# nv-tlabs/ASE

Measured on AMD Instinct MI355X. Metric: ASE PPO-update samples/sec (4096 envs x horizon 32), higher is better.
Workload: dtype f16; 1 GPU; BASELINE configs[1]: ASE agent, 4096 envs x horizon 32, obs 253 / act 31 / amp obs 1400 / latent 64, [1024,1024,512] MLPs + disc + shared-trunk encoder, minibatch 16384 (amp 4096) x 6 mini-epochs = 48 optimisation steps per update; random-init weights; precision_choice=auto without an oracle leg: the first candidate, replay=program, parallelism=single GPU

## Files before the change

ase_amd/backend.py:

```python
import ctypes as C

import torch

from . import lib as L


_HOSTFN = C.CFUNCTYPE(None, C.c_void_p)


def _ptr(t):
    return None if t is None else C.c_void_p(t.data_ptr())


def _ld(t):
    return 0 if t is None else int(t.stride(0))


def _code(dtype):
    if dtype == torch.bfloat16:
        return L.BF16
    if dtype == torch.float32:
        return L.F32
    if dtype == torch.float16:
        return L.F16
    raise L.AseHipError(f"unsupported storage dtype {dtype}")


class HipBackend:
    name = "hip"
    nt_fused_epilogue = True

    def __init__(self, device=None, x3=False):
        self.x3 = x3 if x3 == 'f16' else bool(x3)
        self._recording, self._host_keep, self._host_error = None, {}, None
        self.tn_workspace = True
        if not torch.cuda.is_available():
            raise L.AseHipError("HipBackend needs a ROCm GPU (torch.cuda.is_available() is False); "
                                "the update path has no CPU fallback")
        self.device = torch.device(device if device is not None else f"cuda:{torch.cuda.current_device()}")
        self.lib = L.get()
        self._head_scratch = torch.zeros(L.PPO_SCRATCH, dtype=torch.float64, device=self.device)
        self._head_scratch_ls = None

    def _stream(self):
        return C.c_void_p(torch.cuda.current_stream(self.device).cuda_stream)

    def zero_(self, t):
        assert t.is_contiguous()
        L.check(self.lib.ase_hip_memset(_ptr(t), 0, t.numel() * t.element_size(), self._stream()), "memset")

    def copy_(self, dst, src):
        assert dst.is_contiguous() and src.is_contiguous() and dst.dtype == src.dtype and dst.numel() == src.numel()
        L.check(self.lib.ase_hip_memcpy(_ptr(dst), _ptr(src), dst.numel() * dst.element_size(), self._stream()), "memcpy")

    def mark(self):
        ev = C.c_int(0)
        L.check(self.lib.ase_hip_mark(self._stream(), C.byref(ev)), "mark")
        return ev.value

    def wait(self, ev):
        L.check(self.lib.ase_hip_wait(self._stream(), int(ev)), "wait")

    def prog_create(self):
        p = C.c_void_p()
        L.check(self.lib.ase_hip_prog_create(C.byref(p)), "prog_create")
        return p

    def prog_begin(self, prog):
        L.check(self.lib.ase_hip_prog_begin(prog), "prog_begin")
        self._recording = prog.value
        self._host_keep.setdefault(prog.value, [])

    def prog_end(self, prog):
        self._recording = None
        L.check(self.lib.ase_hip_prog_end(prog), "prog_end")

    def host_call(self, fn):
        if self._recording is None:
            fn()
            return

        def trampoline(_arg, fn=fn):
            try:
                fn()
            except BaseException as e:
                self._host_error = e
        cb = _HOSTFN(trampoline)
        self._host_keep[self._recording].append(cb)
        L.check(self.lib.ase_hip_prog_host(C.cast(cb, C.c_void_p), None), "prog_host")

    def prog_launch(self, prog):
        L.check(self.lib.ase_hip_prog_launch(prog), "prog_launch")
        if self._host_error is not None:
            e, self._host_error = self._host_error, None
            raise e

    def prog_size(self, prog):
        return self.lib.ase_hip_prog_size(prog)

    def prog_destroy(self, prog):
        self.lib.ase_hip_prog_destroy(prog)
        self._host_keep.pop(prog.value, None)

    def _gemm_code(self, dtype, exps=None):
        c = _code(dtype)
        if self.x3 and c == L.F32:
            if self.x3 == 'f16' and exps is not None:
                return L.F32H3 | (int(exps[0]) << 8) | (int(exps[1]) << 16)
            return L.F32X3
        return c

    def gemm_nt(self, A, B, Cm, M, N, K, bias=None, aux=None, aux_mode=L.AUX_NONE, colsum=None, colsum_n=0,
                act=L.ACT_NONE, alpha=1.0, aux_split=0, aux_delta=0, mask_out=None, x3_exps=None, alpha_dev=None,
                seed=None, twin=None, sq=None, store=True):
        dt = self._gemm_code(A.dtype, x3_exps)
        assert B.dtype == A.dtype
        if aux_mode == L.AUX_RELU_BITS:
            assert aux.dtype == torch.int32
        else:
            assert aux is None or aux.dtype == A.dtype
        assert mask_out is None or mask_out.dtype == (A.dtype if act >= L.ACT_SILU else torch.int32)
        if seed is not None or twin is not None or sq is not None:
            assert (dt & 0xFF) == L.F32H3, "seed / twin / sq belong to the half-split f32 launches (x3 = 'f16', x3_exps)"
            assert Cm.dtype == torch.float32 and (store or twin is not None)
            sw, ss = seed if seed is not None else (None, 0.0)
            acc, slot, sscale, dyn = sq if sq is not None else (None, 0, 0.0, None)
            assert acc is None or acc.dtype == torch.float64
            L.check(self.lib.ase_hip_gemm_nt_ex(_ptr(A), _ld(A), _ptr(B), _ld(B), _ptr(Cm) if store else None, _ld(Cm), _ptr(bias), _ptr(aux),
                                                _ld(aux), int(aux_split), int(aux_delta), _ptr(colsum), int(colsum_n),
                                                _ptr(mask_out), _ld(mask_out), M, N, K, act, aux_mode, 0,
                                                float(alpha), _ptr(alpha_dev), dt,
                                                _ptr(sw), 0 if sw is None else sw.numel(), float(ss),
                                                _ptr(twin), _ld(twin), 0 if twin is None else _code(twin.dtype),
                                                None if acc is None else C.c_void_p(acc.data_ptr() + 8 * int(slot)), float(sscale),
                                                _ptr(dyn), self._stream()), "gemm_nt_ex")
            return
        out_f32 = int(Cm.dtype == torch.float32 and A.dtype != torch.float32)
        L.check(self.lib.ase_hip_gemm_nt(_ptr(A), _ld(A), _ptr(B), _ld(B), _ptr(Cm), _ld(Cm), _ptr(bias), _ptr(aux),
                                         _ld(aux), int(aux_split), int(aux_delta), _ptr(colsum), int(colsum_n),
                                         _ptr(mask_out), _ld(mask_out), M, N, K, act, aux_mode, out_f32,
                                         float(alpha), _ptr(alpha_dev), dt, self._stream()), "gemm_nt")

    def gemm_tn(self, A, B, G, M, N, K, n_real, k_real, split_src, split_dst, alpha=1.0, gbias=None, bias_rows=0, alpha_dev=None):
        L.check(self.lib.ase_hip_gemm_tn(_ptr(A), _ld(A), _ptr(B), _ld(B), _ptr(G), _ptr(gbias), int(bias_rows), M, N, K,
                                         n_real, k_real,
                                         split_src, split_dst, float(alpha), _ptr(alpha_dev), self._gemm_code(A.dtype), self._stream()),
                "gemm_tn")

    def grouped_tn_ok(self, dtype, M, n_real, K, bias_rows):
        return dtype in (torch.bfloat16, torch.float16) and M % 64 == 0 and bias_rows % 64 == 0

    def make_tn_plan(self, problems, target_wg=0, alpha_dev=None):
        import struct
        n = len(problems)
        tab = (C.c_int64 * (16 * n))()
        for i, (A, B, G, gb, br, M, N, K, nr, kr, ss, sd, alpha) in enumerate(problems):
            assert A.dtype in (torch.bfloat16, torch.float16) and B.dtype == A.dtype and G.dtype == torch.float32
            row = [A.data_ptr(), _ld(A), B.data_ptr(), _ld(B), G.data_ptr(), 0 if gb is None else gb.data_ptr(), int(br),
                   M, N, K, nr, kr, ss, sd, struct.unpack('<i', struct.pack('<f', float(alpha)))[0], 0]
            for j, v in enumerate(row):
                tab[16 * i + j] = int(v)
        max_work = 8192
        work = (C.c_int32 * (4 * max_work))()
        red = (C.c_int32 * (4 * max_work))()
        n_work, n_red = C.c_int(0), C.c_int(0)
        L.check(self.lib.ase_hip_gemm_tn_grouped_plan(tab, n, int(target_wg), work, max_work, C.byref(n_work), red, max_work,
                                                      C.byref(n_red)), "gemm_tn_grouped_plan")
        nw, nr = n_work.value, n_red.value
        dev_tab = torch.tensor(list(tab), dtype=torch.int64, device=self.device)
        dev_work = torch.tensor(list(work[:4 * nw]), dtype=torch.int32, device=self.device)
        dev_red = torch.tensor(list(red[:4 * nr]), dtype=torch.int32, device=self.device)
        ws = torch.empty(nw * L.TN_SLAB, dtype=torch.float32, device=self.device) if self.tn_workspace else None
        return {'problems': dev_tab, 'work': dev_work, 'n_work': nw, 'red': dev_red, 'n_red': nr, 'ws': ws, 'keep': problems,
                'dtype': _code(problems[0][0].dtype), 'alpha_dev': alpha_dev}

    def gemm_tn_grouped(self, plan):
        L.check(self.lib.ase_hip_gemm_tn_grouped(_ptr(plan['problems']), _ptr(plan['work']), plan['n_work'], _ptr(plan['red']),
                                                 plan['n_red'], _ptr(plan['ws']), _ptr(plan.get('alpha_dev')), plan['dtype'],
                                                 self._stream()),
                "gemm_tn_grouped")

    def refresh_shadow(self, W, Ws, Wts, split_src, split_dst, x3_exp=None):
        n, k = W.shape
        ref = Ws if Ws is not None else Wts
        code = _code(ref.dtype)
        if x3_exp is not None:
            assert ref.dtype == torch.float32
            code = L.F32H3 | (int(x3_exp) << 16)
        L.check(self.lib.ase_hip_refresh_shadow(_ptr(W), n, k, _ptr(Ws), _ld(Ws), _ptr(Wts), _ld(Wts), split_src,
                                                split_dst, code, self._stream()), "refresh_shadow")

    def refresh_shadow_multi(self, desc, items, dtype):
        L.check(self.lib.ase_hip_refresh_shadow_multi(_ptr(desc), desc.shape[0], _code(dtype), self._stream()),
                "refresh_shadow_multi")

    def apply_multi(self, desc, items, dtype, opt_state, acc):
        L.check(self.lib.ase_hip_apply_multi(_ptr(desc), desc.shape[0], _ptr(opt_state), _ptr(acc), _code(dtype),
                                             self._stream()), "apply_multi")

    def apply_multi_split(self, desc, items, dtype, opt_state, acc, desc2, items2):
        assert desc2.shape == (desc.shape[0], 8) and desc2.is_contiguous()
        L.check(self.lib.ase_hip_apply_multi_v2(_ptr(desc), desc.shape[0], _ptr(desc2), _ptr(opt_state), _ptr(acc), _code(dtype),
                                                self._stream()), "apply_multi_v2")

    def gather_multi(self, desc, items, idx, remap, M):
        L.check(self.lib.ase_hip_gather_multi(_ptr(desc), desc.shape[0], _ptr(idx), remap[0], remap[1], M,
                                              self._stream()), "gather_multi")

    def build_amp_obs(self, root_pos, root_rot, root_vel, root_ang_vel, dof_pos, dof_vel, key_body_pos, dof_offsets,
                      local_root_obs, root_height_obs, hist, shift=True):
        n, S, F = hist.shape
        offs = (C.c_int32 * len(dof_offsets))(*[int(x) for x in dof_offsets])
        for t in (root_pos, root_rot, root_vel, root_ang_vel, dof_pos, dof_vel, key_body_pos, hist):
            assert t.dtype == torch.float32 and t.is_contiguous()
        L.check(self.lib.ase_hip_build_amp_obs(_ptr(root_pos), _ptr(root_rot), _ptr(root_vel), _ptr(root_ang_vel), _ptr(dof_pos),
                                               _ptr(dof_vel), _ptr(key_body_pos), n, dof_pos.shape[1], key_body_pos.shape[1], offs,
                                               len(dof_offsets) - 1, int(local_root_obs), int(root_height_obs), _ptr(hist), S,
                                               int(shift), self._stream()), "build_amp_obs")

    def motion_state(self, clips, motion_ids, times):
# ... 541 lines not shown
        L.check(self.lib.ase_hip_rms_moments(_ptr(src), _ld(src), D, _ptr(idx), remap[0], remap[1], M, _ptr(state),
                                             _ptr(sums), self._stream()), "rms_moments")

    @staticmethod
    def _stream_arrays(streams):
        n = len(streams)
        srcs = (C.c_void_p * n)(*[s[0].data_ptr() for s in streams])
        lds = (C.c_int64 * n)(*[int(s[0].stride(0)) for s in streams])
        idxs = (C.c_void_p * n)(*[None if s[1] is None else s[1].data_ptr() for s in streams])
        rh = (C.c_int * n)(*[int(s[2][0]) for s in streams])
        rn = (C.c_int * n)(*[int(s[2][1]) for s in streams])
        return n, srcs, lds, idxs, rh, rn

    def rms_moments_multi(self, streams, D, M, state, sums_list):
        n, srcs, lds, idxs, rh, rn = self._stream_arrays(streams)
        sums = (C.c_void_p * n)(*[t.data_ptr() for t in sums_list])
        L.check(self.lib.ase_hip_rms_moments_multi(srcs, lds, idxs, rh, rn, sums, n, D, M, _ptr(state), self._stream()),
                "rms_moments_multi")

    def rms_normalize_multi(self, streams, D, M, means, stds, outs):
        n, srcs, lds, idxs, rh, rn = self._stream_arrays(streams)
        mp = (C.c_void_p * n)(*[t.data_ptr() for t in means])
        sp = (C.c_void_p * n)(*[t.data_ptr() for t in stds])
        op = (C.c_void_p * n)(*[t.data_ptr() for t in outs])
        lo = (C.c_int64 * n)(*[int(t.stride(0)) for t in outs])
        L.check(self.lib.ase_hip_rms_normalize_multi(srcs, lds, idxs, rh, rn, mp, sp, op, lo, n, D, M, _code(outs[0].dtype),
                                                     self._stream()), "rms_normalize_multi")

    def rms_normalize_multi_twin(self, streams, D, M, means, stds, outs, outs32):
        n, srcs, lds, idxs, rh, rn = self._stream_arrays(streams)
        mp = (C.c_void_p * n)(*[t.data_ptr() for t in means])
        sp = (C.c_void_p * n)(*[t.data_ptr() for t in stds])
        op = (C.c_void_p * n)(*[t.data_ptr() for t in outs])
        lo = (C.c_int64 * n)(*[int(t.stride(0)) for t in outs])
        assert all(t is None or t.dtype == torch.float32 for t in outs32)
        op32 = (C.c_void_p * n)(*[None if t is None else t.data_ptr() for t in outs32])
        lo32 = (C.c_int64 * n)(*[0 if t is None else int(t.stride(0)) for t in outs32])
        L.check(self.lib.ase_hip_rms_normalize_multi_v2(srcs, lds, idxs, rh, rn, mp, sp, op, lo, op32, lo32, n, D, M,
                                                        _code(outs[0].dtype), self._stream()), "rms_normalize_multi_v2")

    def rms_finalize(self, state, D, sums, count, n_streams, mean_out, std_out):
        counts = (C.c_int32 * max(n_streams, 1))(*([int(count)] * max(n_streams, 1)))
        L.check(self.lib.ase_hip_rms_finalize(_ptr(state), D, _ptr(sums), counts, n_streams, _ptr(mean_out),
                                              _ptr(std_out), self._stream()), "rms_finalize")

    def rms_normalize(self, src, D, idx, remap, M, mean, std, outs):
        outs = list(outs) + [None] * (3 - len(outs))
        dt = _code(outs[0].dtype)
        L.check(self.lib.ase_hip_rms_normalize(_ptr(src), _ld(src), D, _ptr(idx), remap[0], remap[1], M, _ptr(mean),
                                               _ptr(std), _ptr(outs[0]), _ld(outs[0]), _ptr(outs[1]), _ld(outs[1]),
                                               _ptr(outs[2]), _ld(outs[2]), dt, self._stream()), "rms_normalize")

    def rms_unnormalize(self, state, x, y):
        L.check(self.lib.ase_hip_rms_unnormalize(_ptr(state), _ptr(x), _ptr(y), x.numel(), self._stream()),
                "rms_unnormalize")

    def gather_rows(self, src, D, idx, remap, M, dst):
        L.check(self.lib.ase_hip_gather_rows(_ptr(src), _ld(src), D, _ptr(idx), remap[0], remap[1], M, _ptr(dst),
                                             _ld(dst), _code(dst.dtype), self._stream()), "gather_rows")

    def reduce_sum(self, x, n, square, acc, slot):
        L.check(self.lib.ase_hip_reduce_sum(_ptr(x), n, int(square), _ptr(acc), slot, self._stream()), "reduce_sum")

    def ppo_head(self, mu, value, mb, new_z, logstd, d_mu, d_value, db_mu, db_value, acc, M, m_global, act_dim,
                 z_dim, masked, div_on, mu_tanh, clip_value, e_clip, critic_coef, bounds_coef, div_coef, div_tar,
                 mu_out=None, grad_scale=1.0, dyn=None, ls_mode=L.LS_FROZEN, d_logstd=None, db_logstd=None, entropy_coef=0.0):
        scratch = self._head_scratch if ls_mode == L.LS_FROZEN else self.reserve_learned_logstd()
        L.check(self.lib.ase_hip_ppo_head(
            _ptr(mu), _ld(mu), _ptr(value), _ld(value), _ptr(mb['actions']), _ptr(mb['mu']), _ptr(mb['sigma']),
            _ptr(mb['old_logp_actions']), _ptr(mb['advantages']), _ptr(mb.get('old_values')), _ptr(mb['returns']),
            _ptr(mb.get('rand_action_mask')), _ptr(mb.get('ase_latents')), _ptr(new_z), _ptr(logstd),
            _ptr(d_mu), _ld(d_mu), _ptr(d_value), _ld(d_value), _ptr(db_mu), _ptr(db_value), _ptr(mu_out), _ptr(acc),
            _ptr(scratch),
            M, m_global, act_dim, z_dim, int(masked), int(div_on), int(mu_tanh), int(clip_value),
            float(e_clip), float(critic_coef), float(bounds_coef), float(div_coef), float(div_tar), float(grad_scale),
            _ptr(dyn), int(ls_mode), _ld(logstd) if ls_mode == L.LS_ROWS else 0, _ptr(d_logstd), _ld(d_logstd),
            _ptr(db_logstd), float(entropy_coef), _code(d_mu.dtype), self._stream()), "ppo_head")

    def reserve_learned_logstd(self):
        if self._head_scratch_ls is None:
            self._head_scratch_ls = torch.zeros(L.PPO_SCRATCH_LS, dtype=torch.float64, device=self.device)
        return self._head_scratch_ls

    def disc_head(self, logit, d_logit, db_logit, acc, amb, amb_global, disc_coef, grad_scale=1.0, dyn=None):
        L.check(self.lib.ase_hip_disc_head(_ptr(logit), _ld(logit), _ptr(d_logit), _ld(d_logit), _ptr(db_logit),
                                           _ptr(acc), amb, amb_global, float(disc_coef), float(grad_scale), _ptr(dyn),
                                           _code(d_logit.dtype), self._stream()), "disc_head")

    def enc_head(self, e, z, d_e, db_enc, enc_out, acc, amb, amb_global, z_dim, enc_coef, grad_scale=1.0, dyn=None):
        L.check(self.lib.ase_hip_enc_head(_ptr(e), _ld(e), _ptr(z), _ld(z), _ptr(d_e), _ld(d_e), _ptr(db_enc),
                                          _ptr(enc_out), _ptr(acc), amb, amb_global, z_dim, float(enc_coef), float(grad_scale),
                                          _ptr(dyn), _code(d_e.dtype), self._stream()), "enc_head")

    def enc_gp_seed(self, e, z, u, rows, z_dim, scale=1.0):
        assert e.dtype == torch.float32 and z.dtype == torch.float32
        L.check(self.lib.ase_hip_enc_gp_seed(_ptr(e), _ld(e), _ptr(z), _ld(z), _ptr(u), _ld(u), rows, z_dim, float(scale),
                                             _code(u.dtype), self._stream()), "enc_gp_seed")

    def enc_gp_back(self, e, z, du, d_e, db_enc, rows, z_dim, grad_scale=1.0, dyn=None):
        assert e.dtype == torch.float32 and z.dtype == torch.float32 and du.dtype == torch.float32
        L.check(self.lib.ase_hip_enc_gp_back(_ptr(e), _ld(e), _ptr(z), _ld(z), _ptr(du), _ld(du), _ptr(d_e), _ld(d_e),
                                             _ptr(db_enc), rows, z_dim, float(grad_scale), _ptr(dyn), _code(d_e.dtype),
                                             self._stream()), "enc_gp_back")

    def gp_seed(self, h, w, g, rows, width, scale=1.0, act=L.ACT_RELU):
        L.check(self.lib.ase_hip_gp_seed(_ptr(h), _ld(h), _ptr(w), _ptr(g), _ld(g), rows, width, float(scale), int(act),
                                         _code(h.dtype), self._stream()), "gp_seed")

    def gp_second(self, twin, g, dg, dz, rows, width, act):
        L.check(self.lib.ase_hip_gp_second(_ptr(twin), _ld(twin), _ptr(g), _ld(g), _ptr(dg), _ld(dg), _ptr(dz), _ld(dz), rows,
                                           width, int(act), _code(dz.dtype), self._stream()), "gp_second")

    def colsum(self, x, rows, cols, out, scale=1.0):
        assert x.dtype == torch.float32 and out.dtype == torch.float32
        L.check(self.lib.ase_hip_colsum(_ptr(x), _ld(x), rows, cols, float(scale), _ptr(out), self._stream()), "colsum")

    def sqnorm(self, x, rows, cols, acc, slot, scale=1.0, dyn=None):
        L.check(self.lib.ase_hip_sqnorm(_ptr(x), _ld(x), rows, cols, _ptr(acc), slot, float(scale), _ptr(dyn), _code(x.dtype),
                                        self._stream()),
                "sqnorm")

    def finalize_scalars(self, acc, out, m_global, amb_global, masked, has_disc, has_enc, has_div, c, opt_state=None, kl_threshold=0.0):
        L.check(self.lib.ase_hip_finalize_scalars(
            _ptr(acc), _ptr(out), m_global, amb_global, int(masked), int(has_disc), int(has_enc), int(has_div),
            float(c['critic_coef']), float(c['entropy_coef']), float(c.get('bounds_loss_coef') or 0.0), float(c.get('disc_coef', 0)),
            float(c.get('disc_logit_reg', 0)), float(c.get('disc_grad_penalty', 0)), float(c.get('disc_weight_decay', 0)),
            float(c.get('enc_coef', 0)), float(c.get('enc_weight_decay', 0)), float(c.get('amp_diversity_bonus', 0)),
            float(c.get('enc_grad_penalty', 0)), _ptr(opt_state), float(kl_threshold), self._stream()), "finalize_scalars")

    def begin_step(self, opt_state, acc, zero2=None, rng_bump=None):
        L.check(self.lib.ase_hip_begin_step(_ptr(opt_state), _ptr(acc), 0 if acc is None else acc.numel(), _ptr(zero2),
                                            0 if zero2 is None else zero2.numel(), _ptr(rng_bump), self._stream()),
                "begin_step")

    def adam(self, w, g, m, v, opt_state):
        L.check(self.lib.ase_hip_adam(_ptr(w), _ptr(g), _ptr(m), _ptr(v), w.numel(), _ptr(opt_state), self._stream()),
                "adam")

    def clip_scale(self, g, acc, slot, max_norm):
        L.check(self.lib.ase_hip_clip_scale(_ptr(g), g.numel(), _ptr(acc[slot:]), float(max_norm), self._stream()), "clip_scale")

    def axpy(self, g, w, c):
        L.check(self.lib.ase_hip_axpy(_ptr(g), _ptr(w), g.numel(), float(c), self._stream()), "axpy")

    def scaler_check(self, buf, scaler):
        assert buf.is_contiguous()
        L.check(self.lib.ase_hip_scaler_check(_ptr(buf), buf.numel(), _code(buf.dtype), _ptr(scaler), self._stream()),
                "scaler_check")

    def scaler_check_multi(self, bufs, scaler, table=None):
        if table is None:
            table = self.make_check_table(bufs)
        L.check(self.lib.ase_hip_scaler_check_multi(_ptr(table['rows']), table['n'], table['wg'], _ptr(scaler), self._stream()),
                "scaler_check_multi")

    def make_check_table(self, bufs):
        rows = []
        for t in bufs:
            assert t.is_contiguous() and t.numel() > 0
            rows.append([t.data_ptr(), t.numel(), _code(t.dtype)])
        big = max(t.numel() * t.element_size() for t in bufs)
        wg = max(1, min(1024, (big + 16383) // 16384))
        return {'rows': torch.tensor(rows, dtype=torch.int64, device=self.device), 'n': len(rows), 'wg': int(wg), 'keep': list(bufs)}

    def scaler_fold(self, scaler, scale_tab):
        L.check(self.lib.ase_hip_scaler_fold(_ptr(scaler), _ptr(scale_tab), self._stream()), "scaler_fold")

    def scaler_step(self, scaler, opt_state, opt_eff, grads, scale_tab=None):
        L.check(self.lib.ase_hip_scaler_step(_ptr(scaler), _ptr(opt_state), _ptr(opt_eff), _ptr(grads), grads.numel(),
                                             _ptr(scale_tab), self._stream()), "scaler_step")
# ... 38 lines not shown
```

ase_amd/csrc/gemm.hip:

```cpp
#include "gemm_nt.h"
#include <math.h>

namespace ase_nt {

unsigned long long* g_nt_prof = nullptr;
int g_nt_prof_clk = 0;

int nt_choice(int M, int N, int K, int es, bool b16) {
    if (N <= 64) return 0;
    const int t256 = ((M + 255) / 256) * ((N + 255) / 256);
    const bool big = N % 256 == 0 && t256 >= 192 && (t256 <= 256 || t256 % 256 == 0 || t256 >= 1024);
    if (big) {
        if (!(b16 && (K * es) % 128 == 0)) return 3;
        const int t192 = ((M + 191) / 192) * (N / 256);
        return (t256 < 256 && t192 <= 256 && t192 > t256) ? 6 : 2;
    }
    if ((K * es) % 128 != 0) return 1;
    const int t128 = ((M + 127) / 128) * ((N + 127) / 128), t64x128 = ((M + 63) / 64) * ((N + 127) / 128);
    if (t128 >= 512) return 1;
    if (t64x128 >= 512) return 4;
    return 5;
}

}

using namespace ase_nt;

extern "C" int ase_hip_debug_nt_profile(void* buf) {
    g_nt_prof = reinterpret_cast<unsigned long long*>(buf);
    return ASE_OK;
}

extern "C" int ase_hip_debug_nt_profile_clock(int shader_clock) {
    g_nt_prof_clk = shader_clock ? 1 : 0;
    return ASE_OK;
}

extern "C" int ase_hip_gemm_nt_kernel_id(int M, int N, int K, int dtype) {
    dtype &= 0xFF;
    return nt_choice(M, N, K, ase_elem_size(dtype), ase_elem_size(dtype) == 2);
}

namespace {

struct NTFused {
    const float* seed_w = nullptr; int seed_n = 0; float seed_scale = 0.f;
    void* twin = nullptr; int64_t ldtwin = 0; int twin_dtype = 0;
    double* sq_acc = nullptr; double sq_scale = 0.0; const float* sq_dyn = nullptr;
    bool any() const { return seed_w || twin || sq_acc; }
};

int gemm_nt_impl(const void* A, int64_t lda, const void* B, int64_t ldb, void* C, int64_t ldc,
                 const float* bias, const void* aux, int64_t ldaux, int aux_split, int aux_delta,
                 float* colsum, int colsum_n, void* mask_out, int64_t ldmask, int M, int N, int K, int act,
                 int aux_mode, int out_f32, float alpha, float* alpha_dev, int dtype_word, const NTFused& fu, void* stream) {
    const int dtype = dtype_word & 0xFF, ea = (dtype_word >> 8) & 0xFF, eb = (dtype_word >> 16) & 0xFF;
    const int es = ase_elem_size(dtype);
    ASE_CHECK_ARG(dtype == ASE_F32 || dtype == ASE_BF16 || dtype == ASE_F32X3 || dtype == ASE_F16 || dtype == ASE_F32H3,
                  "gemm_nt: bad dtype %d", dtype);
    ASE_CHECK_ARG(ea >= 0 && ea <= 24 && eb >= 0 && eb <= 24 && (dtype == ASE_F32H3 || (ea | eb) == 0),
                  "gemm_nt: operand scale exponents (bits 8-15 / 16-23 of dtype) are 0..24 and belong to ASE_F32H3 only");
    ASE_CHECK_ARG(A && B && (C || fu.twin) && M > 0 && N > 0 && K > 0, "gemm_nt: null/empty operand (M=%d N=%d K=%d)", M, N, K);
    if (fu.any()) {
        ASE_CHECK_ARG(dtype == ASE_F32H3 && colsum == nullptr && act <= ASE_ACT_RELU &&
                          (aux_mode == ASE_AUX_NONE || aux_mode == ASE_AUX_RELU_BITS),
                      "gemm_nt_ex: seed / twin / sum of squares belong to ASE_F32H3 launches without column sums, with no activation or "
                      "ReLU and no mask operand or a bit matrix");
        ASE_CHECK_ARG(fu.seed_w == nullptr || (fu.seed_n >= 0 && fu.seed_n <= N), "gemm_nt_ex: seed_n=%d outside [0, N]", fu.seed_n);
        ASE_CHECK_ARG(fu.twin == nullptr || ((fu.twin_dtype == ASE_F16 || fu.twin_dtype == ASE_BF16) && fu.ldtwin >= N &&
                                             ((uintptr_t)fu.twin % 8) == 0 && (fu.ldtwin * 2) % 8 == 0),
                      "gemm_nt_ex: the twin is f16 / bf16, 8-byte aligned, ldtwin >= N in whole 8-byte steps");
        ASE_CHECK_ARG(fu.sq_acc == nullptr || ((uintptr_t)fu.sq_acc % 8) == 0, "gemm_nt_ex: misaligned sq_acc");
    }
    ASE_CHECK_ARG((K * es) % 64 == 0, "gemm_nt: K=%d is not a multiple of %d elements", K, 64 / es);
    ASE_CHECK_ARG(lda >= K && ldb >= K && (ldc >= N || C == nullptr), "gemm_nt: leading dimension too small");
    ASE_CHECK_ARG(((uintptr_t)A % 16) == 0 && ((uintptr_t)B % 16) == 0 && (lda * es) % 16 == 0 && (ldb * es) % 16 == 0,
                  "gemm_nt: A/B must be 16-byte aligned with 16-byte row pitch");
    ASE_CHECK_ARG(aux_mode == ASE_AUX_NONE || aux != nullptr, "gemm_nt: aux_mode %d without aux", aux_mode);
    const bool bits = aux_mode == ASE_AUX_RELU_BITS;
    ASE_CHECK_ARG(N % 4 == 0 && ((uintptr_t)C % 16) == 0 && (ldc * (out_f32 ? 4 : es)) % 8 == 0 &&
                      (aux == nullptr || bits || (((uintptr_t)aux % 8) == 0 && (ldaux * es) % 8 == 0)),
                  "gemm_nt: C / aux must allow 8/16-byte row-vector access (N %% 4 == 0, aligned pitches)");
    ASE_CHECK_ARG(!bits || (((uintptr_t)aux % 4) == 0 && ldaux * 32 >= N), "gemm_nt: bit mask needs ldaux >= N / 32 words");
    const bool smooth = act >= ASE_ACT_SILU;
    ASE_CHECK_ARG(act >= ASE_ACT_NONE && act <= ASE_ACT_SOFTPLUS, "gemm_nt: unknown activation %d", act);
    ASE_CHECK_ARG((aux_mode & 0xFF) <= ASE_AUX_PREACT && ((aux_mode & 0xFF) == ASE_AUX_PREACT || (aux_mode >> 8) == 0) &&
                      (aux_mode >> 8) <= ASE_ACT_SOFTPLUS, "gemm_nt: bad aux_mode 0x%x", aux_mode);
    ASE_CHECK_ARG(mask_out == nullptr || smooth || (N % 32 == 0 && ((uintptr_t)mask_out % 4) == 0 && ldmask * 32 >= N),
                  "gemm_nt: mask_out needs N %% 32 == 0 and ldmask >= N / 32 words");
    ASE_CHECK_ARG(mask_out == nullptr || !smooth || (ldmask >= N && ((uintptr_t)mask_out % 16) == 0 && (ldmask * es) % 8 == 0),
                  "gemm_nt: the pre-activation twin needs ldmask >= N elements, 16-byte alignment");
    NTParams p;
    p.A = (const char*)A; p.lda = lda * es;
    p.B = (const char*)B; p.ldb = ldb * es;
    p.C = (char*)C; p.ldc = ldc * (out_f32 ? 4 : es);
    p.mask_out = smooth ? nullptr : (uint32_t*)mask_out; p.ldmask = ldmask;
    p.pre_out = smooth ? (char*)mask_out : nullptr; p.ldpre = ldmask * es;
    p.bias = bias; p.aux = (const char*)aux; p.ldaux = bits ? ldaux * 4 : ldaux * es; p.aux_split = aux_split > 0 ? aux_split : M; p.aux_delta = aux_delta; p.colsum = colsum; p.colsum_n = colsum ? colsum_n : 0;
    p.M = M; p.N = N; p.K = K; p.act = act; p.aux_mode = aux_mode; p.out_f32 = out_f32; p.alpha = alpha; p.alpha_dev = alpha_dev;
    p.tiles_m = p.tiles_n = 0;
    p.prof = nullptr;
    p.prof_clk = 0;
    p.sa = 1.f;
    p.seed_w = fu.seed_w; p.seed_n = fu.seed_n; p.seed_scale = fu.seed_scale;
    p.twin = (char*)fu.twin; p.ldtwin = fu.ldtwin * 2; p.twin_dtype = fu.twin_dtype;
    p.sq_acc = fu.sq_acc; p.sq_scale = fu.sq_scale; p.sq_dyn = fu.sq_dyn;
    if (dtype == ASE_BF16) return dispatch_nt_bf16(p, (hipStream_t)stream);
    if (dtype == ASE_F16) return dispatch_nt_f16(p, (hipStream_t)stream);
    if (dtype == ASE_F32X3) return dispatch_nt_x3(p, (hipStream_t)stream);
    if (dtype == ASE_F32H3) {
        p.sa = ldexpf(1.f, ea);
        p.alpha = ldexpf(alpha, -(ea + eb));
        return dispatch_nt_h3(p, (hipStream_t)stream);
    }
    return dispatch_nt_f32(p, (hipStream_t)stream);
}

}

extern "C" int ase_hip_gemm_nt(const void* A, int64_t lda, const void* B, int64_t ldb, void* C, int64_t ldc,
                               const float* bias, const void* aux, int64_t ldaux, int aux_split, int aux_delta,
                               float* colsum, int colsum_n, void* mask_out, int64_t ldmask, int M, int N, int K, int act,
                               int aux_mode, int out_f32, float alpha, float* alpha_dev, int dtype_word, void* stream) {
    return gemm_nt_impl(A, lda, B, ldb, C, ldc, bias, aux, ldaux, aux_split, aux_delta, colsum, colsum_n, mask_out, ldmask, M, N, K,
                        act, aux_mode, out_f32, alpha, alpha_dev, dtype_word, NTFused{}, stream);
}

extern "C" int ase_hip_gemm_nt_ex(const void* A, int64_t lda, const void* B, int64_t ldb, void* C, int64_t ldc,
                                  const float* bias, const void* aux, int64_t ldaux, int aux_split, int aux_delta,
                                  float* colsum, int colsum_n, void* mask_out, int64_t ldmask, int M, int N, int K, int act,
                                  int aux_mode, int out_f32, float alpha, float* alpha_dev, int dtype_word,
                                  const float* seed_w, int seed_n, float seed_scale, void* twin, int64_t ldtwin, int twin_dtype,
                                  double* sq_acc, double sq_scale, const float* sq_dyn, void* stream) {
    NTFused fu;
    fu.seed_w = seed_w; fu.seed_n = seed_n; fu.seed_scale = seed_scale;
    fu.twin = twin; fu.ldtwin = ldtwin; fu.twin_dtype = twin_dtype;
    fu.sq_acc = sq_acc; fu.sq_scale = sq_scale; fu.sq_dyn = sq_dyn;
    return gemm_nt_impl(A, lda, B, ldb, C, ldc, bias, aux, ldaux, aux_split, aux_delta, colsum, colsum_n, mask_out, ldmask, M, N, K,
                        act, aux_mode, out_f32, alpha, alpha_dev, dtype_word, fu, stream);
}
```

ase_amd/csrc/gemm_nt.h:

```cpp
#pragma once
#include "common.h"
#include "act.h"
#include <type_traits>

namespace ase_nt {


__device__ __forceinline__ int xcd_remap(int bid, int nwg) {
    const int q = nwg >> 3, r = nwg & 7, xcd = bid & 7, loc = bid >> 3;
    const int base = (xcd < r) ? xcd * (q + 1) : r * (q + 1) + (xcd - r) * q;
    return base + loc;
}


template <int RB> __device__ __forceinline__ int lds_swz(int r) { return RB == 128 ? ((r >> 1) & 7) : ((r >> 2) & 3); }

typedef __attribute__((address_space(1))) const void gptr_t;
typedef __attribute__((address_space(3))) void lptr_t;

template <int N> __device__ __forceinline__ void wait_vmcnt() { asm volatile("s_waitcnt vmcnt(%0)" ::"n"(N) : "memory"); }

struct NTParams {
    const char* A; int64_t lda;
    const char* B; int64_t ldb;
    char* C; int64_t ldc;
    const float* bias;
    const char* aux; int64_t ldaux;
    int aux_split, aux_delta;
    float* colsum; int colsum_n;
    uint32_t* mask_out; int64_t ldmask;
    char* pre_out; int64_t ldpre;
    int M, N, K;
    int act, aux_mode, out_f32;
    float alpha;
    float* alpha_dev;
    float sa;
    int tiles_m, tiles_n;
    unsigned long long* prof;
    int prof_clk;
    const float* seed_w; int seed_n; float seed_scale;
    char* twin; int64_t ldtwin; int twin_dtype;
    double* sq_acc; double sq_scale; const float* sq_dyn;
};


typedef __attribute__((ext_vector_type(4))) int i32x4;

__device__ __forceinline__ i32x4 raw_buffer(const void* base) {
    const uint64_t a = (uint64_t)(uintptr_t)base;
    return i32x4{(int)(uint32_t)a, (int)(uint32_t)(a >> 32), (int)0x7FFFFFFF, 0x00020000};
}
#pragma clang diagnostic push
#pragma clang diagnostic ignored "-Winline-asm"
#define LDS_DMA16_ASM(SET_M0, ...)                                            \
    asm volatile(SET_M0 "\n\tbuffer_load_dwordx4 %1, %2, %3 offen lds"          \
                 :                                                              \
                 : "s"(lds_s), "v"(voff), "s"(rs), "s"(soff), "n"(IMM)          \
                 : "memory", "m0", ##__VA_ARGS__)
template <int IMM = 0, bool ADD = (IMM != 0)>
__device__ __forceinline__ void lds_dma16(uint32_t lds_s, uint32_t voff, i32x4 rs, uint32_t soff) {
    if constexpr (ADD) LDS_DMA16_ASM("s_add_u32 m0, %0, %4", "scc");
    else LDS_DMA16_ASM("s_mov_b32 m0, %0");
}
#undef LDS_DMA16_ASM
template <int IMM>
__device__ __forceinline__ void lds_dma16_global(uint32_t lds_s, const char* src) {
    asm volatile("s_add_u32 m0, %0, %2\n\ts_nop 0\n\tglobal_load_lds_dwordx4 %1, off" : : "s"(lds_s), "v"(src), "n"(IMM) : "memory", "m0", "scc");
}
#pragma clang diagnostic pop

template <typename T, bool SW>
__device__ __forceinline__ f32x16 nt8_mfma(const i32x4& a, const i32x4& b, const f32x16& c) {
    typedef typename V16<T>::x8 x8;
    if constexpr (SW) return mfma16<T>(__builtin_bit_cast(x8, b), __builtin_bit_cast(x8, a), c);
    else return mfma16<T>(__builtin_bit_cast(x8, a), __builtin_bit_cast(x8, b), c);
}


#define NT8_BARRIER()                        \
    do {                                     \
        __builtin_amdgcn_sched_barrier(0);   \
        __builtin_amdgcn_s_barrier();        \
        __builtin_amdgcn_sched_barrier(0);   \
    } while (0)


typedef float f32x2 __attribute__((ext_vector_type(2)));
typedef short i16x2 __attribute__((ext_vector_type(2)));
typedef int i32x2 __attribute__((ext_vector_type(2)));
typedef unsigned short u16x2 __attribute__((ext_vector_type(2)));
typedef __bf16 bf16x2 __attribute__((ext_vector_type(2)));
typedef _Float16 f16x2 __attribute__((ext_vector_type(2)));

template <typename T> __device__ __forceinline__ uint32_t cvt_relu_pk16(f32x2 v, float lo);
template <> __device__ __forceinline__ uint32_t cvt_relu_pk16<bf16_t>(f32x2 v, float lo) {
    const f32x2 l = {lo, lo};
    return __builtin_bit_cast(uint32_t, __builtin_convertvector(__builtin_elementwise_maximum(v, l), bf16x2));
}
template <> __device__ __forceinline__ uint32_t cvt_relu_pk16<f16_t>(f32x2 v, float lo) {
    const f16_t l16 = (f16_t)__builtin_amdgcn_fmed3f(lo, -65504.f, 65504.f);
    const f16x2 hi = {(f16_t)65504.f, (f16_t)65504.f}, l = {l16, l16};
    const f16x2 c = __builtin_elementwise_maximum(__builtin_elementwise_minimum(__builtin_convertvector(v, f16x2), hi), l);
    return __builtin_bit_cast(uint32_t, c);
}

__device__ __forceinline__ uint32_t ovf_fold(uint32_t run, uint32_t packed) {
    const uint32_t mag = packed & 0x7FFF7FFFu;
    asm("v_pk_max_u16 %0, %0, %1" : "+v"(run) : "v"(mag));
    return run;
}
template <typename T> __device__ __forceinline__ bool ovf_hit(uint32_t run) {
    return (run & 0xFFFFu) >= ovf_threshold<T>() || (run >> 16) >= ovf_threshold<T>();
}

template <typename T, int AUXK, bool MASK>
__device__ __forceinline__ uint32_t rows_frag(const f32x16& c, const f32x4 (&bias)[4], uint32_t w, f32x2 al, float relu_lo, int h,
                                              uint32_t (&pk)[4][2]) {
    uint32_t mlo = 0, mhi = 0;
#pragma unroll
    for (int g = 0; g < 4; ++g)
#pragma unroll
        for (int pr = 0; pr < 2; ++pr) {
            f32x2 v = {c[g * 4 + 2 * pr], c[g * 4 + 2 * pr + 1]};
            const f32x2 b = {bias[g][2 * pr], bias[g][2 * pr + 1]};
            v = v * al + b;
// ... 42 lines not shown
        uint32_t mword[NJ];
        uint4 out[NJ][2];
#pragma unroll
        for (int j = 0; j < NJ; ++j) {
            uint32_t pk[4][2];
            mword[j] = rows_frag<T, AUXK, MASK>(acc[i][j], bias[j], AUXK == 2 ? bits[i][j] >> (4 * h) : 0u, al, relu_lo, h, pk);
#pragma unroll
            for (int g = 0; g < 4; g += 2) {
                const auto s0 = __builtin_amdgcn_permlane32_swap(pk[g][0], pk[g + 1][0], false, false);
                const auto s1 = __builtin_amdgcn_permlane32_swap(pk[g][1], pk[g + 1][1], false, false);
                out[j][g >> 1] = make_uint4(s0[0], s1[0], s0[1], s1[1]);
                ovf = ovf_fold(ovf_fold(ovf_fold(ovf_fold(ovf, s0[0]), s1[0]), s0[1]), s1[1]);
            }
        }
        if (row_ok) {
#pragma unroll
            for (int j = 0; j < NJ; ++j)
#pragma unroll
                for (int g = 0; g < 4; g += 2) *reinterpret_cast<uint4*>(crow + (j * 32 + 8 * g) * 2) = out[j][g >> 1];
        }
        if constexpr (MASK) {
#pragma unroll
            for (int jp = 0; jp < NJ; jp += 2) {
                const auto w = __builtin_amdgcn_permlane32_swap(mword[jp], mword[jp + 1], false, false);
                const uint32_t full = w[0] | w[1];
                if (row_ok) p.mask_out[(int64_t)m * p.ldmask + (ncol0 >> 5) + jp + h] = full;
            }
        }
    }
    ovf_report(p.alpha_dev, ovf_hit<T>(ovf));
}

template <typename T, int AUXK, int NJ = 2, int NI = 4>
__device__ __forceinline__ void nt8_epilogue_rows(const NTParams& p, f32x16 (&acc)[NI][NJ], int lane, int mrow0, int ncol0,
                                                  const uint32_t (&bits)[NI][NJ]) {
    if (ncol0 >= p.N) return;
    if (p.mask_out) nt8_epilogue_rows_impl<T, AUXK, true, NJ, NI>(p, acc, lane, mrow0, ncol0, bits);
    else nt8_epilogue_rows_impl<T, AUXK, false, NJ, NI>(p, acc, lane, mrow0, ncol0, bits);
}


template <int UNITS> __device__ __forceinline__ void wait_dma_units() { wait_vmcnt<2 * UNITS>(); }
__device__ __forceinline__ void wait_dma_units_rt(int units) {
    if (units >= 4) wait_vmcnt<8>();
    else if (units == 3) wait_vmcnt<6>();
    else if (units == 2) wait_vmcnt<4>();
    else if (units == 1) wait_vmcnt<2>();
    else wait_vmcnt<0>();
}
__device__ __forceinline__ void nt8_sync_in() {
    NT8_BARRIER();
    asm volatile("s_waitcnt lgkmcnt(0)" ::: "memory");
    __builtin_amdgcn_sched_barrier(0);
    __builtin_amdgcn_s_setprio(1);
}
__device__ __forceinline__ void nt8_sync_out() {
    __builtin_amdgcn_s_setprio(0);
    NT8_BARRIER();
}

#define NT_PROF_STAMP(prof, tid, slot, shader_clk)                                                              \
    do {                                                                                                        \
        if ((prof) && (tid) == 0) (prof)[slot] = (shader_clk) ? (unsigned long long)clock64() : wall_clock64(); \
    } while (0)
#define NT_PROF_CLOSE(prof, tid, slot)                         \
    do {                                                       \
        if (prof) {                                            \
            asm volatile("s_waitcnt vmcnt(0)" ::: "memory");   \
            __syncthreads();                                   \
            if ((tid) == 0) (prof)[slot] = wall_clock64();     \
        }                                                      \
    } while (0)

extern unsigned long long* g_nt_prof;
extern int g_nt_prof_clk;

int nt_choice(int M, int N, int K, int es, bool b16);

int dispatch_nt_bf16(const NTParams& p, hipStream_t s);
int dispatch_nt_f16(const NTParams& p, hipStream_t s);
int dispatch_nt_f32(const NTParams& p, hipStream_t s);
int dispatch_nt_x3(const NTParams& p, hipStream_t s);
int dispatch_nt_h3(const NTParams& p, hipStream_t s);

}
```

ase_amd/csrc/gemm_nt_bf16.hip:

```cpp
#include "gemm_nt_kernels.h"

int ase_nt::dispatch_nt_bf16(const NTParams& p, hipStream_t s) { return dispatch_nt<bf16_t>(p, s); }
```

ase_amd/csrc/gemm_nt_f16.hip:

```cpp
#include "gemm_nt_kernels.h"

int ase_nt::dispatch_nt_f16(const NTParams& p, hipStream_t s) { return dispatch_nt<f16_t>(p, s); }
```

ase_amd/csrc/gemm_nt_kernels.h:

```cpp
#pragma once
#include "gemm_nt.h"
#include <stdlib.h>
#include <utility>

namespace {

using namespace ase_nt;

typedef uint32_t u32x4 __attribute__((ext_vector_type(4)));
template <int N, typename F, int... I> __device__ __forceinline__ void static_for_impl(F&& f, std::integer_sequence<int, I...>) {
    (f(std::integral_constant<int, I>{}), ...);
}
template <int N, typename F> __device__ __forceinline__ void static_for(F&& f) { static_for_impl<N>(f, std::make_integer_sequence<int, N>{}); }

template <typename T> struct Mma;

template <typename T> struct Mma16 {
    typedef typename V16<T>::x8 x8;
    template <int FM, int FN, int RB, bool SW = false>
    static __device__ __forceinline__ void tile(const char* sA, const char* sB, int lane, f32x16 (&acc)[FM][FN]) {
        const int r = lane & 31, h = lane >> 5, sw = lds_swz<RB>(r);
#pragma unroll
        for (int ks = 0; ks < RB / 32; ++ks) {
            x8 a[FM], b[FN];
// ... 620 lines not shown
    NTParams p = p0;
    p.tiles_m = (p.M + BM - 1) / BM;
    p.tiles_n = (p.N + BN - 1) / BN;
    ASE_LAUNCH(kern, dim3(p.tiles_m * p.tiles_n), dim3(WGM * WGN * 64), lds, stream, p);
    ASE_CHECK_LAUNCH("gemm_nt");
    return ASE_OK;
}


struct NT8Lane {
    uint32_t voff[4][2];
    uint32_t dst[4][2];
    int roff[4];
    i32x4 rsA, rsB;
};

template <int KIND>
__device__ __forceinline__ void nt8_piece(const NT8Lane& L, int g, int tile) {
    constexpr bool isB = (KIND == 1 || KIND == 2);
    lds_dma16(__builtin_amdgcn_readfirstlane(L.dst[KIND][g] + (uint32_t)(tile & 1) * 65536u), L.voff[KIND][g], isB ? L.rsB : L.rsA,
              (uint32_t)tile * 128u);
}

template <int KIND>
__device__ __forceinline__ void nt8_issue(const NT8Lane& L, int tile) {
#pragma unroll
    for (int g = 0; g < 2; ++g) nt8_piece<KIND>(L, g, tile);
}

__device__ __forceinline__ void nt8_read(i32x4 (&f)[4], const char* base, const NT8Lane& L) {
#pragma unroll
    for (int ks = 0; ks < 4; ++ks) f[ks] = *reinterpret_cast<const i32x4*>(base + L.roff[ks]);
}

template <typename T, int KIND, bool SW, int NA = 2>
__device__ __forceinline__ void nt8_mma_issue(f32x16& c0, f32x16& c1, const i32x4 (&a0)[4], const i32x4 (&a1)[4],
                                              const i32x4 (&b)[4], const NT8Lane& L, int tile, bool live) {
#pragma unroll
    for (int ks = 0; ks < 4; ++ks) {
        if (ks == 3) NT8_BARRIER();
        c0 = nt8_mfma<T, SW>(a0[ks], b[ks], c0);
        if constexpr (NA == 2) c1 = nt8_mfma<T, SW>(a1[ks], b[ks], c1);
        if (ks == 0 || ks == 2) {
            __builtin_amdgcn_sched_barrier(0);
            if (live) nt8_piece<KIND>(L, ks >> 1, tile);
            __builtin_amdgcn_sched_barrier(0);
        }
    }
    __builtin_amdgcn_sched_barrier(0);
    __builtin_amdgcn_s_setprio(0);
    __builtin_amdgcn_sched_barrier(0);
}

template <typename T, bool TAIL, bool SW, int NI = 4>
__device__ __forceinline__ void nt8_ktile(int t, int nk, const NT8Lane& L, const char* aP, const char* bP,
                                          f32x16 (&acc)[NI][2], i32x4 (&a0)[4], i32x4 (&a1)[4], i32x4 (&b0)[4],
                                          i32x4 (&b1)[4]) {
    constexpr int RB = 128;
    const int U = 4 * nk;
    const bool l1 = !TAIL || t + 1 < nk, l2 = !TAIL || t + 2 < nk;
    nt8_read(b0, bP, L);
    nt8_read(a0, aP, L);
    nt8_read(a1, aP + 32 * RB, L);
    if (!TAIL) wait_dma_units<3>();
    else wait_dma_units_rt(min(U, 4 * t + 6) - (4 * t + 3));
    nt8_sync_in();
    nt8_mma_issue<T, 2, SW>(acc[0][0], acc[1][0], a0, a1, b0, L, t + 1, l1);
    nt8_read(b1, bP + 32 * RB, L);
    if (!TAIL) wait_dma_units<3>();
    else wait_dma_units_rt(min(U, 4 * t + 7) - (4 * t + 4));
    nt8_sync_in();
    nt8_mma_issue<T, 3, SW>(acc[0][1], acc[1][1], a0, a1, b1, L, t + 1, l1);
    nt8_read(a0, aP + 64 * RB, L);
    if constexpr (NI == 4) nt8_read(a1, aP + 96 * RB, L);
    nt8_sync_in();
    nt8_mma_issue<T, 0, SW, NI - 2>(acc[2][1], acc[NI - 1][1], a0, a1, b1, L, t + 2, l2);
    if (!TAIL) wait_dma_units<3>();
    else if (t + 1 < nk) wait_dma_units_rt(min(U, 4 * t + 9) - (4 * t + 6));
    nt8_sync_in();
    nt8_mma_issue<T, 1, SW, NI - 2>(acc[2][0], acc[NI - 1][0], a0, a1, b0, L, t + 2, l2);
}


template <typename T, bool SW, int BM = 256>
__global__ __launch_bounds__(512) void gemm_nt8_kernel(NTParams p) {
    static_assert(sizeof(T) == 2, "the phased kernel takes the 16-bit storage types");
    static_assert(BM == 256 || (BM == 192 && SW), "192-row tiles come with the row-per-lane epilogue");
    constexpr int RB = 128, BN = 256, BK = 64, WM = BM / 2, NI = WM / 32;
    constexpr int kBuf = 512 * RB;
    extern __shared__ __attribute__((aligned(16))) char smem[];
    if (p.alpha_dev) p.alpha *= *p.alpha_dev;

    const int tid = threadIdx.x, lane = tid & 63;
    const int wid = __builtin_amdgcn_readfirstlane(tid >> 6);
    const int wr = wid >> 2, wc = wid & 3;
    const int nwg = p.tiles_m * p.tiles_n;
    const int tile = xcd_remap(blockIdx.x, nwg);
    const int bm0 = (tile / p.tiles_n) * BM, bn0 = (tile % p.tiles_n) * BN;

    NT_PROF_STAMP(p.prof, tid, blockIdx.x * 4 + 0, false);
    NT8Lane L;
    {
        const int lr = lane >> 3, slot = lane & 7;
#pragma unroll
        for (int g = 0; g < 2; ++g) {
            const int ra = g * WM + wid * 8;
            const int rb = (g * 2 + (wid >> 2)) * 64 + (wid & 3) * 8;
            const int ra1 = BM == 256 ? ra + 64 : (wid >> 2) * WM + 64 + (wid & 3) * 8;
            const int rows[4] = {ra, rb, rb + 32, ra1};
#pragma unroll
            for (int kind = 0; kind < 4; ++kind) {
                const int r = rows[kind] + lr;
                const bool isB = (kind == 1 || kind == 2);
                const int64_t grow = isB ? min(bn0 + r, p.N - 1) : min(bm0 + r, p.M - 1);
                L.voff[kind][g] = (uint32_t)(grow * (isB ? p.ldb : p.lda)) + (uint32_t)((slot ^ lds_swz<RB>(r)) << 4);
                L.dst[kind][g] = (uint32_t)(uintptr_t)smem + (isB ? BM * RB : 0) + rows[kind] * RB;
            }
        }
        const int r = lane & 31, h = lane >> 5, sw = lds_swz<RB>(r);
#pragma unroll
        for (int ks = 0; ks < 4; ++ks) L.roff[ks] = r * RB + (((ks * 2 + h) ^ sw) << 4);
        L.rsA = raw_buffer(p.A);
        L.rsB = raw_buffer(p.B);
    }

    f32x16 acc[NI][2];
#pragma unroll
    for (int i = 0; i < NI; ++i)
#pragma unroll
        for (int j = 0; j < 2; ++j)
#pragma unroll
            for (int e = 0; e < 16; ++e) acc[i][j][e] = 0.f;

    AuxReg<T, 2> pre_bits[16];
    uint32_t row_bits[NI][2];
    if constexpr (!SW) {
        if (p.aux_mode == ASE_AUX_RELU_BITS) nt_aux_load<T, 4, 2, 2, 2, 2>(p, 0, lane, bm0 + wr * WM, bn0 + wc * 64, pre_bits);
    }

    const int nk = p.K / BK;
    nt8_issue<0>(L, 0);
    nt8_issue<1>(L, 0);
    nt8_issue<2>(L, 0);
    nt8_issue<3>(L, 0);
    if (nk > 1) {
        nt8_issue<0>(L, 1);
        nt8_issue<1>(L, 1);
    }
    bool mask_dma = false;
    if constexpr (SW) {
        mask_dma = p.aux_mode == ASE_AUX_RELU_BITS && bn0 + wc * 64 < p.N;
        if (mask_dma) {
            char* mlds = smem + 2 * kBuf + wid * 1024;
#pragma unroll
            for (int i = 0; i < NI; ++i) {
                const int m = bm0 + wr * WM + i * 32 + (lane & 31);
                const int ma = (m >= p.aux_split) ? m - p.aux_delta : m;
                const uint32_t* w = reinterpret_cast<const uint32_t*>(p.aux + (int64_t)min(ma, p.M - 1) * p.ldaux) +
                                    ((bn0 + wc * 64) >> 5) + (lane >> 5);
                __builtin_amdgcn_global_load_lds((gptr_t*)w, (lptr_t*)(mlds + i * 256), 4, 0, 0);
            }
        }
    }
    if (nk > 1) {
        if (mask_dma) wait_vmcnt<8 + NI>(); else wait_dma_units<4>();
    } else {
        if (mask_dma) wait_vmcnt<4 + NI>(); else wait_dma_units<2>();
    }
    NT8_BARRIER();
    NT_PROF_STAMP(p.prof, tid, blockIdx.x * 4 + 1, p.prof_clk);
    if (wr == 1) NT8_BARRIER();

    i32x4 a0[4], a1[4], b0[4], b1[4];
    const int aoff = wr * WM * RB, boff = BM * RB + wc * 64 * RB;
    int t = 0;
    for (; t + 2 < nk; ++t) {
        const char* buf = smem + (t & 1) * kBuf;
        nt8_ktile<T, false, SW, NI>(t, nk, L, buf + aoff, buf + boff, acc, a0, a1, b0, b1);
    }
    for (; t < nk; ++t) {
        const char* buf = smem + (t & 1) * kBuf;
        nt8_ktile<T, true, SW, NI>(t, nk, L, buf + aoff, buf + boff, acc, a0, a1, b0, b1);
    }
    if (wr == 0) NT8_BARRIER();
    __syncthreads();
    NT_PROF_STAMP(p.prof, tid, blockIdx.x * 4 + 2, p.prof_clk);

    float* slab = reinterpret_cast<float*>(smem) + wid * (64 * 64);
    if constexpr (SW) {
        if (p.aux_mode == ASE_AUX_RELU_BITS) {
            const uint32_t* mw = reinterpret_cast<const uint32_t*>(smem + 2 * kBuf + wid * 1024);
#pragma unroll
            for (int i = 0; i < NI; ++i) {
                row_bits[i][0] = mw[i * 64 + (lane & 31)];
                row_bits[i][1] = mw[i * 64 + 32 + (lane & 31)];
            }
            nt8_epilogue_rows<T, 2, 2, NI>(p, acc, lane, bm0 + wr * WM, bn0 + wc * 64, row_bits);
        } else nt8_epilogue_rows<T, 0, 2, NI>(p, acc, lane, bm0 + wr * WM, bn0 + wc * 64, row_bits);
    } else if constexpr (BM == 256) {
        if (p.aux_mode == ASE_AUX_RELU_BITS)
            nt_epilogue_impl<T, 4, 2, 2, 2, 2, true>(p, acc, slab, lane, bm0 + wr * 128, bn0 + wc * 64, &pre_bits);
        else
            nt_epilogue<T, 4, 2, 2, 2>(p, acc, slab, lane, bm0 + wr * 128, bn0 + wc * 64);
    }
    NT_PROF_CLOSE(p.prof, tid, blockIdx.x * 4 + 3);
}

template <typename T, bool SW = false, int BM = 256> int launch_nt8(const NTParams& p0, hipStream_t stream) {
    constexpr int lds = 2 * 512 * 128 + (SW ? 8 * 1024 : 0);
    constexpr auto kern = gemm_nt8_kernel<T, SW, BM>;
    if (const int rc = ase_dynamic_lds<kern>("gemm_nt8", lds)) return rc;
    NTParams p = p0;
    p.prof = g_nt_prof;
    p.prof_clk = g_nt_prof_clk;
    p.tiles_m = (p.M + BM - 1) / BM;
    p.tiles_n = (p.N + 255) / 256;
    ASE_LAUNCH(kern, dim3(p.tiles_m * p.tiles_n), dim3(512), lds, stream, p);
    ASE_CHECK_LAUNCH("gemm_nt8");
    return ASE_OK;
}

}
#include "gemm_nt4.h"
namespace {

inline bool rows_epi(const NTParams& p, int wave_cols) {
    return !p.out_f32 && p.N % wave_cols == 0 && p.colsum == nullptr && p.act <= ASE_ACT_RELU &&
           (p.mask_out == nullptr || p.act == ASE_ACT_RELU) &&
           (p.aux_mode == ASE_AUX_NONE || p.aux_mode == ASE_AUX_RELU_BITS);
}

template <typename T> int dispatch_nt(const NTParams& p, hipStream_t s) {
    const bool k128 = (p.K * (int)sizeof(T)) % 128 == 0;
    const bool fits32 = (int64_t)p.M * p.lda < (int64_t)0x7FFFFFFF && (int64_t)p.N * p.ldb < (int64_t)0x7FFFFFFF;
    int choice = nt_choice(p.M, p.N, p.K, (int)sizeof(T), sizeof(T) == 2);
    if ((choice == 2 || choice == 6) && !fits32) choice = 3;
    if constexpr (std::is_same<T, f32h_t>::value) {
        if (p.seed_w || p.twin || p.sq_acc) {
            switch (choice) {
                case 0: return launch_nt<T, 2, 2, 1, 1, 64, 4, 1, false, true>(p, s);
                case 2: case 3: case 6:
                    if (k128) return launch_nt<T, 4, 2, 2, 4, 128, 2, 1, false, true>(p, s);
                    return launch_nt<T, 4, 2, 2, 4, 64, 4, 1, false, true>(p, s);
                case 4: return launch_nt<T, 2, 2, 1, 2, 128, 2, 2, false, true>(p, s);
                case 5: return launch_nt<T, 2, 2, 1, 1, 128, 4, 2, false, true>(p, s);
                default:
                    if (k128) return launch_nt<T, 2, 2, 2, 2, 128, 2, 2, false, true>(p, s);
                    return launch_nt<T, 2, 2, 2, 2, 64, 4, 2, false, true>(p, s);
            }
        }
    }
    switch (choice) {
        case 0: return launch_nt<T, 2, 2, 1, 1, 64, 4>(p, s);
        case 6:
            if constexpr (sizeof(T) == 2) if (rows_epi(p, 64)) return launch_nt8<T, true, 192>(p, s);
            [[fallthrough]];
        case 2:
            if constexpr (sizeof(T) == 2) {
                if (p.M >= 65536 && rows_epi(p, 128)) return launch_nt4<T>(p, s);
                if (rows_epi(p, 64)) return launch_nt8<T, true>(p, s);
                return launch_nt8<T, false>(p, s);
            }
            [[fallthrough]];
        case 3:
            if (k128) return launch_nt<T, 4, 2, 2, 4, 128, 2>(p, s);
            return launch_nt<T, 4, 2, 2, 4, 64, 4>(p, s);
        case 4:
            if constexpr (sizeof(T) == 2) if (rows_epi(p, 64)) return launch_nt<T, 2, 2, 1, 2, 128, 2, 2, true>(p, s);
            return launch_nt<T, 2, 2, 1, 2, 128, 2, 2>(p, s);
        case 5:
            if constexpr (sizeof(T) == 2) if (rows_epi(p, 32)) return launch_nt<T, 2, 2, 1, 1, 128, 4, 2, true>(p, s);
            return launch_nt<T, 2, 2, 1, 1, 128, 4, 2>(p, s);
        default:
            if constexpr (sizeof(T) == 2) if (k128 && rows_epi(p, 64)) return launch_nt<T, 2, 2, 2, 2, 128, 2, 1, true>(p, s);
            if (k128) return launch_nt<T, 2, 2, 2, 2, 128, 2>(p, s);
            return launch_nt<T, 2, 2, 2, 2, 64, 4>(p, s);
    }
}

}
```

ase_amd/csrc/heads.hip:

```cpp
#include "common.h"
#include "act.h"

namespace {

constexpr float kHalfLog2Pi = 0.91893853320467274178f;

__global__ __launch_bounds__(256) void reduce_sum_kernel(const float* __restrict__ x, int64_t n, int square,
                                                         double* __restrict__ acc) {
    __shared__ double sm[16];
    double v[1] = {0.0};
    for (int64_t i = blockIdx.x * (int64_t)blockDim.x + threadIdx.x; i < n; i += (int64_t)gridDim.x * blockDim.x) {
        const double t = (double)x[i];
        v[0] += square ? t * t : t;
    }
    block_sum<1>(v, sm);
    if (threadIdx.x == 0) atomic_add_f64(acc, v[0]);
}

struct PpoArgs {
    const float* mu; int64_t ld_mu;
    const float* value; int64_t ld_v;
    const float *actions, *old_mu, *old_sigma, *old_logp, *adv, *old_value, *ret, *mask, *z, *new_z, *logstd;
    void* d_mu; int64_t ld_dmu;
    void* d_value; int64_t ld_dv;
// ... 141 lines not shown
            } else {
                c = (R - v) * (R - v);
                dv = 2.f * (v - R);
            }
            const T ov = from_f32<T>(p.gs * (p.critic_coef * dv / (float)p.m_global));
            reinterpret_cast<T*>(p.d_value)[(int64_t)i * p.ld_dv] = ov;
            bad |= ovf_hit1(ov);
            dv_out += p.inv_gs * to_f32(ov);
            part[0] += (double)(mk * a_loss);
            part[1] += (double)(mk * b_row);
            part[2] += (double)(mk * ent_row);
            part[3] += (double)(mk * ((fabsf(ratio - 1.f) > p.e_clip) ? 1.f : 0.f));
            part[4] += (double)c;
            part[5] += (double)kl_row;
            part[6] += (double)(mk * div_row);
        }
    }
    ovf_report(p.gs_dev, bad);
    double* const slabs = p.scratch + 8;
    double* mine = slabs + (int64_t)blockIdx.x * NSLOT;
    sdb[rib][lane] = gm_out + gm2_out;
    if (lane == 0) sdb[rib][LPR] = dv_out;
    if constexpr (LS != LS_FROZEN) sdl[rib][lane] = gl_out;
    __syncthreads();
    if (threadIdx.x < LPR + 1) {
        float t = 0.f;
#pragma unroll
        for (int q = 0; q < ROWS; ++q) t += sdb[q][threadIdx.x];
        mine[7 + (threadIdx.x < LPR ? threadIdx.x : 64)] = (double)t;
    }
    if constexpr (LS != LS_FROZEN) {
        if (threadIdx.x >= 128 && threadIdx.x < 128 + LPR) {
            const int c = threadIdx.x - 128;
            float t = 0.f;
#pragma unroll
            for (int q = 0; q < ROWS; ++q) t += sdl[q][c];
            mine[kPpoSlots + c] = (double)t;
        }
    }
    block_sum<7>(part, sm);
    if (threadIdx.x == 0) {
#pragma unroll
        for (int k = 0; k < 7; ++k) mine[k] = part[k];
    }
}

template <int NS>
__global__ __launch_bounds__(256) void ppo_head_fold_kernel(const double* __restrict__ slabs, int nblocks, double* __restrict__ acc,
                                                            float* __restrict__ db_mu, float* __restrict__ db_value, int act_dim,
                                                            int div_on, float* __restrict__ db_ls) {
    __shared__ double fold[4][NS];
    const int c = threadIdx.x & 63, g4 = threadIdx.x >> 6;
    const int per = (nblocks + gridDim.x - 1) / gridDim.x, lo = blockIdx.x * per, hi = min(nblocks, lo + per);
    for (int cc = c; cc < NS; cc += 64) {
        double t[8] = {0, 0, 0, 0, 0, 0, 0, 0};
        int b = lo + g4;
        for (; b + 28 < hi; b += 32) {
#pragma unroll
            for (int u = 0; u < 8; ++u) t[u] += slabs[(int64_t)(b + 4 * u) * NS + cc];
        }
        for (; b < hi; b += 4) t[0] += slabs[(int64_t)b * NS + cc];
        fold[g4][cc] = ((t[0] + t[1]) + (t[2] + t[3])) + ((t[4] + t[5]) + (t[6] + t[7]));
    }
    __syncthreads();
    if (threadIdx.x < NS) {
        const int cc = threadIdx.x;
        const double t = fold[0][cc] + fold[1][cc] + fold[2][cc] + fold[3][cc];
        if (cc < 7) {
            const int slot[7] = {ASE_ACC_A_LOSS, ASE_ACC_B_LOSS, ASE_ACC_ENTROPY, ASE_ACC_CLIPPED, ASE_ACC_C_LOSS, ASE_ACC_KL, ASE_ACC_DIV};
            if (cc < 6 || div_on) atomic_add_f64(acc + slot[cc], t);
        } else if (db_mu) {
            const int j = cc - 7;
            if (j < act_dim) atomic_add_f32(db_mu + j, (float)t);
            else if (j == 64 && db_value) atomic_add_f32(db_value, (float)t);
        }
        if (NS > 72 && cc >= 72 && cc - 72 < act_dim && db_ls) atomic_add_f32(db_ls + (cc - 72), (float)t);
    }
}

template <typename T>
__global__ __launch_bounds__(256) void disc_head_kernel(const float* __restrict__ logit, int64_t ld_l, T* __restrict__ d_logit,
                                                        int64_t ld_d, float* __restrict__ db_logit, double* __restrict__ acc,
                                                        int amb, int amb_global, float disc_coef, float gs,
                                                        float* __restrict__ gs_dev) {
    __shared__ double sm[5 * 16];
    if (gs_dev) gs *= *gs_dev;
    const int r = blockIdx.x * blockDim.x + threadIdx.x;
    double part[5] = {0, 0, 0, 0, 0};
    bool bad = false;
    if (r < 3 * amb) {
        const float l = logit[(int64_t)r * ld_l];
        const float sp_abs = log1pf(expf(-fabsf(l)));
        float g;
        if (r < 2 * amb) {
            part[0] = (double)(fmaxf(l, 0.f) + sp_abs);
            part[2] = (l < 0.f) ? 1.0 : 0.0;
            const float sig = 1.f / (1.f + expf(-l));
            g = disc_coef * 0.5f * sig / (2.f * (float)amb_global);
        } else {
            part[1] = (double)(fmaxf(-l, 0.f) + sp_abs);
            part[3] = (l > 0.f) ? 1.0 : 0.0;
            const float sig_neg = 1.f / (1.f + expf(l));
            g = -disc_coef * 0.5f * sig_neg / (float)amb_global;
        }
        const T o = from_f32<T>(gs * g);
        d_logit[(int64_t)r * ld_d] = o;
        bad = ovf_hit1(o);
        part[4] = (double)(to_f32(o) / gs);
    }
    ovf_report(gs_dev, bad);
    block_sum<5>(part, sm);
    if (threadIdx.x == 0) {
        if (db_logit) atomic_add_f32(db_logit, (float)part[4]);
        atomic_add_f64(acc + ASE_ACC_BCE_AGENT, part[0]);
        atomic_add_f64(acc + ASE_ACC_BCE_DEMO, part[1]);
        atomic_add_f64(acc + ASE_ACC_AGENT_ACC, part[2]);
        atomic_add_f64(acc + ASE_ACC_DEMO_ACC, part[3]);
    }
}

template <typename T>
__global__ __launch_bounds__(256) void enc_head_kernel(const float* __restrict__ e, int64_t ld_e, const float* __restrict__ z,
                                                       int64_t ld_z, T* __restrict__ d_e, int64_t ld_de,
                                                       float* __restrict__ db_enc, float* __restrict__ enc_out,
                                                       double* __restrict__ acc, int amb, int amb_global, int z_dim,
                                                       float enc_coef, float gs, float* __restrict__ gs_dev) {
    __shared__ double sm[16];
    if (gs_dev) gs *= *gs_dev;
    __shared__ float sdb[4][128];
    float dbv[2] = {0.f, 0.f};
    const int lane = threadIdx.x & 63;
    double part[1] = {0.0};
    bool bad = false;
    for (int r = blockIdx.x * 4 + (threadIdx.x >> 6); r < amb; r += gridDim.x * 4) {
        float ev[2] = {0.f, 0.f}, zv[2] = {0.f, 0.f};
#pragma unroll
        for (int q = 0; q < 2; ++q) {
            const int j = lane + 64 * q;
            if (j < z_dim) {
                ev[q] = e[(int64_t)r * ld_e + j];
                zv[q] = z[(int64_t)r * ld_z + j];
            }
        }
        const float ss = wave_sum(ev[0] * ev[0] + ev[1] * ev[1]);
        const float nrm = floor_nan(sqrtf(ss), 1e-12f);
        const float h0 = ev[0] / nrm, h1 = ev[1] / nrm;
        const float dot = wave_sum(h0 * zv[0] + h1 * zv[1]);
        const float sc = enc_coef / (float)amb_global;
#pragma unroll
        for (int q = 0; q < 2; ++q) {
            const int j = lane + 64 * q;
            if (j < z_dim) {
                const float h = q ? h1 : h0;
                const T o = from_f32<T>(gs * (-sc * (zv[q] - h * dot) / nrm));
                d_e[(int64_t)r * ld_de + j] = o;
                bad |= ovf_hit1(o);
                dbv[q] += to_f32(o) / gs;
                if (enc_out) enc_out[(int64_t)r * z_dim + j] = h;
            }
        }
        if (lane == 0) part[0] += (double)(-dot);
    }
    ovf_report(gs_dev, bad);
    if (db_enc) {
        sdb[threadIdx.x >> 6][lane] = dbv[0];
        sdb[threadIdx.x >> 6][lane + 64] = dbv[1];
        __syncthreads();
        if (threadIdx.x < z_dim) {
            const float t = sdb[0][threadIdx.x] + sdb[1][threadIdx.x] + sdb[2][threadIdx.x] + sdb[3][threadIdx.x];
            atomic_add_f32(db_enc + threadIdx.x, t);
        }
    }
    block_sum<1>(part, sm);
    if (threadIdx.x == 0) atomic_add_f64(acc + ASE_ACC_ENC, part[0]);
}

template <typename T, int MODE>
__global__ __launch_bounds__(256) void enc_gp_kernel(const float* __restrict__ e, int64_t ld_e, const float* __restrict__ z,
                                                     int64_t ld_z, const float* __restrict__ du, int64_t ld_du,
                                                     T* __restrict__ out, int64_t ld_out, float* __restrict__ db_enc,
                                                     int rows, int z_dim, float scale, float* __restrict__ scale_dev) {
    __shared__ float sdb[4][128];
    if (scale_dev) scale *= *scale_dev;
    float dbv[2] = {0.f, 0.f};
    bool bad = false;
    const int lane = threadIdx.x & 63;
    for (int r = blockIdx.x * 4 + (threadIdx.x >> 6); r < rows; r += gridDim.x * 4) {
        float ev[2] = {0.f, 0.f}, zv[2] = {0.f, 0.f}, dv[2] = {0.f, 0.f};
#pragma unroll
        for (int q = 0; q < 2; ++q) {
            const int j = lane + 64 * q;
            if (j < z_dim) {
                ev[q] = e[(int64_t)r * ld_e + j];
                zv[q] = z[(int64_t)r * ld_z + j];
                if (MODE == 1) dv[q] = du[(int64_t)r * ld_du + j];
            }
        }
        const float len = sqrtf(wave_sum(ev[0] * ev[0] + ev[1] * ev[1]));
        const float nrm = floor_nan(len, 1e-12f);
        const bool flat = len < 1e-12f;
// ... 180 lines not shown
    out[ASE_RES_LOSS] = (float)loss;
    if (a.opt_state) {
        double lr = a.opt_state[1];
        const double cur = lr;
        out[ASE_RES_LR] = (float)cur;
        if (kl > 2.0 * (double)a.kl_threshold) lr = fmax(cur / 1.5, 1e-6);
        if (kl < 0.5 * (double)a.kl_threshold) lr = fmin(cur * 1.5, 1e-2);
        a.opt_state[1] = lr;
    }
}

inline int grid_for(int64_t n, int block = 256, int cap = 2048) {
    int64_t g = (n + block - 1) / block;
    return (int)(g < 1 ? 1 : (g > cap ? cap : g));
}

}

extern "C" int ase_hip_reduce_sum(const float* x, int64_t n, int square, double* acc, int slot, void* stream) {
    ASE_CHECK_ARG(x && acc && n > 0 && slot >= 0, "reduce_sum: null/empty operand");
    ASE_LAUNCH(reduce_sum_kernel, dim3(grid_for(n, 1024, 128)), dim3(256), 0, (hipStream_t)stream, x, n, square,
                       acc + slot);
    ASE_CHECK_LAUNCH("reduce_sum");
    return ASE_OK;
}

extern "C" int ase_hip_ppo_head(const float* mu, int64_t ld_mu, const float* value, int64_t ld_v,
                                const float* mb_actions, const float* mb_old_mu, const float* mb_old_sigma,
                                const float* mb_old_logp, const float* mb_adv, const float* mb_old_value,
                                const float* mb_return, const float* mb_mask, const float* mb_z, const float* new_z,
                                const float* logstd, void* d_mu, int64_t ld_dmu, void* d_value, int64_t ld_dv,
                                float* db_mu, float* db_value, float* mu_out, double* acc, double* scratch, int M, int m_global, int act_dim, int z_dim, int masked,
                                int div_on, int mu_tanh, int clip_value, float e_clip, float critic_coef,
                                float bounds_coef, float div_coef, float div_tar, float grad_scale, float* grad_scale_dev,
                                int ls_mode, int64_t ld_ls, void* d_ls, int64_t ld_dls, float* db_ls, float entropy_coef, int dtype,
                                void* stream) {
    ASE_CHECK_ARG(mu && value && mb_actions && mb_old_mu && mb_old_sigma && mb_old_logp && mb_adv && mb_return &&
                      logstd && d_mu && d_value && acc && scratch && M > 0 && m_global >= M,
                  "ppo_head: null/empty operand");
    ASE_CHECK_ARG(act_dim >= 1 && act_dim <= 64, "ppo_head: act_dim %d not in [1,64]", act_dim);
    ASE_CHECK_ARG(!masked || mb_mask, "ppo_head: masked reduction without a mask");
    ASE_CHECK_ARG(!div_on || (mb_z && new_z && z_dim > 0), "ppo_head: diversity loss without latents");
    ASE_CHECK_ARG(!clip_value || mb_old_value, "ppo_head: clip_value without old values");
    ASE_CHECK_ARG(grad_scale > 0.f, "ppo_head: grad_scale must be positive");
    ASE_CHECK_ARG(ls_mode >= LS_FROZEN && ls_mode <= LS_ROWS, "ppo_head: log-std mode %d", ls_mode);
    ASE_CHECK_ARG(ls_mode != LS_ROWS || ld_ls >= act_dim, "ppo_head: per-row log-std stride %lld < act_dim", (long long)ld_ls);
    ASE_CHECK_ARG(!d_ls || (ls_mode != LS_FROZEN && ld_dls >= act_dim), "ppo_head: bad d logstd operand");
    PpoArgs p;
    p.mu = mu; p.ld_mu = ld_mu; p.value = value; p.ld_v = ld_v;
    p.actions = mb_actions; p.old_mu = mb_old_mu; p.old_sigma = mb_old_sigma; p.old_logp = mb_old_logp;
    p.adv = mb_adv; p.old_value = mb_old_value; p.ret = mb_return; p.mask = mb_mask; p.z = mb_z; p.new_z = new_z;
    p.logstd = logstd; p.d_mu = d_mu; p.ld_dmu = ld_dmu; p.d_value = d_value; p.ld_dv = ld_dv; p.db_mu = db_mu; p.db_value = db_value; p.mu_out = mu_out;
    p.acc = acc; p.scratch = scratch; p.M = M; p.m_global = m_global; p.act_dim = act_dim; p.z_dim = z_dim; p.masked = masked;
    p.div_on = div_on; p.mu_tanh = mu_tanh; p.clip_value = clip_value; p.e_clip = e_clip; p.critic_coef = critic_coef;
    p.bounds_coef = bounds_coef; p.div_coef = div_coef; p.div_tar = div_tar; p.gs = grad_scale; p.inv_gs = 1.f / grad_scale; p.gs_dev = grad_scale_dev;
    p.ld_ls = ld_ls; p.d_ls = d_ls; p.ld_dls = ld_dls; p.db_ls = db_ls; p.entropy_coef = entropy_coef;
    const int rows = act_dim <= 32 ? 8 : 4;
    const dim3 grid(min((M + rows - 1) / rows, 1024));
    const int rc = ase_dispatch_storage(dtype, [&](auto tag) {
        typedef typename decltype(tag)::type T;
        if (ls_mode == LS_FROZEN) {
            if (act_dim <= 32) ASE_LAUNCH((ppo_head_kernel<T, 32, LS_FROZEN>), grid, dim3(256), 0, (hipStream_t)stream, p);
            else ASE_LAUNCH((ppo_head_kernel<T, 64, LS_FROZEN>), grid, dim3(256), 0, (hipStream_t)stream, p);
        } else if (ls_mode == LS_VECTOR) {
            if (act_dim <= 32) ASE_LAUNCH((ppo_head_kernel<T, 32, LS_VECTOR>), grid, dim3(256), 0, (hipStream_t)stream, p);
            else ASE_LAUNCH((ppo_head_kernel<T, 64, LS_VECTOR>), grid, dim3(256), 0, (hipStream_t)stream, p);
        } else {
            if (act_dim <= 32) ASE_LAUNCH((ppo_head_kernel<T, 32, LS_ROWS>), grid, dim3(256), 0, (hipStream_t)stream, p);
            else ASE_LAUNCH((ppo_head_kernel<T, 64, LS_ROWS>), grid, dim3(256), 0, (hipStream_t)stream, p);
        }
        return ASE_OK;
    });
    ASE_CHECK_ARG(rc == ASE_OK, "ppo_head: bad dtype %d", dtype);
    if (ls_mode == LS_FROZEN)
        ASE_LAUNCH(ppo_head_fold_kernel<kPpoSlots>, dim3(grid.x >= 64 ? 8 : 1), dim3(256), 0, (hipStream_t)stream, (const double*)(scratch + 8),
                   (int)grid.x, acc, db_mu, db_value, act_dim, div_on, (float*)nullptr);
    else
        ASE_LAUNCH(ppo_head_fold_kernel<kPpoSlotsLs>, dim3(grid.x >= 64 ? 8 : 1), dim3(256), 0, (hipStream_t)stream, (const double*)(scratch + 8),
                   (int)grid.x, acc, db_mu, db_value, act_dim, div_on, db_ls);
    ASE_CHECK_LAUNCH("ppo_head");
    return ASE_OK;
}

extern "C" int ase_hip_disc_head(const float* logit, int64_t ld_l, void* d_logit, int64_t ld_d, float* db_logit,
                                 double* acc, int amb, int amb_global, float disc_coef, float grad_scale,
                                 float* grad_scale_dev, int dtype, void* stream) {
    ASE_CHECK_ARG(logit && d_logit && acc && amb > 0 && amb_global >= amb && grad_scale > 0.f, "disc_head: null/empty operand");
    const dim3 grid((3 * amb + 255) / 256);
    const int rc = ase_dispatch_storage(dtype, [&](auto tag) {
        typedef typename decltype(tag)::type T;
        ASE_LAUNCH(disc_head_kernel<T>, grid, dim3(256), 0, (hipStream_t)stream, logit, ld_l, (T*)d_logit, ld_d, db_logit, acc, amb,
                   amb_global, disc_coef, grad_scale, grad_scale_dev);
        return ASE_OK;
    });
    ASE_CHECK_ARG(rc == ASE_OK, "disc_head: bad dtype %d", dtype);
    ASE_CHECK_LAUNCH("disc_head");
    return ASE_OK;
}

extern "C" int ase_hip_enc_head(const float* e, int64_t ld_e, const float* z, int64_t ld_z, void* d_e, int64_t ld_de,
                                float* db_enc, float* enc_out, double* acc, int amb, int amb_global, int z_dim, float enc_coef,
                                float grad_scale, float* grad_scale_dev, int dtype, void* stream) {
    ASE_CHECK_ARG(e && z && d_e && acc && amb > 0 && amb_global >= amb && grad_scale > 0.f, "enc_head: null/empty operand");
    ASE_CHECK_ARG(z_dim >= 1 && z_dim <= 128, "enc_head: z_dim %d not in [1,128]", z_dim);
    const dim3 grid(min((amb + 3) / 4, 128));
    const int rc = ase_dispatch_storage(dtype, [&](auto tag) {
        typedef typename decltype(tag)::type T;
        ASE_LAUNCH(enc_head_kernel<T>, grid, dim3(256), 0, (hipStream_t)stream, e, ld_e, z, ld_z, (T*)d_e, ld_de, db_enc, enc_out, acc,
                   amb, amb_global, z_dim, enc_coef, grad_scale, grad_scale_dev);
        return ASE_OK;
    });
    ASE_CHECK_ARG(rc == ASE_OK, "enc_head: bad dtype %d", dtype);
    ASE_CHECK_LAUNCH("enc_head");
    return ASE_OK;
}

extern "C" int ase_hip_enc_gp_seed(const float* e, int64_t ld_e, const float* z, int64_t ld_z, void* u, int64_t ld_u, int rows,
                                   int z_dim, float scale, int dtype, void* stream) {
    ASE_CHECK_ARG(e && z && u && rows > 0, "enc_gp_seed: null/empty operand");
    ASE_CHECK_ARG(z_dim >= 1 && z_dim <= 128, "enc_gp_seed: z_dim %d not in [1,128]", z_dim);
    const dim3 grid(min((rows + 3) / 4, 1024));
    const int rc = ase_dispatch_storage(dtype, [&](auto tag) {
        typedef typename decltype(tag)::type T;
        ASE_LAUNCH((enc_gp_kernel<T, 0>), grid, dim3(256), 0, (hipStream_t)stream, e, ld_e, z, ld_z, (const float*)nullptr,
                   (int64_t)0, (T*)u, ld_u, (float*)nullptr, rows, z_dim, scale, (float*)nullptr);
        return ASE_OK;
    });
    ASE_CHECK_ARG(rc == ASE_OK, "enc_gp_seed: bad dtype %d", dtype);
    ASE_CHECK_LAUNCH("enc_gp_seed");
    return ASE_OK;
}

extern "C" int ase_hip_enc_gp_back(const float* e, int64_t ld_e, const float* z, int64_t ld_z, const float* du, int64_t ld_du,
                                   void* d_e, int64_t ld_de, float* db_enc, int rows, int z_dim, float grad_scale,
                                   float* grad_scale_dev, int dtype, void* stream) {
    ASE_CHECK_ARG(e && z && du && d_e && rows > 0 && grad_scale > 0.f, "enc_gp_back: null/empty operand");
    ASE_CHECK_ARG(z_dim >= 1 && z_dim <= 128, "enc_gp_back: z_dim %d not in [1,128]", z_dim);
    const dim3 grid(min((rows + 3) / 4, 128));
    const int rc = ase_dispatch_storage(dtype, [&](auto tag) {
        typedef typename decltype(tag)::type T;
        ASE_LAUNCH((enc_gp_kernel<T, 1>), grid, dim3(256), 0, (hipStream_t)stream, e, ld_e, z, ld_z, du, ld_du, (T*)d_e, ld_de,
                   db_enc, rows, z_dim, grad_scale, grad_scale_dev);
        return ASE_OK;
    });
    ASE_CHECK_ARG(rc == ASE_OK, "enc_gp_back: bad dtype %d", dtype);
    ASE_CHECK_LAUNCH("enc_gp_back");
    return ASE_OK;
}

extern "C" int ase_hip_gp_seed(const void* h, int64_t ld_h, const float* w, void* g, int64_t ld_g, int rows, int width,
                               float scale, int act, int dtype, void* stream) {
    ASE_CHECK_ARG(h && w && g && rows > 0 && width > 0, "gp_seed: null/empty operand");
    ASE_CHECK_ARG(act >= ASE_ACT_RELU && act <= ASE_ACT_SOFTPLUS, "gp_seed: activation %d", act);
    const dim3 grid(grid_for((int64_t)rows * width));
    const int rc = ase_dispatch_storage(dtype, [&](auto tag) {
        typedef typename decltype(tag)::type T;
        ASE_LAUNCH(gp_seed_kernel<T>, grid, dim3(256), 0, (hipStream_t)stream, (const T*)h, ld_h, w, (T*)g, ld_g, rows, width, scale,
                   act);
        return ASE_OK;
    });
    ASE_CHECK_ARG(rc == ASE_OK, "gp_seed: bad dtype %d", dtype);
    ASE_CHECK_LAUNCH("gp_seed");
    return ASE_OK;
}

extern "C" int ase_hip_gp_second(const void* twin, int64_t ld_t, const void* g, int64_t ld_g, const void* dg, int64_t ld_dg,
                                 void* dz, int64_t ld_dz, int rows, int width, int act, int dtype, void* stream) {
    ASE_CHECK_ARG(twin && g && dg && dz && rows > 0 && width > 0, "gp_second: null/empty operand");
    ASE_CHECK_ARG(act >= ASE_ACT_RELU && act <= ASE_ACT_SOFTPLUS, "gp_second: activation %d", act);
    const dim3 grid(grid_for((int64_t)rows * width));
    const int rc = ase_dispatch_storage(dtype, [&](auto tag) {
        typedef typename decltype(tag)::type T;
        ASE_LAUNCH(gp_second_kernel<T>, grid, dim3(256), 0, (hipStream_t)stream, (const T*)twin, ld_t, (const T*)g, ld_g, (const T*)dg,
                   ld_dg, (T*)dz, ld_dz, rows, width, act);
        return ASE_OK;
    });
    ASE_CHECK_ARG(rc == ASE_OK, "gp_second: bad dtype %d", dtype);
    ASE_CHECK_LAUNCH("gp_second");
    return ASE_OK;
}
// ... 47 lines not shown
```

ase_amd/engine.py:

```python
import contextlib
import math

import torch

from . import lib as L
from .forward import _ACT, _AUX, Dense, ForwardEngine, P


class _StepState:
    __slots__ = ('disc_fwd_out', 'merged_stats', 'stats_mark_a', 'stats_mark_b', 'stats_exchanged', 'pre_done', 'prep',
                 'lat_ready', 'fill_done', 'early_fork', 'enc_z_ready', 'gp_x_done', 'gp_value_done', 'disc_acc_mark',
                 'acc_in_bucket', 'lr_live')

    def __init__(self):
        self.disc_fwd_out = self.stats_mark_a = self.stats_mark_b = self.pre_done = self.prep = self.lat_ready = None
        self.fill_done = self.early_fork = self.gp_value_done = self.disc_acc_mark = None
        self.merged_stats = self.stats_exchanged = self.enc_z_ready = self.gp_x_done = self.acc_in_bucket = self.lr_live = False


class UpdateEngine(ForwardEngine):

    def __init__(self, kind, net, cfg, backend, *, minibatch, amp_minibatch=0, dtype=torch.bfloat16,
                 world_size=1, rank=0, dp_mode='shard', grad_scale=None):
        self.R, self.rank = world_size, rank
        assert dp_mode in ('shard', 'horovod')
        self.shard = dp_mode == 'shard'
        div = world_size if self.shard else 1
        assert minibatch % div == 0 and amp_minibatch % div == 0
        self.Mg, self.AMBg = minibatch, amp_minibatch
        self.M, self.AMB = minibatch // div, amp_minibatch // div
        scale_given = grad_scale is not None
        if grad_scale is None:
            grad_scale = 2.0 ** max(0, round(math.log2(max(minibatch, 4) / 4.0))) if dtype == torch.float16 else 1.0
        ls = cfg.get('loss_scale', None)
        if ls is None:
            ls = 'dynamic' if (cfg.get('mixed_precision', False) and dtype == torch.float16 and not scale_given) else 'static'
        assert ls in ('static', 'dynamic'), ls
        self.dyn_scale = ls == 'dynamic'
        if self.dyn_scale:
            assert dtype == torch.float16, "loss_scale: dynamic belongs to half storage (precision f16 / f16gp32 / f16gpx3)"
            assert not (cfg.get('graph_capture') == 'hipgraph' and (world_size > 1 or cfg.get('force_dist', False))), \
                "loss_scale: dynamic exchanges its overflow flag inside the optimizer phase: not capturable as a hipGraph"
            sc = dict(init_scale=65536.0, growth_factor=2.0, backoff_factor=0.5, growth_interval=2000)
            unknown = set(cfg.get('loss_scaler', {}) or {}) - set(sc)
            assert not unknown, f"unknown loss_scaler keys {sorted(unknown)}"
            sc.update(cfg.get('loss_scaler', {}) or {})
            for k in ('init_scale', 'growth_factor', 'backoff_factor'):
                assert sc[k] > 0 and math.log2(sc[k]) == round(math.log2(sc[k])), f"loss_scaler.{k} must be a power of two"
            assert sc['growth_factor'] >= 1.0 and sc['backoff_factor'] <= 1.0 and int(sc['growth_interval']) >= 1
            self.loss_scaler = sc
            if not scale_given:
                grad_scale = float(sc['init_scale'])
        self._gs_init = float(grad_scale)
        self.gs = 1.0 if self.dyn_scale else float(grad_scale)
        self.truncate = bool(cfg.get('truncate_grads', False))
        self.grad_norm = float(cfg.get('grad_norm', 1.0))
        self.bounds_coef = float(cfg.get('bounds_loss_coef') or 0.0)
        self.adaptive_lr = cfg.get('lr_schedule', 'constant') == 'adaptive'
        self.kl_threshold = float(cfg.get('kl_threshold', 0.008))
        self.masked = kind in ('amp', 'ase')
        self.div_on = kind == 'ase' and cfg.get('amp_diversity_bonus', 0) != 0
        self.enc_gp = kind == 'ase' and cfg.get('enc_grad_penalty', 0) != 0 and cfg.get('enc_coef', 0) != 0
        self.ls_mode = {'frozen': L.LS_FROZEN, 'vector': L.LS_VECTOR, 'head': L.LS_ROWS}[getattr(net, 'sigma_mode', 'frozen')]
        self.gp32 = bool(cfg.get('gp_f32', False)) and kind in ('amp', 'ase') and dtype in (torch.float16, torch.bfloat16) and \
            cfg.get('disc_coef', 0) * cfg.get('disc_grad_penalty', 0) != 0
        self.multi_stream = bool(cfg.get('multi_stream', True)) and getattr(backend, 'name', '') == 'hip'
        self._side_streams = None
        o = dict(tn_grouped=True, tn_wg_side=64, disc_early=True, short_prologue=True, relu_bits=True, fused_apply=True,
                 apply_wide=True, xstep=True, gp_stream='auto', side_priority=None, prefetch=True, gp_fuse='auto')
        unknown = set(cfg.get('engine_opts', {}) or {}) - set(o)
        assert not unknown, f"unknown engine_opts {sorted(unknown)}"
        o.update(cfg.get('engine_opts', {}) or {})
        self.engine_opts = o
        self._tn_defer = bool(getattr(backend, 'grouped_tn_ok', None)) and bool(o['tn_grouped'])
        self._tn_queue, self._tn_plans = [], {}
        self._tn_wg_side = int(o['tn_wg_side'])
        self._disc_early = bool(o['disc_early'])
        self._short_prologue = bool(o['short_prologue']) and cfg.get('graph_capture') != 'hipgraph'
        self._apply_groups = None
        self._use_bits = bool(o['relu_bits'])
        self._fused_apply = hasattr(backend, 'apply_multi') and bool(o['fused_apply'])
        self._xstep = bool(o['xstep']) and cfg.get('graph_capture') != 'hipgraph'
        gp_side = (self.dyn_scale or self.M < 8192) if o['gp_stream'] == 'auto' else bool(o['gp_stream'])
        self._gp_side = gp_side and cfg.get('graph_capture') != 'hipgraph'
        self._gp_fuse = bool(self.gp32 and getattr(backend, 'nt_fused_epilogue', False) and cfg.get('gp_f32') == 'x3'
                             and getattr(backend, 'x3', None) is not None and (o['gp_fuse'] == 'auto' or bool(o['gp_fuse'])))
        self._gp_split = self._gp_fuse and hasattr(backend, 'apply_multi_split') and self._fused_apply and dtype == torch.float16
        self._prefetch = bool(o['prefetch'])
        self._par, self._par_set, self._last_par, self._fenced = 0, False, None, False
        sp = o['side_priority']
        if sp is None:
            sp = [0, -1, 0] if (self.gp32 or self.dyn_scale) else [-1, 0, 0]
        self._side_prio = [int(x) for x in sp] if isinstance(sp, (list, tuple)) else [int(sp)] * 3
        self._gp_stream_obj = None
        self._xs = False
        self._st = _StepState()
        self._apply_wide = bool(o['apply_wide'])
        self._apply_desc = self._apply_items = None
        self.force_dist = bool(cfg.get('force_dist', False))
        self.dp_grad_dtype = cfg.get('dp_grad_dtype', 'f32')
        assert self.dp_grad_dtype in ('f32', 'bf16'), self.dp_grad_dtype
        self._xbuf = {}
        self._mb_desc = None
        self._mb_desc_key = None
        super().__init__(kind, net, cfg, backend, dtype=dtype)

    def _bind_params(self):
        super()._bind_params()
        net, dev = self.net, self.dev
        n = self.params.numel()
        self.grads = torch.zeros(n, dtype=torch.float32, device=dev)
        self.adam_m = torch.zeros(n, dtype=torch.float32, device=dev)
        self.adam_v = torch.zeros(n, dtype=torch.float32, device=dev)
        self.n_train = net.trainable_numel
        lr = float(self.cfg['learning_rate'])
        self.opt_state = torch.tensor([0.0, lr, 0.9, 0.999, 1e-8, 1.0, 1.0, 0.0], dtype=torch.float64, device=dev)
        self.scaler = torch.zeros(8, dtype=torch.float64, device=dev)
        self.scale_tab = torch.tensor([1.0, 0.0, 1.0, 0.0, 1.0, 0.0, 1.0, 0.0], dtype=torch.float32, device=dev)
        if self.dyn_scale:
            sc = self.loss_scaler
            self.scaler[4:8] = torch.tensor([self._gs_init, sc['growth_factor'], sc['backoff_factor'], float(int(sc['growth_interval']))],
                                            dtype=torch.float64)
            self.set_grad_scale(self._gs_init)
        self.opt_eff = self.opt_state.clone()
        self._scaler_list = None
        self._check_tabs = {}
        for d in self.layers:
            d.gW, d.gb = [], []
            for name, nr, off in d.parts:
                o, _ = net.param_slices[name + '.weight']
                d.gW.append(self.grads[o:o + nr * d.K].view(nr, d.K))
                ob, _ = net.param_slices[name + '.bias']
                d.gb.append(self.grads[ob:ob + nr])
        self.glogstd = None
        if self.ls_mode != L.LS_FROZEN and hasattr(self.be, 'reserve_learned_logstd'):
            self.be.reserve_learned_logstd()
        if self.sigma_mode == 'vector':
            o, shp = net.param_slices['sigma']
            assert o + shp[0] <= self.n_train, "the learned log-std vector must be trainable"
            self.glogstd = self.grads[o:o + shp[0]]
        self.l2_terms = []
        c = self.cfg
        if self.has_disc:
            dc, wd, lr_ = c['disc_coef'], c['disc_weight_decay'], c['disc_logit_reg']
            for d in self.disc:
                self.l2_terms.append((d.W[0], d.gW[0], dc * 2.0 * wd, L.ACC_DISC_W2 if wd != 0 else None))
            self.l2_terms.append((self.disc_head.W[0], self.disc_head.gW[0], dc * 2.0 * (wd + lr_), None))
        if self.has_enc and c.get('enc_weight_decay', 0) != 0:
            ew = c['enc_coef'] * 2.0 * c['enc_weight_decay']
            chain = self.enc_chain if self.enc_sep else self.disc
            for d in chain:
                self.l2_terms.append((d.W[0], d.gW[0], ew, L.ACC_ENC_W2))
            eh = self.enc_head if self.enc_sep else self.disc_head
            ei = 0 if self.enc_sep else 1
            self.l2_terms.append((eh.W[ei], eh.gW[ei], ew, L.ACC_ENC_W2))

    def _latent_seed(self):
        return super()._latent_seed() + (0 if self.shard else 7919 * self.rank)

    def _alloc(self):
        super()._alloc()
        dev, T = self.dev, self.dtype
        M, AMB = self.M, self.AMB
        Ra = 2 * M if self.div_on else M
        self.Ra = Ra

        def zt(r, c, dt=T):
            return torch.zeros(r, c, dtype=dt, device=dev)

        def with_bits(h, d):
            if d.act == L.ACT_RELU and self._use_bits:
                self._bits[h.untyped_storage().data_ptr()] = (h, torch.zeros(h.shape[0], h.shape[1] // 32, dtype=torch.int32,
                                                                                device=dev))
            elif d.act >= L.ACT_SILU:
                self._bits[h.untyped_storage().data_ptr()] = (h, torch.zeros_like(h))
            return h

        def chain_bufs(chain, rows):
            return [with_bits(zt(rows, d.n_pad), d) for d in chain], [zt(rows, d.n_pad) for d in chain]

        f32 = torch.float32
        nset = 2 if (self._prefetch and self._xstep and self.multi_stream) else 1
        self._Xa2 = [zt(Ra, self.actor[0].k_pad) for _ in range(nset)]
        self._Xc2 = [zt(M, self.critic[0].k_pad) for _ in range(nset)]
        self.Xa, self.Xc = self._Xa2[0], self._Xc2[0]
        self.Ha, self.dZa = chain_bufs(self.actor, Ra)
        self.Hc, self.dZc = chain_bufs(self.critic, M)
        self.MU = zt(Ra, self.mu_head.n_pad, f32)
        self.dMU = zt(Ra, self.mu_head.n_pad)
        self.V = zt(M, self.value_head.n_pad, f32)
        self.dV = zt(M, self.value_head.n_pad)
        if self.style:
            self._Zs2 = [zt(Ra, P(self.z)) for _ in range(nset)]
            self.Zs = self._Zs2[0]
            self.Hs, self.dZs = chain_bufs(self.style[:-1], Ra)
            self.dStyle = zt(Ra, P(self.z))
            self.new_z = zt(M, self.z, f32)
            self.div_rng = torch.tensor([self._latent_seed() ^ 0xD1755EED, 0], dtype=torch.int64, device=dev)
        if self.has_disc:
            Rd = 3 * AMB
            self.Xd4 = zt(4 * AMB, self.disc[0].k_pad)
            self.Xd = self.Xd4[:Rd]
            self.G0 = self.Xd4[Rd:]
            self.Hd4 = [with_bits(zt(4 * AMB, d.n_pad), d) for d in self.disc]
            self.dZd4 = [zt(4 * AMB, d.n_pad) for d in self.disc]
            self.Hd = [h[:Rd] for h in self.Hd4]
            self.dGp = [h[Rd:] for h in self.Hd4]
            self.dZd = [z[:Rd] for z in self.dZd4]
            self.Gp = [z[Rd:] for z in self.dZd4]
            self.HD = zt(Rd, self.disc_head.n_pad, f32)
            self.dHD = zt(Rd, self.disc_head.n_pad)
            self.GpTop = zt(AMB, self.disc[-1].n_pad, f32)
            if self.gp32:
                assert all(d.act == L.ACT_RELU for d in self.disc), "gp_f32 is built for ReLU discriminators"
                import types
                g = self._gp32 = types.SimpleNamespace()
                g.X = zt(AMB, self.disc[0].k_pad, f32)
                g.Ws = [zt(d.n_pad, d.k_pad, f32) for d in self.disc]
                g.Wts = [zt(d.k_pad, d.n_pad, f32) for d in self.disc]
                g.H = [None if (self._gp_fuse and d is self.disc[-1]) else zt(AMB, d.n_pad, f32) for d in self.disc]
                g.bits = [torch.zeros(AMB, d.n_pad // 32, dtype=torch.int32, device=dev) for d in self.disc]
                g.Gp = [zt(AMB, d.n_pad, f32) for d in self.disc]
                g.G0 = (torch.empty(AMB, self.disc[0].k_pad, dtype=f32, device='meta') if self._gp_fuse
                        else zt(AMB, self.disc[0].k_pad, f32))
                g.cast = None
            if self.enc_chain:
                self.He, self.dZe = chain_bufs(self.enc_chain, AMB)
                self.E = zt(AMB, self.enc_head.n_pad, f32)
                self.dE = zt(AMB, self.enc_head.n_pad)
            if self.has_enc:
                self.enc_z = zt(AMB, self.z, f32)
            if self.enc_gp:
                ech = self.enc_chain if self.enc_chain else self.disc
                ehead = self.enc_head if self.enc_chain else self.disc_head
                self.Ue = zt(AMB, ehead.n_pad)
                self.Re = [zt(AMB, d.n_pad) for d in ech]
                self.Ge = zt(AMB, ech[0].k_pad)
                self.Qe = [zt(AMB, d.n_pad) for d in ech]
                self.DUe = zt(AMB, ehead.n_pad, f32)
            self.amp_mean = zt(3, self.amp, f32)
            self.amp_std = zt(3, self.amp, f32)
        n_amp = 3 * 2 * self.amp if self.has_disc else 0
        self.stats_flat = torch.zeros(n_amp + 2 * self.obs + 1, dtype=torch.float64, device=dev)
        self.obs_sums = self.stats_flat[n_amp:n_amp + 2 * self.obs]
        if self.has_disc:
            self.amp_sums_flat = self.stats_flat[:n_amp]
            self.amp_sums = self.amp_sums_flat.view(3, 2 * self.amp)
        self.obs_mean = zt(1, self.obs, f32)
        self.obs_std = zt(1, self.obs, f32)
        self.acc = torch.zeros(L.ACC_COUNT, dtype=torch.float64, device=dev)
        self.set_result_slots(1)
        self.mb = {'actions': zt(M, self.act, f32), 'mu': zt(M, self.act, f32), 'sigma': zt(M, self.act, f32),
                   'old_logp_actions': zt(M, 1, f32), 'advantages': zt(M, 1, f32), 'old_values': zt(M, 1, f32),
                   'returns': zt(M, 1, f32)}
        if self.masked:
            self.mb['rand_action_mask'] = zt(M, 1, f32)
        if self.z:
            self.mb['ase_latents'] = zt(M, self.z, f32)

    def set_result_slots(self, n):
        dev = self.dev
        self.res_ring = torch.zeros(n, L.RES_COUNT, dtype=torch.float32, device=dev)
        self.logit_ring = torch.zeros(n, 3 * self.AMB, dtype=torch.float32, device=dev) if self.has_disc else None
        self.use_slot(0)

    def use_slot(self, i):
        self.slot = i
        self.use_parity(i)
        self.res = self.res_ring[i]
        self.logit_slot = self.logit_ring[i].view(-1, 1) if self.logit_ring is not None else None

    def use_parity(self, p):
        self._par = p = p % len(self._Xa2)
        self._par_set = True
        self.Xa, self.Xc = self._Xa2[p], self._Xc2[p]
        if self.style:
            self.Zs = self._Zs2[p]

    def refresh_shadows(self):
        super().refresh_shadows()
        if self._gp_split:
            self._gp_refresh()

    def _gp_refresh(self):
        g = self._gp32
        half = self.cfg.get('gp_f32') == 'x3' and getattr(self.be, 'x3', None) is not None
        for l, d in enumerate(self.disc):
            self.be.refresh_shadow(d.W[0], g.Ws[l], g.Wts[l], d.split_src, d.split_dst, **({'x3_exp': 11} if half else {}))

    def _apply(self, opt_state, a=None, b=None):
        desc, items = self._apply_desc[a:b], self._apply_items[a:b]
        if self._gp_split:
            self.be.apply_multi_split(desc, items, self.dtype, opt_state, self.acc, self._apply_desc2[a:b], self._apply_items2[a:b])
        else:
            self.be.apply_multi(desc, items, self.dtype, opt_state, self.acc)

    def _build_apply_desc(self):
        if self._apply_desc is not None:
            return
        import struct
        c = self.cfg
        terms = {}
        for W, gW, coef, slot in self.l2_terms:
            t = terms.setdefault(W.data_ptr(), [0.0, []])
            t[0] += coef
            if slot is not None and slot not in t[1]:
                t[1].append(slot)
        if self.has_disc:
            t = terms.setdefault(self.disc_head.W[0].data_ptr(), [0.0, []])
            t[1].insert(0, L.ACC_LOGIT_W2)
            if c['disc_weight_decay'] != 0 and L.ACC_DISC_W2 not in t[1]:
                t[1].append(L.ACC_DISC_W2)
        base = self.params.data_ptr()
        rows, items = [], []
        for d, j, row, item in self._shadow_rows():
            W, ws, wts, _, _, b, bs = item
            gW, gb, nr = d.gW[j], d.gb[j], b.numel()
            ow, ob = (W.data_ptr() - base) // 4, (b.data_ptr() - base) // 4
            mW, vW = self.adam_m[ow:ow + W.numel()], self.adam_v[ow:ow + W.numel()]
            mb, vb = self.adam_m[ob:ob + nr], self.adam_v[ob:ob + nr]
            coef, slots = terms.get(W.data_ptr(), [0.0, []])
            assert len(slots) <= 2, slots
            sa = slots[0] if len(slots) > 0 else -1
            sb = slots[1] if len(slots) > 1 else -1
            gap = d.split_dst - d.split_src
            wide = int(self._apply_wide and d.K % 4 == 0 and ws.stride(0) % 4 == 0 and wts.stride(0) % 4 == 0
                       and (d.split_src >= d.K or (d.split_src % 4 == 0 and gap % 4 == 0))
                       and ws.data_ptr() % 16 == 0 and wts.data_ptr() % 16 == 0)
            rows.append(row + [gW.data_ptr(), mW.data_ptr(), vW.data_ptr(), gb.data_ptr(), mb.data_ptr(), vb.data_ptr(),
                               struct.unpack('<i', struct.pack('<f', float(coef)))[0], sa, sb, wide, 0, 0])
# ... 110 lines not shown
                    src = ds[k].view(ds[k].shape[0], -1)
                    rows.append([src.data_ptr(), src.stride(0), src.shape[1], dst.data_ptr(), dst.stride(0), L.F32])
                    items.append((src, src.shape[1], dst))
            if self.z and part_in != 1:
                src = ds['ase_latents'].view(ds['ase_latents'].shape[0], -1)
                code = {torch.bfloat16: L.BF16, torch.float16: L.F16}.get(self.dtype, L.F32)
                for dst in (self.Zs[:self.M], self.Xc[:, self.actor[0].split_dst:]):
                    rows.append([src.data_ptr(), src.stride(0), self.z, dst.data_ptr(), dst.stride(0), code])
                    items.append((src, self.z, dst))
            self._mb_desc[part] = torch.tensor(rows, dtype=torch.int64, device=self.dev) if rows else None
            self._mb_items[part] = items
        if self._mb_desc[part] is not None:
            self.be.gather_multi(self._mb_desc[part], self._mb_items[part], idx, remap, self.M)

    def sync_from_rank0(self):
        if self.R <= 1 and not self.force_dist:
            return
        import torch.distributed as dist
        bufs = [self.params, self.adam_m, self.adam_v, self.opt_state, self.obs_state, self.val_state]
        if self.has_disc:
            bufs.append(self.amp_state)
        if self.style and self.shard:
            bufs += [self.rng_state, self.div_rng]
        for t in bufs:
            self._staged(lambda x: dist.broadcast(x, 0), t)
        self.refresh_shadows()

    def step(self, ds, idx, remap, amp_streams=None, new_z=None, apply=True, fence=True):
        inline = apply and self._fused_apply and not self.truncate
        self._xs = bool(self._xstep and inline and self.has_disc and self._short_prologue and self._disc_early
                        and self._amp_stats_in_branch())
        if self._xs and (fence or new_z is not None):
            self.fence_side_streams()
        if len(self._Xa2) == 2:
            rec = getattr(self.be, '_recording', None) is not None
            if not rec:
                if not self._par_set:
                    self.use_parity(self._par ^ 1 if self._last_par is not None else self._par)
                if self._xs and self._par == self._last_par and not self._fenced:
                    self.fence_side_streams()
                self._last_par = self._par
            self._par_set, self._fenced = False, False
        self.phase_stats(ds, idx, remap, amp_streams, advance=apply, new_z=new_z)
        self._allreduce_stats()
        self._st.lr_live = apply
        self.phase_main(ds, idx, remap, amp_streams, new_z, inline_apply=inline)
        if inline:
            self.phase_finish()
        else:
            self._allreduce_grads()
            self.phase_apply(apply)
        return self.res

    def _draw_new_latents(self, new_z):
        be, M = self.be, self.M
        if new_z is not None:
            be.copy_(self.new_z, new_z.contiguous())
            be.gather_rows(self.new_z, self.z, None, (0, 0), M, self.Zs[M:])
        else:
            be.sample_latents(self.new_z, M, self.z, self.div_rng,
                              row_offset=self.rank * M if (self.shard and self.R > 1) else 0, advance=False,
                              z2=self.Zs[M:])

    def phase_stats(self, ds, idx, remap, amp_streams=None, advance=True, new_z=None):
        st = self._st = _StepState()
        be, c, M = self.be, self.cfg, self.M
        pf = self._xs and self._prefetch and len(self._Xa2) == 2
        merged = st.merged_stats = bool(pf and self._dist_shard() and self.has_disc and self.masked)
        if merged:
            self._build_apply_desc()
            with self._Branch(self, self._side(0), nowait=True):
                be.begin_step(None, None, zero2=self.stats_flat, rng_bump=self.div_rng if self.div_on else None)
                self.gather_minibatch(ds, idx, remap, part=1)
                be.reduce_sum(self.mb['rand_action_mask'], M, False, self.stats_flat, self.stats_flat.numel() - 1)
                if c.get('normalize_input', True):
                    be.rms_moments(ds['obs'], self.obs, idx, remap, M, self.obs_state, self.obs_sums)
                st.stats_mark_a = self._mark()
        if self._xs:
            self._build_apply_desc()
            lo, hi = self._apply_groups['disc'][2:]
            with self._Branch(self, self._side(1), nowait=True):
                be.zero_(self.grads[lo:hi])
                if not merged:
                    be.zero_(self.amp_sums)
                st.disc_fwd_out = self._disc_forward(amp_streams, ds)
        if pf:
            with self._Branch(self, self._side(0), nowait=True) as st.pre_done:
                if merged:
                    be.wait(st.stats_mark_b)
                else:
                    be.begin_step(None, None, zero2=self.obs_sums, rng_bump=self.div_rng if self.div_on else None)
                if c.get('normalize_input', True) and not merged:
                    be.rms_moments(ds['obs'], self.obs, idx, remap, M, self.obs_state, self.obs_sums)
                    if self._dist_shard():
                        self._ar(self.obs_sums)
                self._obs_inputs(ds, idx, remap)
                self.gather_minibatch(ds, idx, remap, part=2)
                if self.div_on:
                    self._draw_new_latents(new_z)
                st.lat_ready = self._mark()
                if not merged:
                    self.gather_minibatch(ds, idx, remap, part=1)
            tail = self._mark()
            plo, phi = self._apply_groups['policy'][2:]
            with self._Branch(self, self._side(0), tail) as st.prep:
                be.begin_step(self.opt_state if advance else None, self.acc, zero2=None, rng_bump=None)
                st.early_fork = self._mark()
                be.zero_(self.grads[plo:phi])
                if merged:
                    be.copy_(self.acc[L.ACC_MASK_SUM:L.ACC_MASK_SUM + 1], self.stats_flat[-1:])
                elif self.masked:
                    be.reduce_sum(self.mb['rand_action_mask'], M, False, self.acc, L.ACC_MASK_SUM)
                    if self._dist_shard():
                        self._ar(self.acc[L.ACC_MASK_SUM:L.ACC_MASK_SUM + 1])
            st.stats_exchanged = True
            return
        be.begin_step(self.opt_state if advance else None, self.acc,
                      zero2=self.obs_sums if self._xs else self.stats_flat, rng_bump=self.div_rng if self.div_on else None)
        if self._short_prologue and self._amp_stats_in_branch():
            m0 = self._mark()
            with self._Branch(self, self._side(1), m0):
                be.zero_(self.grads[:self.n_train])
                st.fill_done = self._mark()
            st.early_fork = st.fill_done if self.has_disc else None
            with self._Branch(self, self._side(0), m0) as st.prep:
                self.gather_minibatch(ds, idx, remap, part=2)
                if self.div_on:
                    self._draw_new_latents(new_z)
                st.lat_ready = self._mark()
                self.gather_minibatch(ds, idx, remap, part=1)
                if self.masked:
                    be.reduce_sum(self.mb['rand_action_mask'], M, False, self.acc, L.ACC_MASK_SUM)
            if c.get('normalize_input', True):
                be.rms_moments(ds['obs'], self.obs, idx, remap, M, self.obs_state, self.obs_sums)
            return
        be.zero_(self.grads[:self.n_train])
        st.early_fork = self._mark() if (self.has_disc and self._amp_stats_in_branch() and self._disc_early) else None
        self.gather_minibatch(ds, idx, remap)
        if self.masked:
            be.reduce_sum(self.mb['rand_action_mask'], M, False, self.acc, L.ACC_MASK_SUM)
        if c.get('normalize_input', True):
            be.rms_moments(ds['obs'], self.obs, idx, remap, M, self.obs_state, self.obs_sums)
        if self.has_disc and not self._amp_stats_in_branch():
            self._amp_moments(amp_streams)

    def _amp_stats_in_branch(self):
        return self.multi_stream and not (self._dist_shard() and self.cfg.get('graph_capture') == 'hipgraph')

    def _dist_shard(self):
        return self._dist_on() and self.shard

    @property
    def _m_den(self):
        return self.Mg if self.shard else self.M

    @property
    def _amb_den(self):
        return self.AMBg if self.shard else self.AMB

    def _obs_inputs(self, ds, idx, remap):
        be, M = self.be, self.M
        if self.cfg.get('normalize_input', True):
            be.rms_finalize(self.obs_state, self.obs, self.obs_sums, self._m_den, 1, self.obs_mean, self.obs_std)
        else:
            self._identity_stats(self.obs_mean, self.obs_std)
        outs = [self.Xa[:M], self.Xc]
        if self.div_on:
# ... 49 lines not shown
            self.eng, self.stream, self.after, self.nowait = eng, stream, after, nowait

        def __enter__(self):
            if self.stream is not None:
                after = None if self.nowait else (self.after if self.after is not None else self.eng.be.mark())
                self.ctx = torch.cuda.stream(self.stream)
                self.ctx.__enter__()
                if after is not None:
                    self.eng.be.wait(after)
            return self

        def __exit__(self, *a):
            if self.stream is not None:
                self.done = self.eng.be.mark()
                self.ctx.__exit__(*a)

    def _join_branch(self, br):
        if br.stream is not None:
            self.be.wait(br.done)

    def _mark(self):
        return self.be.mark() if self.multi_stream else None

    def _finish_branch(self, group, inline_apply, last=False):
        self._flush_tn(0 if last else self._tn_wg_side)
        if inline_apply:
            a, b, lo, hi = self._apply_groups[group]
            if self._dist_on():
                with_acc = bool(last and self.shard and self.dp_grad_dtype == 'f32')
                if with_acc and self._st.disc_acc_mark is not None:
                    self.be.wait(self._st.disc_acc_mark)
                self._exchange_bucket(group, lo, hi, with_acc)
                self._st.acc_in_bucket = with_acc
                if not self.shard:
                    self._host(lambda: self.grads[lo:hi].mul_(1.0 / self.R))
            if self.dyn_scale:
                self._dyn_check(group, lo, hi)
                if last:
                    self._dyn_apply()
            else:
                self._apply(self.opt_state, a, b)

    def _disc_forward(self, amp_streams, ds=None):
        self._disc_inputs(amp_streams, ds)
        return self._disc_matrices()

    def _disc_inputs(self, amp_streams, ds=None):
        be, c, AMB, st = self.be, self.cfg, self.AMB, self._st
        if self._amp_stats_in_branch():
            self._amp_moments(amp_streams)
            self._exchange_amp_sums()
        if self.has_disc and c.get('normalize_amp_input', True):
            be.rms_finalize(self.amp_state, self.amp, self.amp_sums, self._amb_den, 3, self.amp_mean, self.amp_std)
        else:
            self._identity_stats(self.amp_mean, self.amp_std)
        x_twin = self._gp_fuse and hasattr(be, 'rms_normalize_multi_twin') and self.amp % 4 == 0 and \
            all(src.stride(0) % 4 == 0 for src, _, _ in amp_streams)
        gp_fork = self._mark() if (self.gp32 and self._gp_side and not x_twin) else None
        if self.has_enc and ds is not None:
            self._gather_enc_z(ds, amp_streams)
        xd = [self.Xd[s * AMB:(s + 1) * AMB] for s in range(3)]
        st.gp_x_done = x_twin
        if x_twin:
            be.rms_normalize_multi_twin(amp_streams, self.amp, AMB, [self.amp_mean[s] for s in range(3)],
                                        [self.amp_std[s] for s in range(3)], xd, [None, None, self._gp32.X])
            gp_fork = self._mark() if self._gp_side else None
        elif self.amp % 4 == 0 and all(src.stride(0) % 4 == 0 for src, _, _ in amp_streams):
            be.rms_normalize_multi(amp_streams, self.amp, AMB, [self.amp_mean[s] for s in range(3)],
                                   [self.amp_std[s] for s in range(3)], xd)
        else:
            for s, (src, sidx, srm) in enumerate(amp_streams):
                be.rms_normalize(src, self.amp, sidx, srm, AMB, self.amp_mean[s], self.amp_std[s], [xd[s]])
        if self.gp32:
            gp_coef = c['disc_coef'] * c['disc_grad_penalty']
            if gp_fork is not None:
                with self._Branch(self, self._gp_stream(), gp_fork) as st.gp_value_done:
                    self._gp_value(amp_streams, gp_coef)
            else:
                self._gp_value(amp_streams, gp_coef)

    def _disc_matrices(self):
        be, AMB = self.be, self.AMB
        Rd = 3 * AMB
        hd = self._fwd_chain(self.disc, self.Xd, self.Hd, Rd)
        self._fwd(self.disc_head, hd, self.HD, Rd)
        if self.logit_slot is not None:
            be.gather_rows(self.HD, 1, None, (0, 0), Rd, self.logit_slot)
        he = None
        if self.enc_chain:
            he = self._fwd_chain(self.enc_chain, self.Xd[:AMB], self.He, AMB)
            self._fwd(self.enc_head, he, self.E, AMB)
        return hd, he

    def _gp_stream(self):
        if not self.multi_stream:
            return None
        if self._gp_stream_obj is None:
            self._gp_stream_obj = torch.cuda.Stream(device=self.dev, priority=self._side_prio[2])
        return self._gp_stream_obj

    def phase_main(self, ds, idx, remap, amp_streams=None, new_z=None, inline_apply=False):
        be, c, M, AMB, st = self.be, self.cfg, self.M, self.AMB, self._st
        Ra, Rd = self.Ra, 3 * AMB
        if inline_apply:
            self._build_apply_desc()
        fork0 = st.early_fork if st.early_fork is not None else self._mark()
        disc_early = self.has_disc and st.early_fork is not None and self._disc_early

        if st.disc_fwd_out is not None:
            hd, he = st.disc_fwd_out
        elif disc_early:
            with self._Branch(self, self._side(1), fork0):
                hd, he = self._disc_forward(amp_streams)
        if st.pre_done is None:
            self._obs_inputs(ds, idx, remap)
        fork1 = self._mark()
        if st.prep is not None:
            be.wait(st.lat_ready)
        elif self.div_on:
            self._draw_new_latents(new_z)

        if self.style:
            sd = self.actor[0].split_dst
            h = self._fwd_chain(self.style[:-1], self.Zs, self.Hs, Ra)
            self._fwd(self.style[-1], h, self.Xa[:, sd:], Ra)
        ha = self._fwd_chain(self.actor, self.Xa, self.Ha, Ra)
        self._fwd(self.mu_head, ha, self.MU, Ra)

        with self._Branch(self, self._side(0), fork1) as br_critic:
            hc = self._fwd_chain(self.critic, self.Xc, self.Hc, M)
            self._fwd(self.value_head, hc, self.V, M)

        br_disc = None
        if self.has_disc:
            tnq, self._tn_queue = self._tn_queue, []
            with self._Branch(self, self._side(1), fork0) as br_disc:
                if not disc_early:
                    hd, he = self._disc_forward(amp_streams)
                be.disc_head(self.HD, self.dHD, self.disc_head.gb[0], self.acc, AMB, self._amb_den, c['disc_coef'],
                             grad_scale=self.gs, dyn=self._dS)
                if self.has_enc:
                    self._gather_enc_z(ds, amp_streams)
                    if self.enc_sep:
                        be.enc_head(self.E, self.enc_z, self.dE, self.enc_head.gb[0], None, self.acc, AMB, self._amb_den,
                                    self.z, c['enc_coef'], grad_scale=self.gs, dyn=self._dS)
                    else:
                        off = self.disc_head.parts[1][2]
                        be.enc_head(self.HD[:AMB, off:], self.enc_z, self.dHD[:AMB, off:], self.disc_head.gb[1], None,
                                    self.acc, AMB, self._amb_den, self.z, c['enc_coef'], grad_scale=self.gs, dyn=self._dS)
                if self.enc_gp:
                    self._enc_grad_penalty(he if self.enc_chain else hd[:AMB])
                self._wgrad(self.disc_head, self.dHD, hd, Rd)
                last = self.disc[-1]
                self._dgrad(self.disc_head, self.dHD, self.dZd[-1], Rd, self.Hd[-1], last.act)
                self._disc_backward()
                if self.enc_chain:
                    self._head_backward(self.enc_head, self.dE, he, self.enc_chain, self.Xd[:AMB], self.He, self.dZe, AMB)
                st.disc_acc_mark = self._mark()
                self._finish_branch('disc', inline_apply)
            self._tn_queue = tnq
        self._join_branch(br_critic)
        if st.prep is not None:
            self._join_branch(st.prep)
            if st.fill_done is not None:
                be.wait(st.fill_done)

        ls_kw = {}
        if self.sigma_mode == 'head':
            off = self.mu_head.parts[1][2]
            ls_kw = dict(ls_mode=L.LS_ROWS, d_logstd=self.dMU[:, off:], db_logstd=self.mu_head.gb[1],
                         entropy_coef=c.get('entropy_coef', 0.0))
        elif self.sigma_mode == 'vector':
            ls_kw = dict(ls_mode=L.LS_VECTOR, db_logstd=self.glogstd, entropy_coef=c.get('entropy_coef', 0.0))
        be.ppo_head(self.MU, self.V, self.mb, self.new_z if self.div_on else None, self._logstd_of(self.MU), self.dMU, self.dV,
                    self.mu_head.gb[0], self.value_head.gb[0], self.acc, M, self._m_den, self.act, self.z,
                    self.masked, self.div_on, self.mu_tanh, c['clip_value'], c['e_clip'], c['critic_coef'],
                    self.bounds_coef, c.get('amp_diversity_bonus', 0.0), c.get('amp_diversity_tar', 0.0), grad_scale=self.gs, dyn=self._dS,
                    **ls_kw)
        fork2 = self._mark()

        self._head_backward(self.mu_head, self.dMU, ha, self.actor, self.Xa, self.Ha, self.dZa, Ra)
        tn_actor, self._tn_queue = self._tn_queue, []
        with self._Branch(self, self._side(0), fork2) as br_cb:
            self._head_backward(self.value_head, self.dV, hc, self.critic, self.Xc, self.Hc, self.dZc, M)
            tn_actor = tn_actor + self._tn_queue
            self._tn_queue = []
        if self.style:
            a0, sdn = self.actor[0], self.style[-1]
            sd = a0.split_dst
            self._dgrad(a0, self.dZa[0], self.dStyle, Ra, self.Xa[:, sd:], sdn.act, wts=a0.Wts[sd:], n_out=P(self.z))
            hs_last = self.Hs[-1] if self.Hs else self.Zs
            self._wgrad(sdn, self.dStyle, hs_last, Ra)
            if self.Hs:
                p = self.style[-2]
                self._dgrad(sdn, self.dStyle, self.dZs[-1], Ra, self.Hs[-1], p.act)
                self._bwd_chain(self.style[:-1], self.Zs, self.Hs, self.dZs, Ra)
        self._join_branch(br_cb)
        self._tn_queue = tn_actor + self._tn_queue
        self._finish_branch('policy', inline_apply, last=True)
        if br_disc is not None:
            self._join_branch(br_disc)

    def phase_finish(self):
        if self._dist_shard() and not self._st.acc_in_bucket:
            self._ar(self.acc[1:L.ACC_LOGIT_W2])
        self._finalize(self._st.lr_live)

    def _finalize(self, apply):
        self._average_kl()
        self.be.finalize_scalars(self.acc, self.res, self._m_den, self._amb_den, self.masked, self.has_disc, self.has_enc,
                                 self.div_on, self.cfg, opt_state=self.opt_state if (self.adaptive_lr and apply) else None,
                                 kl_threshold=self.kl_threshold)

    def phase_apply(self, apply=True):
        be, c = self.be, self.cfg
        if apply and self._fused_apply and not self.truncate and not self.dyn_scale:
            self._build_apply_desc()
            self._apply(self.opt_state)
        else:
            if self.has_disc:
                for W, gW, coef, slot in self.l2_terms:
                    if coef != 0:
                        be.axpy(gW.view(-1), W.view(-1), coef)
# ... 113 lines not shown
        assert self.dyn_scale
        return False

    def _enc_grad_penalty(self, h_top):
        be, c, AMB = self.be, self.cfg, self.AMB
        sep = bool(self.enc_chain)
        chain = self.enc_chain if sep else self.disc
        head = self.enc_head if sep else self.disc_head
        H = self.He if sep else [h[:AMB] for h in self.Hd]
        for d in chain:
            assert d.act == L.ACT_RELU, "analytic gradient penalty needs ReLU encoder layers"
        if sep:
            e, d_e, db, off = self.E, self.dE, self.enc_head.gb[0], 0
        else:
            off = self.disc_head.parts[1][2]
            e, d_e, db = self.HD[:AMB, off:], self.dHD[:AMB, off:], self.disc_head.gb[1]
        cg = c['enc_coef'] * c['enc_grad_penalty'] * 2.0 / self._amb_den
        s = math.sqrt(cg)
        nl = len(chain)
        be.enc_gp_seed(e, self.enc_z, self.Ue[:, off:], AMB, self.z, scale=s)
        self._dgrad(head, self.Ue, self.Re[-1], AMB, H[-1], chain[-1].act)
        for l in range(nl - 1, 0, -1):
            self._dgrad(chain[l], self.Re[l], self.Re[l - 1], AMB, H[l - 1], chain[l - 1].act)
        d0 = chain[0]
        S = self.gs
        self._nt(self.Re[0], d0.Wts, self.Ge, AMB, d0.k_pad, d0.n_pad, alpha=S, alpha_dev=self._dS)
        be.sqnorm(self.Ge, AMB, d0.k_pad, self.acc, L.ACC_ENC_GP, scale=1.0 / (cg * S * S), dyn=self._dI2)
        x = self.Ge
        for l in range(nl):
            d = chain[l]
            aux, mode = self._aux(H[l], L.AUX_RELU_MASK)
            self._nt(x, d.Ws, self.Qe[l], AMB, d.n_pad, d.k_pad, aux=aux, aux_mode=mode)
            x = self.Qe[l]
        self._nt(x, head.Ws, self.DUe, AMB, head.n_pad, head.k_pad, alpha=s / S, alpha_dev=self._dI)
        for l in range(nl):
            d = chain[l]
            self._tn(self.Re[l], self.Ge if l == 0 else self.Qe[l - 1], d.gW[0], AMB, d.n_pad, d.k_pad, d.N, d.K,
                     d.split_src, d.split_dst)
        for (name, nr, poff), gW in zip(head.parts, head.gW):
            if sep or poff == off:
                self._tn(self.Ue[:, poff:], self.Qe[-1], gW, AMB, P(nr), head.k_pad, nr, head.K, head.split_src, head.split_dst)
        be.enc_gp_back(e, self.enc_z, self.DUe[:, off:], d_e, db, AMB, self.z, grad_scale=S, dyn=self._dS)

    def _gp_scales(self):
        if self.dyn_scale:
            return 64.0, 1.0 / 64.0
        e = int(round(math.log2(self.gs)))
        sc = 2.0 ** ((e + 1) // 2)
        return sc, self.gs / sc

    def _disc_backward(self):
        be, c, AMB = self.be, self.cfg, self.AMB
        Rd = 3 * AMB
        nl = len(self.disc)
        gp_coef = c['disc_coef'] * c['disc_grad_penalty']
        if gp_coef == 0:
            be.zero_(self.G0)
            self._bwd_chain(self.disc, self.Xd, self.Hd, self.dZd, Rd)
            return
        if self.gp32:
            return self._gp_f32(gp_coef)
        if any(d.act != L.ACT_RELU for d in self.disc):
            return self._disc_backward_curved(gp_coef)
        assert nl >= 2, "gradient penalty with a single discriminator layer is not implemented"
        cg = gp_coef * 2.0 / self.AMBg
        s = math.sqrt(cg)
        top = self.disc[-1]
        Sc, Sr = self._gp_scales()
        be.gp_seed(self.Hd[-1][2 * AMB:], self.disc_head.W[0].view(-1), self.Gp[-1], AMB, top.N, scale=s * Sc)
        for l in range(nl - 1, 0, -1):
            d, pl = self.disc[l], self.disc[l - 1]
            aux, mode = self._aux(self.Hd4[l - 1], _AUX[pl.act])
            self._nt(self.dZd4[l], d.Wts, self.dZd4[l - 1], 4 * AMB, d.k_pad, d.n_pad, aux=aux, aux_mode=mode,
                       aux_split=Rd, aux_delta=AMB)
        d0 = self.disc[0]
        self._nt(self.Gp[0], d0.Wts, self.G0, AMB, d0.k_pad, d0.n_pad, alpha=Sr / Sc, alpha_dev=self._dS)
        be.sqnorm(self.G0, AMB, d0.k_pad, self.acc, L.ACC_GP, scale=1.0 / (cg * Sr * Sr), dyn=self._dI2)
        self._gp_chain_backward(lambda l: self._aux(self.Hd[l][2 * AMB:], L.AUX_RELU_MASK), s / Sr)
        for l in range(nl):
            self._wgrad_stacked(l)

    def _gp_chain_backward(self, mask, top_scale):
        AMB, nl, d0 = self.AMB, len(self.disc), self.disc[0]
        aux, mode = mask(0)
        self._nt(self.G0, d0.Ws, self.dGp[0], AMB, d0.n_pad, d0.k_pad, aux=aux, aux_mode=mode)
        for l in range(1, nl):
            d = self.disc[l]
            last = l == nl - 1
            aux, mode = mask(l)
            self._nt(self.dGp[l - 1], d.Ws, self.GpTop if last else self.dGp[l], AMB, d.n_pad, d.k_pad, aux=aux,
                     aux_mode=mode, alpha=top_scale if last else 1.0, alpha_dev=self._dI if last else None)
            if last:
                self.be.colsum(self.GpTop, AMB, d.N, self.disc_head.gW[0].view(-1))

    def _wgrad_stacked(self, l):
        d, AMB = self.disc[l], self.AMB
        X = self.Xd4 if l == 0 else self.Hd4[l - 1]
        self._tn(self.dZd4[l], X, d.gW[0], 4 * AMB, d.n_pad, d.k_pad, d.N, d.K, d.split_src, d.split_dst,
                 gbias=d.gb[0], bias_rows=3 * AMB)

    def _gp_value(self, amp_streams, gp_coef):
        be, AMB, g = self.be, self.AMB, self._gp32
        nl, S = len(self.disc), self.gs
        s = math.sqrt(gp_coef * 2.0 / self.AMBg)
        bits = L.AUX_RELU_BITS
        if not self._st.gp_x_done:
            src, sidx, srm = amp_streams[2]
            be.rms_normalize(src, self.amp, sidx, srm, AMB, self.amp_mean[2], self.amp_std[2], [g.X])
        fuse = self._gp_fuse
        with self._gp_mode() as ex:
            if not self._gp_split:
                self._gp_refresh()
            top = self.disc[-1]
            x = g.X
            for l, d in enumerate(self.disc):
                if fuse and l == nl - 1:
                    self._nt(x, g.Ws[l], g.Gp[-1], AMB, d.n_pad, d.k_pad, bias=d.bs, act=L.ACT_RELU, mask_out=g.bits[l],
                             seed=(self.disc_head.W[0].view(-1), s), twin=self.Gp[-1], **ex(12 if l == 0 else 6))
                    break
                self._nt(x, g.Ws[l], g.H[l], AMB, d.n_pad, d.k_pad, bias=d.bs, act=L.ACT_RELU, mask_out=g.bits[l],
                           **ex(12 if l == 0 else 6))
                x = g.H[l]
            if not fuse:
                be.gp_seed(g.H[-1], self.disc_head.W[0].view(-1), g.Gp[-1], AMB, top.N, scale=s)
            for l in range(nl - 1, 0, -1):
                d = self.disc[l]
                self._nt(g.Gp[l], g.Wts[l], g.Gp[l - 1], AMB, d.k_pad, d.n_pad, aux=g.bits[l - 1], aux_mode=bits,
                         **({'twin': self.Gp[l - 1]} if fuse else {}), **ex(12))
            if not fuse:
                d0 = self.disc[0]
                self._nt(g.Gp[0], g.Wts[0], g.G0, AMB, d0.k_pad, d0.n_pad, alpha=S, alpha_dev=self._dS, **ex(12))

    @contextlib.contextmanager
    def _gp_mode(self):
        be = self.be
        x3_prev = getattr(be, 'x3', None)
        mode = self.cfg.get('gp_f32')
        half = mode == 'x3' and x3_prev is not None
        if half:
            be.x3 = 'f16'
        try:
            yield (lambda ea: {'x3_exps': (ea, 11)}) if half else (lambda ea: {})
        finally:
            if x3_prev is not None:
                be.x3 = x3_prev

    def _gp_f32(self, gp_coef):
        AMB, g, S, d0 = self.AMB, self._gp32, self.gs, self.disc[0]
        cg = gp_coef * 2.0 / self.AMBg
        s = math.sqrt(cg)
        if self._st.gp_value_done is not None:
            self._join_branch(self._st.gp_value_done)
            self._st.gp_value_done = None
        if self._gp_fuse:
            with self._gp_mode() as ex:
                self._nt(g.Gp[0], g.Wts[0], g.G0, AMB, d0.k_pad, d0.n_pad, alpha=S, alpha_dev=self._dS, twin=self.G0, store=False,
                         sq=(self.acc, L.ACC_GP, 1.0 / (cg * S * S), self._dI2), **ex(12))
        else:
            self._gp_convert(cg)
        self._gp_backward(s)

    def _gp_convert(self, cg):
        be, AMB, g = self.be, self.AMB, self._gp32
        nl, S, d0 = len(self.disc), self.gs, self.disc[0]
        be.sqnorm(g.G0, AMB, d0.k_pad, self.acc, L.ACC_GP, scale=1.0 / (cg * S * S), dyn=self._dI2)
        if g.cast is None:
            code = {torch.bfloat16: L.BF16, torch.float16: L.F16}[self.dtype]
            items = [(g.Gp[l], self.disc[l].n_pad, self.Gp[l]) for l in range(nl)] + [(g.G0, d0.k_pad, self.G0)]
            rows = [[src.data_ptr(), src.stride(0), c, dst.data_ptr(), dst.stride(0), code] for src, c, dst in items]
            g.cast = (torch.tensor(rows, dtype=torch.int64, device=self.dev), items)
        be.gather_multi(g.cast[0], g.cast[1], None, (0, 0), AMB)

    def _gp_backward(self, s):
        g, nl = self._gp32, len(self.disc)
        for l in range(nl - 1, 0, -1):
            self._dgrad(self.disc[l], self.dZd[l], self.dZd[l - 1], 3 * self.AMB, self.Hd[l - 1], self.disc[l - 1].act)
        self._gp_chain_backward(lambda l: (g.bits[l], L.AUX_RELU_BITS), s / self.gs)
        for l in range(nl):
            self._wgrad_stacked(l)

    def _disc_backward_curved(self, gp_coef):
        be, AMB = self.be, self.AMB
        Rd, nl = 3 * AMB, len(self.disc)
        cg = gp_coef * 2.0 / self.AMBg
        s = math.sqrt(cg)
        demo = slice(2 * AMB, 3 * AMB)
        top = self.disc[-1]
        Sc, Sr = self._gp_scales()
        be.gp_seed(self._twin(self.Hd[-1][demo], top), self.disc_head.W[0].view(-1), self.Gp[-1], AMB, top.N, scale=s * Sc,
                   act=top.act)
        for l in range(nl - 1, 0, -1):
            d, pl = self.disc[l], self.disc[l - 1]
            aux, mode = self._aux(self.Hd[l - 1][demo], _AUX[pl.act])
            self._nt(self.Gp[l], d.Wts, self.Gp[l - 1], AMB, d.k_pad, d.n_pad, aux=aux, aux_mode=mode)
        d0 = self.disc[0]
        self._nt(self.Gp[0], d0.Wts, self.G0, AMB, d0.k_pad, d0.n_pad, alpha=Sr / Sc, alpha_dev=self._dS)
        be.sqnorm(self.G0, AMB, d0.k_pad, self.acc, L.ACC_GP, scale=1.0 / (cg * Sr * Sr), dyn=self._dI2)
        x = self.G0
        for l in range(nl):
            d = self.disc[l]
            last = l == nl - 1
            aux, mode = self._aux(self.Hd[l][demo], _AUX[d.act])
            self._nt(x, d.Ws, self.GpTop if last else self.dGp[l], AMB, d.n_pad, d.k_pad, aux=aux, aux_mode=mode,
                       alpha=s / Sr if last else 1.0, alpha_dev=self._dI if last else None)
            if last:
                be.colsum(self.GpTop, AMB, d.N, self.disc_head.gW[0].view(-1))
            if last:
                self._nt(x, d.Ws, self.dGp[l], AMB, d.n_pad, d.k_pad, aux=aux, aux_mode=mode)
            x = self.dGp[l]
        for l in range(nl - 1, -1, -1):
            d = self.disc[l]
            be.gp_second(self._twin(self.Hd[l][demo], d), self.Gp[l], self.dGp[l], self.dZd[l][demo], AMB, d.N, d.act)
            self._wgrad_stacked(l)
            if l > 0:
                pl = self.disc[l - 1]
                self._dgrad(d, self.dZd[l], self.dZd[l - 1], Rd, self.Hd[l - 1], pl.act)

    def _host(self, fn):
        if self.dev.type != 'cuda':
            self.be.host_call(fn)
            return
        s = torch.cuda.current_stream(self.dev)

        def run():
            with torch.cuda.stream(s):
                fn()
        self.be.host_call(run)

    @staticmethod
    def _staged(op, t):
        import torch.distributed as dist
        if t.is_cuda and dist.get_backend() == 'gloo':
            h = t.cpu()
            op(h)
            t.copy_(h)
        else:
            op(t)

    def _ar(self, t):
        import torch.distributed as dist
# ... 146 lines not shown
```

ase_amd/lib.py:

```python
import ctypes as C
import os

_HERE = os.path.dirname(os.path.abspath(__file__))
LIB_PATH = os.path.join(_HERE, "csrc", "libase_hip.so")

ABI_VERSION = 9
PPO_SCRATCH = 1024 * 72 + 8
PPO_SCRATCH_LS = 1024 * 136 + 8
LS_FROZEN, LS_VECTOR, LS_ROWS = 0, 1, 2
TN_SLAB = 65536 + 256
F32, BF16, F32X3, F16, F32H3 = 0, 1, 2, 3, 4
ACT_NONE, ACT_RELU, ACT_TANH, ACT_SILU, ACT_ELU, ACT_GELU, ACT_SIGMOID, ACT_SELU, ACT_SOFTPLUS = range(9)
AUX_NONE, AUX_RELU_MASK, AUX_TANH_GRAD, AUX_RELU_BITS, AUX_PREACT = 0, 1, 2, 3, 4
TASK_HEADING, TASK_LOCATION, TASK_REACH, TASK_STRIKE = range(4)
TASK_OBS_COLS = (5, 2, 3, 15)
TASK_RESET_DRAWS = (3, 2, 3, 4)
RESET_FRAME, RESET_TABLE, RESET_MOTION = range(3)
RESET_HAS_TABLE, RESET_HAS_MOTION = 1, 2
KIND_U8, KIND_I32, KIND_I64, KIND_F32 = range(4)
ROLLOUT_STORE_MAX_FIELDS, ROLLOUT_STORE_ROWS = 16, 8
PROJ_DRAWS, PROJ_MAX_SLOTS = 7, 32
INIT_DEFAULT, INIT_START, INIT_RANDOM, INIT_HYBRID = range(4)

(ACC_MASK_SUM, ACC_A_LOSS, ACC_B_LOSS, ACC_ENTROPY, ACC_CLIPPED, ACC_C_LOSS, ACC_KL, ACC_DIV, ACC_BCE_AGENT,
 ACC_BCE_DEMO, ACC_AGENT_ACC, ACC_DEMO_ACC, ACC_GP, ACC_ENC, ACC_ENC_GP, ACC_LOGIT_W2, ACC_DISC_W2, ACC_ENC_W2,
 ACC_GRAD_SQ) = range(19)
ACC_COUNT = 24
(RES_A_LOSS, RES_C_LOSS, RES_B_LOSS, RES_ENTROPY, RES_CLIP_FRAC, RES_KL, RES_DISC_LOSS, RES_DISC_GP,
 RES_DISC_LOGIT_LOSS, RES_DISC_AGENT_ACC, RES_DISC_DEMO_ACC, RES_ENC_LOSS, RES_DIV_LOSS, RES_LOSS,
 RES_MASK_SUM, RES_ENC_GP, RES_LR) = range(17)
RES_COUNT = 20

_p, _i, _i64, _f, _d = C.c_void_p, C.c_int, C.c_int64, C.c_float, C.c_double

SIGNATURES = {
    "ase_hip_gemm_nt": [_p, _i64, _p, _i64, _p, _i64, _p, _p, _i64, _i, _i, _p, _i, _p, _i64, _i, _i, _i, _i, _i, _i, _f, _p, _i, _p],
    "ase_hip_gemm_nt_ex": [_p, _i64, _p, _i64, _p, _i64, _p, _p, _i64, _i, _i, _p, _i, _p, _i64, _i, _i, _i, _i, _i, _i, _f, _p, _i,
                           _p, _i, _f, _p, _i64, _i, _p, _d, _p, _p],
    "ase_hip_gemm_tn": [_p, _i64, _p, _i64, _p, _p, _i, _i, _i, _i, _i, _i, _i, _i, _f, _p, _i, _p],
    "ase_hip_refresh_shadow": [_p, _i, _i, _p, _i64, _p, _i64, _i, _i, _i, _p],
    "ase_hip_refresh_shadow_multi": [_p, _i, _i, _p],
    "ase_hip_gather_multi": [_p, _i, _p, _i, _i, _i, _p],
    "ase_hip_rms_moments": [_p, _i64, _i, _p, _i, _i, _i, _p, _p, _p],
    "ase_hip_rms_finalize": [_p, _i, _p, _p, _i, _p, _p, _p],
    "ase_hip_rms_normalize": [_p, _i64, _i, _p, _i, _i, _i, _p, _p, _p, _i64, _p, _i64, _p, _i64, _i, _p],
    "ase_hip_rms_unnormalize": [_p, _p, _p, _i64, _p],
    "ase_hip_gather_rows": [_p, _i64, _i, _p, _i, _i, _i, _p, _i64, _i, _p],
    "ase_hip_reduce_sum": [_p, _i64, _i, _p, _i, _p],
    "ase_hip_ppo_head": [_p, _i64, _p, _i64] + [_p] * 11 + [_p, _i64, _p, _i64, _p, _p, _p, _p, _p] + [_i] * 8 + [_f] * 6 + [_p]
                        + [_i, _i64, _p, _i64, _p, _f] + [_i, _p],
    "ase_hip_disc_head": [_p, _i64, _p, _i64, _p, _p, _i, _i, _f, _f, _p, _i, _p],
    "ase_hip_enc_head": [_p, _i64, _p, _i64, _p, _i64, _p, _p, _p, _i, _i, _i, _f, _f, _p, _i, _p],
    "ase_hip_gp_seed": [_p, _i64, _p, _p, _i64, _i, _i, _f, _i, _i, _p],
    "ase_hip_gp_second": [_p, _i64, _p, _i64, _p, _i64, _p, _i64, _i, _i, _i, _i, _p],
    "ase_hip_colsum": [_p, _i64, _i, _i, _f, _p, _p],
    "ase_hip_sqnorm": [_p, _i64, _i, _i, _p, _i, _d, _p, _i, _p],
    "ase_hip_finalize_scalars": [_p, _p, _i, _i, _i, _i, _i, _i] + [_f] * 11 + [_p, _f, _p],
    "ase_hip_enc_gp_seed": [_p, _i64, _p, _i64, _p, _i64, _i, _i, _f, _i, _p],
    "ase_hip_enc_gp_back": [_p, _i64, _p, _i64, _p, _i64, _p, _i64, _p, _i, _i, _f, _p, _i, _p],
    "ase_hip_clip_scale": [_p, _i64, _p, _f, _p],
    "ase_hip_begin_step": [_p, _p, _i, _p, _i, _p, _p],
    "ase_hip_adam": [_p, _p, _p, _p, _i64, _p, _p],
    "ase_hip_axpy": [_p, _p, _i64, _f, _p],
    "ase_hip_scaler_check": [_p, _i64, _i, _p, _p],
    "ase_hip_scaler_check_multi": [_p, _i, _i, _p, _p],
    "ase_hip_scaler_fold": [_p, _p, _p],
    "ase_hip_scaler_step": [_p, _p, _p, _p, _i64, _p, _p],
    "ase_hip_disc_reward": [_p, _i64, _p, _i64, _f, _p],
    "ase_hip_enc_reward": [_p, _i64, _p, _i64, _p, _i64, _i, _f, _p],
    "ase_hip_gae": [_p, _p, _p, _p, _p, _p, _f, _f, _f, _d, _d, _p, _p, _i, _i, _p],
    "ase_hip_adv_norm": [_p, _p, _p, _p, _p, _i64, _i, _i, _p],
    "ase_hip_ring_store": [_p, _i64, _i, _p, _i, _i, _i, _p, _i64, _i64, _p],
    "ase_hip_sample_latents": [_p, _i, _i, _p, _i64, _i, _p, _i64, _i, _p],
    "ase_hip_rms_moments_multi": [_p, _p, _p, _p, _p, _p, _i, _i, _i, _p, _p],
    "ase_hip_rms_normalize_multi": [_p, _p, _p, _p, _p, _p, _p, _p, _p, _i, _i, _i, _i, _p],
    "ase_hip_rms_normalize_multi_v2": [_p, _p, _p, _p, _p, _p, _p, _p, _p, _p, _p, _i, _i, _i, _i, _p],
    "ase_hip_normalize_rows": [_p, _i64, _p, _i64, _i, _i, _p],
    "ase_hip_sample_actions": [_p, _i64, _p, _i64, _p, _p, _p, _p, _p, _p, _p, _i, _i, _i, _p],
    "ase_hip_debug_nt_profile": [_p],
    "ase_hip_debug_nt_profile_clock": [_i],
    "ase_hip_motion_state": [_p] * 6 + [_i] + [_p] * 6 + [_i, _p, _p, _i, _p, _i] + [_p] * 8,
    "ase_hip_build_amp_obs": [_p, _p, _p, _p, _p, _p, _p, _i, _i, _i, _p, _i, _i, _i, _p, _i, _i, _p],
    "ase_hip_humanoid_obs_max": [_p, _p, _p, _p, _i, _i, _i, _i, _p, _i, _p, _i64, _i, _p],
    "ase_hip_humanoid_reset": [_p, _p, _p, _p, _p, _i, _p, _p, _i, _i, _i, _f, _i, _p, _p, _p],
    "ase_hip_task_obs": [_i, _p, _p, _p, _p, _p, _i, _p, _i, _p, _i64, _i, _p],
    "ase_hip_task_reward": [_i, _p, _p, _p, _p, _p, _f, _p, _p, _i, _i, _f, _i, _p, _p],
    "ase_hip_task_reset": [_i, _p, _i, _p, _p, _p, _i, _p, _p, _i64, _i64, _p, _i64, _p, _p, _p, _p, _i64] + [_d] * 8 + [_i, _i, _p],
    "ase_hip_proj_launch": [_p, _p, _i, _i, _p, _i, _p, _p, _p, _i, _p, _i64, _p, _i64, _i64, _p, _i64, _i64, _i, _i, _p, _i64, _i64]
                           + [_d] * 7 + [_p, _p, _p, _i, _p],
    "ase_hip_latent_renew": [_p, _i, _p, _i64, _p, _p, _i, _p, _i, _p, _i, _i64, _i64, _p, _i64, _p, _i64, _i, _i, _i, _p],
    "ase_hip_amp_reset": [_p] * 6 + [_i] + [_p] * 6 + [_i, _p, _i] + [_p] * 5 + [_i, _i, _p, _p, _p, _i, _p, _i64, _p, _p, _i64, _i,
                          _p, _p, _p, _p, _i, _i, _i, _f, _p, _i, _p],
    "ase_hip_amp_reset_due": [_p] * 6 + [_i] + [_p] * 6 + [_i, _p, _i] + [_p, _i] + [_p, _p, _p, _i] + [_i, _d, _i, _d, _d, _i]
                             + [_p, _i] + [_p] * 4 + [_p] * 5 + [_p, _i64, _p, _p, _i64, _i] + [_p] * 4 + [_i, _i, _i, _f, _p, _i, _p],
    "ase_hip_amp_demo_fetch": [_p] * 6 + [_i] + [_p] * 4 + [_i, _p, _p, _i, _p, _i] + [_p] * 4 + [_i, _p, _p] + [_i, _i, _f, _f, _i, _i]
                              + [_p, _i64, _i, _i, _p, _p],
    "ase_hip_rollout_store": [_p, _i, _p, _f, _f, _p, _i64, _p, _i, _p, _i64, _p, _p, _i, _p, _i64, _p, _p, _p, _i, _p, _i64, _p,
                              _i, _i, _p, _i, _p],
    "ase_hip_hrl_latent": [_p, _i64, _p, _i64, _p, _i64, _i, _i, _i, _p],
    "ase_hip_hrl_llc_action": [_p, _i64, _p, _p, _p, _i64, _i, _i, _i, _p],
    "ase_hip_hrl_accum": [_p, _p, _i, _p, _i, _p, _i64, _f, _p, _i64, _i, _i, _i, _p, _p, _p, _p, _i, _p],
    "ase_hip_env_pre_step": [_p, _i64, _f, _p, _i64, _p, _i64, _i, _p, _p, _p, _f, _p, _i64, _p, _p, _i, _i, _p],
    "ase_hip_env_post_step": [_p, _i64, _i64] * 7 + [_i, _i, _i, _i, _i, _p, _i64, _i, _f, _i, _i, _i, _p, _i64, _p, _p, _p, _p, _f, _p,
                              _i64, _i, _f, _p, _p, _p, _p, _i, _p, _i64, _p, _i, _f, _i, _p, _p, _p, _p, _i, _p, _i, _p, _i, _p],
    "ase_hip_clip_frames": [_p] * 6 + [_i] + [_p] * 4 + [_i, _i, _p, _p, _i] + [_p] * 7,
    "ase_hip_gemm_nt_kernel_id": [_i, _i, _i, _i],
    "ase_hip_gemm_tn_kernel_id": [_i, _i, _i, _i, _i, _i64, _i64, _i],
    "ase_hip_apply_multi": [_p, _i, _p, _p, _i, _p],
    "ase_hip_apply_multi_v2": [_p, _i, _p, _p, _p, _i, _p],
    "ase_hip_gemm_tn_grouped_plan": [_p, _i, _i, _p, _i, _p, _p, _i, _p],
    "ase_hip_prog_create": [_p],
    "ase_hip_prog_destroy": [_p],
    "ase_hip_prog_begin": [_p],
    "ase_hip_prog_end": [_p],
    "ase_hip_prog_size": [_p],
    "ase_hip_prog_launch": [_p],
    "ase_hip_prog_host": [_p, _p],
    "ase_hip_mark": [_p, _p],
    "ase_hip_wait": [_p, _i],
    "ase_hip_memset": [_p, _i, _i64, _p],
    "ase_hip_memcpy": [_p, _p, _i64, _p],
    "ase_hip_gemm_tn_grouped": [_p, _p, _i, _p, _i, _p, _p, _i, _p],
}


class AseHipError(RuntimeError):
    pass


def rollout_store_ws(n_envs):
    return 3 * ((int(n_envs) + ROLLOUT_STORE_ROWS - 1) // ROLLOUT_STORE_ROWS)


def load():
# ... 31 lines not shown
```

include/ase_hip.h:

```cpp
#ifndef ASE_HIP_H
#define ASE_HIP_H

#include <stdint.h>

#ifdef __cplusplus
extern "C" {
#endif

#define ASE_HIP_ABI_VERSION 9

enum { ASE_F32 = 0, ASE_BF16 = 1, ASE_F32X3 = 2 ,
       ASE_F32H3 = 4 ,
       ASE_F16 = 3  };
enum { ASE_ACT_NONE = 0, ASE_ACT_RELU = 1, ASE_ACT_TANH = 2, ASE_ACT_SILU = 3, ASE_ACT_ELU = 4, ASE_ACT_GELU = 5,
       ASE_ACT_SIGMOID = 6, ASE_ACT_SELU = 7, ASE_ACT_SOFTPLUS = 8 };
enum { ASE_AUX_NONE = 0, ASE_AUX_RELU_MASK = 1, ASE_AUX_TANH_GRAD = 2, ASE_AUX_RELU_BITS = 3 ,
       ASE_AUX_PREACT = 4  };
enum { ASE_OK = 0, ASE_EINVAL = -1, ASE_ELAUNCH = -2, ASE_EUNSUPPORTED = -3 };

int ase_hip_abi_version(void);
const char* ase_hip_last_error(void);

int ase_hip_gemm_nt_kernel_id(int M, int N, int K, int dtype);

int ase_hip_debug_nt_profile(void* buf);
int ase_hip_debug_nt_profile_clock(int shader_clock);


int ase_hip_gemm_nt(const void* A, int64_t lda, const void* B, int64_t ldb, void* C, int64_t ldc,
                    const float* bias, const void* aux, int64_t ldaux, int aux_split, int aux_delta,
                    float* colsum, int colsum_n, void* mask_out, int64_t ldmask, int M, int N, int K, int act,
                    int aux_mode, int out_f32, float alpha, float* alpha_dev, int dtype, void* stream);

int ase_hip_gemm_nt_ex(const void* A, int64_t lda, const void* B, int64_t ldb, void* C, int64_t ldc,
                       const float* bias, const void* aux, int64_t ldaux, int aux_split, int aux_delta,
                       float* colsum, int colsum_n, void* mask_out, int64_t ldmask, int M, int N, int K, int act,
                       int aux_mode, int out_f32, float alpha, float* alpha_dev, int dtype,
                       const float* seed_w, int seed_n, float seed_scale, void* twin, int64_t ldtwin, int twin_dtype,
                       double* sq_acc, double sq_scale, const float* sq_dyn, void* stream);

int ase_hip_gemm_tn(const void* A, int64_t lda, const void* B, int64_t ldb, float* G, float* gbias,
                    int bias_rows, int M, int N, int K, int n_real, int k_real, int split_src, int split_dst,
                    float alpha, const float* alpha_dev, int dtype, void* stream);

int ase_hip_gemm_tn_kernel_id(int M, int N, int K, int n_real, int bias_rows, int64_t lda, int64_t ldb, int dtype);

#define ASE_TN_SLAB (65536 + 256)
int ase_hip_gemm_tn_grouped_plan(int64_t* problems, int n_problems, int target_wg, int32_t* work, int max_work,
                                 int* n_work, int32_t* red, int max_red, int* n_red);
int ase_hip_gemm_tn_grouped(const int64_t* problems, const int32_t* work, int n_work, const int32_t* red, int n_red,
                            float* workspace, const float* alpha_dev, int dtype, void* stream);

int ase_hip_refresh_shadow(const float* W, int n_real, int k_real, void* Ws, int64_t ldws,
                           void* Wts, int64_t ldwts, int split_src, int split_dst, int dtype,
                           void* stream);

int ase_hip_refresh_shadow_multi(const int64_t* desc, int n_layers, int dtype, void* stream);


int ase_hip_rms_moments(const float* src, int64_t ld_src, int D, const int32_t* idx, int remap_h,
                        int remap_n, int M, const double* state, double* sums, void* stream);

int ase_hip_rms_moments_multi(const float* const* srcs, const int64_t* ld_srcs, const int32_t* const* idxs,
                              const int* remap_h, const int* remap_n, double* const* sums, int n_streams, int D, int M,
                              const double* state, void* stream);
int ase_hip_rms_normalize_multi(const float* const* srcs, const int64_t* ld_srcs, const int32_t* const* idxs,
                                const int* remap_h, const int* remap_n, const float* const* means,
                                const float* const* stds, void* const* outs, const int64_t* ld_outs, int n_streams, int D,
                                int M, int dtype, void* stream);
int ase_hip_rms_normalize_multi_v2(const float* const* srcs, const int64_t* ld_srcs, const int32_t* const* idxs,
                                   const int* remap_h, const int* remap_n, const float* const* means,
                                   const float* const* stds, void* const* outs, const int64_t* ld_outs,
                                   float* const* outs32, const int64_t* ld_outs32, int n_streams, int D, int M, int dtype,
                                   void* stream);

int ase_hip_rms_finalize(double* state, int D, const double* sums, const int32_t* counts ,
                         int n_streams, float* mean_out, float* std_out, void* stream);

int ase_hip_rms_normalize(const float* src, int64_t ld_src, int D, const int32_t* idx, int remap_h,
                          int remap_n, int M, const float* mean, const float* std,
                          void* out0, int64_t ld0, void* out1, int64_t ld1, void* out2, int64_t ld2,
                          int dtype, void* stream);

int ase_hip_rms_unnormalize(const double* state, const float* x, float* y, int64_t n, void* stream);

int ase_hip_gather_rows(const float* src, int64_t ld_src, int D, const int32_t* idx, int remap_h,
                        int remap_n, int M, void* dst, int64_t ld_dst, int dst_dtype, void* stream);

int ase_hip_gather_multi(const int64_t* desc, int n_fields, const int32_t* idx, int remap_h, int remap_n,
                         int M, void* stream);

enum {
    ASE_ACC_MASK_SUM = 0,
    ASE_ACC_A_LOSS,
    ASE_ACC_B_LOSS,
    ASE_ACC_ENTROPY,
    ASE_ACC_CLIPPED,
    ASE_ACC_C_LOSS,
    ASE_ACC_KL,
    ASE_ACC_DIV,
    ASE_ACC_BCE_AGENT,
    ASE_ACC_BCE_DEMO,
    ASE_ACC_AGENT_ACC,
    ASE_ACC_DEMO_ACC,
    ASE_ACC_GP,
    ASE_ACC_ENC,
    ASE_ACC_ENC_GP,
    ASE_ACC_LOGIT_W2,
    ASE_ACC_DISC_W2,
    ASE_ACC_ENC_W2,
    ASE_ACC_GRAD_SQ,
    ASE_ACC_COUNT = 24
};

int ase_hip_reduce_sum(const float* x, int64_t n, int square, double* acc, int slot, void* stream);

#define ASE_PPO_SCRATCH (1024 * 72 + 8)
#define ASE_PPO_SCRATCH_LS (1024 * 136 + 8)
#define ASE_LS_FROZEN 0
#define ASE_LS_VECTOR 1
#define ASE_LS_ROWS 2
int ase_hip_ppo_head(const float* mu, int64_t ld_mu, const float* value, int64_t ld_v,
                     const float* mb_actions, const float* mb_old_mu, const float* mb_old_sigma,
                     const float* mb_old_logp, const float* mb_adv, const float* mb_old_value,
                     const float* mb_return, const float* mb_mask, const float* mb_z,
                     const float* new_z, const float* logstd,
                     void* d_mu, int64_t ld_dmu, void* d_value, int64_t ld_dv,
                     float* db_mu, float* db_value, float* mu_out, double* acc, double* scratch,
                     int M, int m_global, int act_dim, int z_dim, int masked, int div_on, int mu_tanh,
                     int clip_value, float e_clip, float critic_coef, float bounds_coef,
                     float div_coef, float div_tar, float grad_scale, float* grad_scale_dev,
                     int ls_mode, int64_t ld_ls, void* d_ls, int64_t ld_dls, float* db_ls, float entropy_coef,
                     int dtype, void* stream);

int ase_hip_disc_head(const float* logit, int64_t ld_l, void* d_logit, int64_t ld_d, float* db_logit,
                      double* acc, int amb, int amb_global, float disc_coef, float grad_scale, float* grad_scale_dev, int dtype,
                      void* stream);

int ase_hip_enc_head(const float* e, int64_t ld_e, const float* z, int64_t ld_z, void* d_e,
                     int64_t ld_de, float* db_enc, float* enc_out, double* acc, int amb, int amb_global,
                     int z_dim, float enc_coef, float grad_scale, float* grad_scale_dev, int dtype, void* stream);

int ase_hip_enc_gp_seed(const float* e, int64_t ld_e, const float* z, int64_t ld_z, void* u, int64_t ld_u, int rows,
                        int z_dim, float scale, int dtype, void* stream);
int ase_hip_enc_gp_back(const float* e, int64_t ld_e, const float* z, int64_t ld_z, const float* du, int64_t ld_du,
                        void* d_e, int64_t ld_de, float* db_enc, int rows, int z_dim, float grad_scale, float* grad_scale_dev,
                        int dtype, void* stream);

int ase_hip_gp_seed(const void* h, int64_t ld_h, const float* w, void* g, int64_t ld_g, int rows,
                    int width, float scale, int act, int dtype, void* stream);

int ase_hip_gp_second(const void* twin, int64_t ld_t, const void* g, int64_t ld_g, const void* dg, int64_t ld_dg,
                      void* dz, int64_t ld_dz, int rows, int width, int act, int dtype, void* stream);

int ase_hip_colsum(const float* x, int64_t ld, int rows, int cols, float scale, float* out, void* stream);

int ase_hip_sqnorm(const void* x, int64_t ld, int rows, int cols, double* acc, int slot, double scale, const float* scale_dev,
                   int dtype, void* stream);

enum {
    ASE_RES_A_LOSS = 0, ASE_RES_C_LOSS, ASE_RES_B_LOSS, ASE_RES_ENTROPY, ASE_RES_CLIP_FRAC, ASE_RES_KL,
    ASE_RES_DISC_LOSS, ASE_RES_DISC_GP, ASE_RES_DISC_LOGIT_LOSS, ASE_RES_DISC_AGENT_ACC,
    ASE_RES_DISC_DEMO_ACC, ASE_RES_ENC_LOSS, ASE_RES_DIV_LOSS, ASE_RES_LOSS, ASE_RES_MASK_SUM, ASE_RES_ENC_GP,
    ASE_RES_LR,
    ASE_RES_COUNT = 20
};
int ase_hip_finalize_scalars(const double* acc, float* out, int m_global, int amb_global, int masked,
                             int has_disc, int has_enc, int has_div, float critic_coef,
                             float entropy_coef, float bounds_coef, float disc_coef, float disc_logit_reg,
                             float disc_grad_penalty, float disc_weight_decay, float enc_coef,
                             float enc_weight_decay, float div_coef, float enc_grad_penalty, double* opt_state_lr,
                             float kl_threshold, void* stream);

int ase_hip_clip_scale(float* g, int64_t n, const double* sqnorm, float max_norm, void* stream);

int ase_hip_begin_step(double* opt_state, double* acc, int n_acc, double* zero2, int n_zero2, uint64_t* rng_bump,
                       void* stream);
int ase_hip_adam(float* w, const float* g, float* m, float* v, int64_t n, const double* opt_state,
                 void* stream);
int ase_hip_axpy(float* g, const float* w, int64_t n, float c, void* stream);

int ase_hip_scaler_check(const void* buf, int64_t n, int dtype, double* scaler, void* stream);
int ase_hip_scaler_check_multi(const int64_t* table, int n_bufs, int wg_per_buf, double* scaler, void* stream);
int ase_hip_scaler_fold(double* scaler, float* scale_tab, void* stream);
int ase_hip_scaler_step(double* scaler, double* opt_state, double* opt_eff, float* grads, int64_t n, float* scale_tab,
                        void* stream);


int ase_hip_disc_reward(const float* logit, int64_t ld_l, float* r, int64_t n, float scale, void* stream);
int ase_hip_enc_reward(const float* e, int64_t ld_e, const float* z, int64_t ld_z, float* r, int64_t n,
                       int z_dim, float scale, void* stream);
int ase_hip_gae(const uint8_t* dones, const float* values, const float* next_values,
                const float* r_task, const float* r_disc, const float* r_enc, float w_task, float w_disc,
                float w_enc, double gamma, double tau, float* advs, float* returns, int H, int N, void* stream);
int ase_hip_adv_norm(const float* returns, const float* values, const float* mask, float* adv,
                     double* acc3, int64_t n, int normalize, int phase, void* stream);

int ase_hip_ring_store(const float* src, int64_t ld_src, int D, const int32_t* idx, int remap_h,
                       int remap_n, int n, float* dst, int64_t size, int64_t head, void* stream);

int ase_hip_normalize_rows(const float* x, int64_t ld_x, float* y, int64_t ld_y, int n, int dim, void* stream);

int ase_hip_sample_actions(const float* mu, int64_t ld_mu, const float* logstd, int64_t ld_logstd, const float* rand_probs,
                           uint64_t* rng_state, float* mu_out, float* sigma_out, float* actions, float* neglogp,
                           float* rand_mask, int n, int act_dim, int mu_tanh, void* stream);

int ase_hip_sample_latents(float* z, int rows, int dim, uint64_t* rng_state, int64_t row_offset, int advance,
                           void* z2 ,
                           int64_t ld_z2, int z2_dtype, void* stream);

enum { ASE_KIND_U8 = 0, ASE_KIND_I32 = 1, ASE_KIND_I64 = 2, ASE_KIND_F32 = 3 };
#define ASE_ROLLOUT_STORE_MAX_FIELDS 16
#define ASE_ROLLOUT_STORE_ROWS 8
#define ASE_ROLLOUT_STORE_WS(n_envs) (3 * (((n_envs) + ASE_ROLLOUT_STORE_ROWS - 1) / ASE_ROLLOUT_STORE_ROWS))
int ase_hip_rollout_store(const int64_t* fields, int n_fields, const float* rewards, float shift, float scale,
                          float* rewards_out, int64_t rewards_ss, const void* dones, int dones_kind, uint8_t* dones_out,
                          int64_t dones_ss, const float* next_values, const void* terminate, int terminate_kind,
                          float* next_values_out, int64_t next_values_ss, float* cur_rewards, float* cur_lengths,
                          double* meter, int max_size, double* workspace, int64_t workspace_doubles, int32_t* done_ids_out,
                          int n_envs, int slot, const int32_t* slot_dev, int n_slots, void* stream);
// ... 156 lines not shown
```

Measured before the change: 1.848 million samples/s.

## Stack disc forward and gradient-penalty backward rows into one NT GEMM launch

Adds a stacked NT GEMM kernel variant in which the row tiles above a split run the discriminator forward (bias, ReLU, mask output) and the row tiles below run the gradient-penalty chain backward (ReLU-bit mask, separate alpha), all over the same weight operand. The discriminator layers now make one launch over 4*AMB rows instead of separate forward and GP-backward launches, which cuts launch count and reuses the weights. The GP squared-norm term is reordered to accumulate into a scratch cell that is zeroed with the amp sums and folded into the loss accumulator by the disc head kernel. This moves the GP computation earlier in the schedule, adds a dependency between the stacked launch and the disc head, and falls back to two plain launches when the shape conditions are not met.

```diff
diff --git a/ase_amd/backend.py b/ase_amd/backend.py
--- a/ase_amd/backend.py
+++ b/ase_amd/backend.py
@@ -29,6 +29,7 @@
 class HipBackend:
     name = "hip"
     nt_fused_epilogue = True
+    nt_stack = True
 
     def __init__(self, device=None, x3=False):
         self.x3 = x3 if x3 == 'f16' else bool(x3)
@@ -112,7 +113,7 @@
 
     def gemm_nt(self, A, B, Cm, M, N, K, bias=None, aux=None, aux_mode=L.AUX_NONE, colsum=None, colsum_n=0,
                 act=L.ACT_NONE, alpha=1.0, aux_split=0, aux_delta=0, mask_out=None, x3_exps=None, alpha_dev=None,
-                seed=None, twin=None, sq=None, store=True):
+                seed=None, twin=None, sq=None, store=True, stack=None):
         dt = self._gemm_code(A.dtype, x3_exps)
         assert B.dtype == A.dtype
         if aux_mode == L.AUX_RELU_BITS:
@@ -136,6 +137,16 @@
                                                 _ptr(dyn), self._stream()), "gemm_nt_ex")
             return
         out_f32 = int(Cm.dtype == torch.float32 and A.dtype != torch.float32)
+        if stack is not None:
+            split, aux2, alpha2, alpha_dev2 = stack
+            assert aux is None and aux_mode == L.AUX_NONE and colsum is None, "a stacked launch takes its mask operand in stack=(...)"
+            assert aux2 is None or aux2.dtype == torch.int32
+            L.check(self.lib.ase_hip_gemm_nt_stacked(_ptr(A), _ld(A), _ptr(B), _ld(B), _ptr(Cm), _ld(Cm), _ptr(bias), _ptr(aux2),
+                                                     _ld(aux2), int(split), int(split), None, 0, _ptr(mask_out), _ld(mask_out),
+                                                     M, N, K, act, L.AUX_NONE if aux2 is None else L.AUX_RELU_BITS, out_f32,
+                                                     float(alpha), _ptr(alpha_dev), int(split), float(alpha2), _ptr(alpha_dev2), dt,
+                                                     self._stream()), "gemm_nt_stacked")
+            return
         L.check(self.lib.ase_hip_gemm_nt(_ptr(A), _ld(A), _ptr(B), _ld(B), _ptr(Cm), _ld(Cm), _ptr(bias), _ptr(aux),
                                          _ld(aux), int(aux_split), int(aux_delta), _ptr(colsum), int(colsum_n),
                                          _ptr(mask_out), _ld(mask_out), M, N, K, act, aux_mode, out_f32,
@@ -843,10 +854,11 @@
             self._head_scratch_ls = torch.zeros(L.PPO_SCRATCH_LS, dtype=torch.float64, device=self.device)
         return self._head_scratch_ls
 
-    def disc_head(self, logit, d_logit, db_logit, acc, amb, amb_global, disc_coef, grad_scale=1.0, dyn=None):
-        L.check(self.lib.ase_hip_disc_head(_ptr(logit), _ld(logit), _ptr(d_logit), _ld(d_logit), _ptr(db_logit),
-                                           _ptr(acc), amb, amb_global, float(disc_coef), float(grad_scale), _ptr(dyn),
-                                           _code(d_logit.dtype), self._stream()), "disc_head")
+    def disc_head(self, logit, d_logit, db_logit, acc, amb, amb_global, disc_coef, grad_scale=1.0, dyn=None, gp_add=None):
+        assert gp_add is None or gp_add.dtype == torch.float64
+        L.check(self.lib.ase_hip_disc_head_v2(_ptr(logit), _ld(logit), _ptr(d_logit), _ld(d_logit), _ptr(db_logit),
+                                              _ptr(acc), amb, amb_global, float(disc_coef), float(grad_scale), _ptr(dyn),
+                                              _ptr(gp_add), _code(d_logit.dtype), self._stream()), "disc_head")
 
     def enc_head(self, e, z, d_e, db_enc, enc_out, acc, amb, amb_global, z_dim, enc_coef, grad_scale=1.0, dyn=None):
         L.check(self.lib.ase_hip_enc_head(_ptr(e), _ld(e), _ptr(z), _ld(z), _ptr(d_e), _ld(d_e), _ptr(db_enc),
diff --git a/ase_amd/csrc/gemm.hip b/ase_amd/csrc/gemm.hip
--- a/ase_amd/csrc/gemm.hip
+++ b/ase_amd/csrc/gemm.hip
@@ -50,10 +50,10 @@
     bool any() const { return seed_w || twin || sq_acc; }
 };
 
-int gemm_nt_impl(const void* A, int64_t lda, const void* B, int64_t ldb, void* C, int64_t ldc,
-                 const float* bias, const void* aux, int64_t ldaux, int aux_split, int aux_delta,
-                 float* colsum, int colsum_n, void* mask_out, int64_t ldmask, int M, int N, int K, int act,
-                 int aux_mode, int out_f32, float alpha, float* alpha_dev, int dtype_word, const NTFused& fu, void* stream) {
+int nt_fill(NTParams& p, const void* A, int64_t lda, const void* B, int64_t ldb, void* C, int64_t ldc,
+            const float* bias, const void* aux, int64_t ldaux, int aux_split, int aux_delta,
+            float* colsum, int colsum_n, void* mask_out, int64_t ldmask, int M, int N, int K, int act,
+            int aux_mode, int out_f32, float alpha, float* alpha_dev, int dtype_word, const NTFused& fu) {
     const int dtype = dtype_word & 0xFF, ea = (dtype_word >> 8) & 0xFF, eb = (dtype_word >> 16) & 0xFF;
     const int es = ase_elem_size(dtype);
     ASE_CHECK_ARG(dtype == ASE_F32 || dtype == ASE_BF16 || dtype == ASE_F32X3 || dtype == ASE_F16 || dtype == ASE_F32H3,
@@ -90,7 +90,6 @@
                   "gemm_nt: mask_out needs N %% 32 == 0 and ldmask >= N / 32 words");
     ASE_CHECK_ARG(mask_out == nullptr || !smooth || (ldmask >= N && ((uintptr_t)mask_out % 16) == 0 && (ldmask * es) % 8 == 0),
                   "gemm_nt: the pre-activation twin needs ldmask >= N elements, 16-byte alignment");
-    NTParams p;
     p.A = (const char*)A; p.lda = lda * es;
     p.B = (const char*)B; p.ldb = ldb * es;
     p.C = (char*)C; p.ldc = ldc * (out_f32 ? 4 : es);
@@ -105,14 +104,27 @@
     p.seed_w = fu.seed_w; p.seed_n = fu.seed_n; p.seed_scale = fu.seed_scale;
     p.twin = (char*)fu.twin; p.ldtwin = fu.ldtwin * 2; p.twin_dtype = fu.twin_dtype;
     p.sq_acc = fu.sq_acc; p.sq_scale = fu.sq_scale; p.sq_dyn = fu.sq_dyn;
+    p.stack_split = 0; p.alpha2 = 0.f; p.alpha_dev2 = nullptr;
+    if (dtype == ASE_F32H3) {
+        p.sa = ldexpf(1.f, ea);
+        p.alpha = ldexpf(alpha, -(ea + eb));
+    }
+    return ASE_OK;
+}
+
+int gemm_nt_impl(const void* A, int64_t lda, const void* B, int64_t ldb, void* C, int64_t ldc,
+                 const float* bias, const void* aux, int64_t ldaux, int aux_split, int aux_delta,
+                 float* colsum, int colsum_n, void* mask_out, int64_t ldmask, int M, int N, int K, int act,
+                 int aux_mode, int out_f32, float alpha, float* alpha_dev, int dtype_word, const NTFused& fu, void* stream) {
+    NTParams p;
+    if (const int rc = nt_fill(p, A, lda, B, ldb, C, ldc, bias, aux, ldaux, aux_split, aux_delta, colsum, colsum_n, mask_out, ldmask, M, N, K,
+                               act, aux_mode, out_f32, alpha, alpha_dev, dtype_word, fu))
+        return rc;
+    const int dtype = dtype_word & 0xFF;
     if (dtype == ASE_BF16) return dispatch_nt_bf16(p, (hipStream_t)stream);
     if (dtype == ASE_F16) return dispatch_nt_f16(p, (hipStream_t)stream);
     if (dtype == ASE_F32X3) return dispatch_nt_x3(p, (hipStream_t)stream);
-    if (dtype == ASE_F32H3) {
-        p.sa = ldexpf(1.f, ea);
-        p.alpha = ldexpf(alpha, -(ea + eb));
-        return dispatch_nt_h3(p, (hipStream_t)stream);
-    }
+    if (dtype == ASE_F32H3) return dispatch_nt_h3(p, (hipStream_t)stream);
     return dispatch_nt_f32(p, (hipStream_t)stream);
 }
 
@@ -139,3 +151,34 @@
     return gemm_nt_impl(A, lda, B, ldb, C, ldc, bias, aux, ldaux, aux_split, aux_delta, colsum, colsum_n, mask_out, ldmask, M, N, K,
                         act, aux_mode, out_f32, alpha, alpha_dev, dtype_word, fu, stream);
 }
+
+extern "C" int ase_hip_gemm_nt_stacked(const void* A, int64_t lda, const void* B, int64_t ldb, void* C, int64_t ldc,
+                                       const float* bias, const void* aux, int64_t ldaux, int aux_split, int aux_delta,
+                                       float* colsum, int colsum_n, void* mask_out, int64_t ldmask, int M, int N, int K, int act,
+                                       int aux_mode, int out_f32, float alpha, float* alpha_dev, int split, float alpha2,
+                                       float* alpha_dev2, int dtype_word, void* stream) {
+    ASE_CHECK_ARG(M > 0 && split > 0 && split < M, "gemm_nt_stacked: split=%d outside (0, M=%d)", split, M);
+    ASE_CHECK_ARG(colsum == nullptr && out_f32 == 0, "gemm_nt_stacked: neither row block takes column sums or an f32 output");
+    ASE_CHECK_ARG(act == ASE_ACT_NONE || act == ASE_ACT_RELU, "gemm_nt_stacked: the first block's activation is NONE or RELU, not %d", act);
+    ASE_CHECK_ARG(mask_out == nullptr || act == ASE_ACT_RELU, "gemm_nt_stacked: mask_out only behind ReLU");
+    ASE_CHECK_ARG(aux_mode == ASE_AUX_NONE || aux_mode == ASE_AUX_RELU_BITS, "gemm_nt_stacked: the mask operand is a bit matrix, not mode %d",
+                  aux_mode);
+    ASE_CHECK_ARG(aux_mode == ASE_AUX_NONE || (aux_split == split && aux_delta == split),
+                  "gemm_nt_stacked: the mask operand belongs to the second block alone (aux_split = aux_delta = split)");
+    const int dtype = dtype_word & 0xFF, es = ase_elem_size(dtype);
+    NTParams p;
+    if (const int rc = nt_fill(p, A, lda, B, ldb, C, ldc, bias, aux, ldaux, 0, 0, nullptr, 0, mask_out, ldmask, M, N, K, act, aux_mode, 0,
+                               alpha, alpha_dev, dtype_word, NTFused{}))
+        return rc;
+    const bool fits32 = (int64_t)M * p.lda < (int64_t)0x7FFFFFFF && (int64_t)N * p.ldb < (int64_t)0x7FFFFFFF;
+    if ((dtype == ASE_BF16 || dtype == ASE_F16) && split % 256 == 0 && M < 65536 && fits32 && nt_choice(M, N, K, es, true) == 2) {
+        p.stack_split = split; p.alpha2 = alpha2; p.alpha_dev2 = alpha_dev2;
+        return dtype == ASE_F16 ? dispatch_nt_stacked_f16(p, (hipStream_t)stream) : dispatch_nt_stacked_bf16(p, (hipStream_t)stream);
+    }
+    if (const int rc = gemm_nt_impl(A, lda, B, ldb, C, ldc, bias, nullptr, 0, 0, 0, nullptr, 0, mask_out, ldmask, split, N, K, act, ASE_AUX_NONE,
+                                    0, alpha, alpha_dev, dtype_word, NTFused{}, stream))
+        return rc;
+    return gemm_nt_impl((const char*)A + (int64_t)split * lda * es, lda, B, ldb, (char*)C + (int64_t)split * ldc * es, ldc, nullptr, aux, ldaux,
+                        0, 0, nullptr, 0, nullptr, 0, M - split, N, K, ASE_ACT_NONE, aux_mode, 0, alpha2, alpha_dev2, dtype_word, NTFused{},
+                        stream);
+}
diff --git a/ase_amd/csrc/gemm_nt.h b/ase_amd/csrc/gemm_nt.h
--- a/ase_amd/csrc/gemm_nt.h
+++ b/ase_amd/csrc/gemm_nt.h
@@ -41,6 +41,9 @@
     const float* seed_w; int seed_n; float seed_scale;
     char* twin; int64_t ldtwin; int twin_dtype;
     double* sq_acc; double sq_scale; const float* sq_dyn;
+    int stack_split;
+    float alpha2;
+    float* alpha_dev2;
 };
 
 
@@ -249,5 +252,7 @@
 int dispatch_nt_f32(const NTParams& p, hipStream_t s);
 int dispatch_nt_x3(const NTParams& p, hipStream_t s);
 int dispatch_nt_h3(const NTParams& p, hipStream_t s);
-
-}
+int dispatch_nt_stacked_bf16(const NTParams& p, hipStream_t s);
+int dispatch_nt_stacked_f16(const NTParams& p, hipStream_t s);
+
+}
diff --git a/ase_amd/csrc/gemm_nt_bf16.hip b/ase_amd/csrc/gemm_nt_bf16.hip
--- a/ase_amd/csrc/gemm_nt_bf16.hip
+++ b/ase_amd/csrc/gemm_nt_bf16.hip
@@ -1,3 +1,4 @@
 #include "gemm_nt_kernels.h"
 
 int ase_nt::dispatch_nt_bf16(const NTParams& p, hipStream_t s) { return dispatch_nt<bf16_t>(p, s); }
+int ase_nt::dispatch_nt_stacked_bf16(const NTParams& p, hipStream_t s) { return dispatch_nt_stacked<bf16_t>(p, s); }
diff --git a/ase_amd/csrc/gemm_nt_f16.hip b/ase_amd/csrc/gemm_nt_f16.hip
--- a/ase_amd/csrc/gemm_nt_f16.hip
+++ b/ase_amd/csrc/gemm_nt_f16.hip
@@ -1,3 +1,4 @@
 #include "gemm_nt_kernels.h"
 
 int ase_nt::dispatch_nt_f16(const NTParams& p, hipStream_t s) { return dispatch_nt<f16_t>(p, s); }
+int ase_nt::dispatch_nt_stacked_f16(const NTParams& p, hipStream_t s) { return dispatch_nt_stacked<f16_t>(p, s); }
diff --git a/ase_amd/csrc/gemm_nt_kernels.h b/ase_amd/csrc/gemm_nt_kernels.h
--- a/ase_amd/csrc/gemm_nt_kernels.h
+++ b/ase_amd/csrc/gemm_nt_kernels.h
@@ -726,14 +726,17 @@
 }
 
 
-template <typename T, bool SW, int BM = 256>
+template <typename T, bool SW, int BM = 256, bool STK = false>
 __global__ __launch_bounds__(512) void gemm_nt8_kernel(NTParams p) {
     static_assert(sizeof(T) == 2, "the phased kernel takes the 16-bit storage types");
     static_assert(BM == 256 || (BM == 192 && SW), "192-row tiles come with the row-per-lane epilogue");
+    static_assert(!STK || (SW && BM == 256), "the stacked form comes with the row-per-lane epilogue on 256-row tiles");
     constexpr int RB = 128, BN = 256, BK = 64, WM = BM / 2, NI = WM / 32;
     constexpr int kBuf = 512 * RB;
     extern __shared__ __attribute__((aligned(16))) char smem[];
-    if (p.alpha_dev) p.alpha *= *p.alpha_dev;
+    if constexpr (!STK) {
+        if (p.alpha_dev) p.alpha *= *p.alpha_dev;
+    }
 
     const int tid = threadIdx.x, lane = tid & 63;
     const int wid = __builtin_amdgcn_readfirstlane(tid >> 6);
@@ -741,6 +744,18 @@
     const int nwg = p.tiles_m * p.tiles_n;
     const int tile = xcd_remap(blockIdx.x, nwg);
     const int bm0 = (tile / p.tiles_n) * BM, bn0 = (tile % p.tiles_n) * BN;
+    if constexpr (STK) {
+        if (bm0 >= p.stack_split) {
+            p.bias = nullptr;
+            p.act = ASE_ACT_NONE;
+            p.mask_out = nullptr;
+            p.alpha = p.alpha2;
+            p.alpha_dev = p.alpha_dev2;
+        } else {
+            p.aux_mode = ASE_AUX_NONE;
+        }
+        if (p.alpha_dev) p.alpha *= *p.alpha_dev;
+    }
 
     NT_PROF_STAMP(p.prof, tid, blockIdx.x * 4 + 0, false);
     NT8Lane L;
@@ -799,8 +814,10 @@
 #pragma unroll
             for (int i = 0; i < NI; ++i) {
                 const int m = bm0 + wr * WM + i * 32 + (lane & 31);
-                const int ma = (m >= p.aux_split) ? m - p.aux_delta : m;
-                const uint32_t* w = reinterpret_cast<const uint32_t*>(p.aux + (int64_t)min(ma, p.M - 1) * p.ldaux) +
+                int ma;
+                if constexpr (STK) ma = min(m, p.M - 1) - p.stack_split;
+                else ma = min((m >= p.aux_split) ? m - p.aux_delta : m, p.M - 1);
+                const uint32_t* w = reinterpret_cast<const uint32_t*>(p.aux + (int64_t)ma * p.ldaux) +
                                     ((bn0 + wc * 64) >> 5) + (lane >> 5);
                 __builtin_amdgcn_global_load_lds((gptr_t*)w, (lptr_t*)(mlds + i * 256), 4, 0, 0);
             }
@@ -850,9 +867,9 @@
     NT_PROF_CLOSE(p.prof, tid, blockIdx.x * 4 + 3);
 }
 
-template <typename T, bool SW = false, int BM = 256> int launch_nt8(const NTParams& p0, hipStream_t stream) {
+template <typename T, bool SW = false, int BM = 256, bool STK = false> int launch_nt8(const NTParams& p0, hipStream_t stream) {
     constexpr int lds = 2 * 512 * 128 + (SW ? 8 * 1024 : 0);
-    constexpr auto kern = gemm_nt8_kernel<T, SW, BM>;
+    constexpr auto kern = gemm_nt8_kernel<T, SW, BM, STK>;
     if (const int rc = ase_dynamic_lds<kern>("gemm_nt8", lds)) return rc;
     NTParams p = p0;
     p.prof = g_nt_prof;
@@ -922,4 +939,6 @@
     }
 }
 
-}
+template <typename T> int dispatch_nt_stacked(const NTParams& p, hipStream_t s) { return launch_nt8<T, true, 256, true>(p, s); }
+
+}
diff --git a/ase_amd/csrc/heads.hip b/ase_amd/csrc/heads.hip
--- a/ase_amd/csrc/heads.hip
+++ b/ase_amd/csrc/heads.hip
@@ -247,7 +247,7 @@
 __global__ __launch_bounds__(256) void disc_head_kernel(const float* __restrict__ logit, int64_t ld_l, T* __restrict__ d_logit,
                                                         int64_t ld_d, float* __restrict__ db_logit, double* __restrict__ acc,
                                                         int amb, int amb_global, float disc_coef, float gs,
-                                                        float* __restrict__ gs_dev) {
+                                                        float* __restrict__ gs_dev, const double* __restrict__ gp_add) {
     __shared__ double sm[5 * 16];
     if (gs_dev) gs *= *gs_dev;
     const int r = blockIdx.x * blockDim.x + threadIdx.x;
@@ -281,6 +281,7 @@
         atomic_add_f64(acc + ASE_ACC_BCE_DEMO, part[1]);
         atomic_add_f64(acc + ASE_ACC_AGENT_ACC, part[2]);
         atomic_add_f64(acc + ASE_ACC_DEMO_ACC, part[3]);
+        if (gp_add && blockIdx.x == 0) atomic_add_f64(acc + ASE_ACC_GP, *gp_add);
     }
 }
 
@@ -627,20 +628,28 @@
     return ASE_OK;
 }
 
-extern "C" int ase_hip_disc_head(const float* logit, int64_t ld_l, void* d_logit, int64_t ld_d, float* db_logit,
-                                 double* acc, int amb, int amb_global, float disc_coef, float grad_scale,
-                                 float* grad_scale_dev, int dtype, void* stream) {
+extern "C" int ase_hip_disc_head_v2(const float* logit, int64_t ld_l, void* d_logit, int64_t ld_d, float* db_logit,
+                                    double* acc, int amb, int amb_global, float disc_coef, float grad_scale,
+                                    float* grad_scale_dev, const double* gp_add, int dtype, void* stream) {
     ASE_CHECK_ARG(logit && d_logit && acc && amb > 0 && amb_global >= amb && grad_scale > 0.f, "disc_head: null/empty operand");
+    ASE_CHECK_ARG(((uintptr_t)gp_add % 8) == 0, "disc_head: misaligned gp_add");
     const dim3 grid((3 * amb + 255) / 256);
     const int rc = ase_dispatch_storage(dtype, [&](auto tag) {
         typedef typename decltype(tag)::type T;
         ASE_LAUNCH(disc_head_kernel<T>, grid, dim3(256), 0, (hipStream_t)stream, logit, ld_l, (T*)d_logit, ld_d, db_logit, acc, amb,
-                   amb_global, disc_coef, grad_scale, grad_scale_dev);
+                   amb_global, disc_coef, grad_scale, grad_scale_dev, gp_add);
         return ASE_OK;
     });
     ASE_CHECK_ARG(rc == ASE_OK, "disc_head: bad dtype %d", dtype);
     ASE_CHECK_LAUNCH("disc_head");
     return ASE_OK;
+}
+
+extern "C" int ase_hip_disc_head(const float* logit, int64_t ld_l, void* d_logit, int64_t ld_d, float* db_logit,
+                                 double* acc, int amb, int amb_global, float disc_coef, float grad_scale,
+                                 float* grad_scale_dev, int dtype, void* stream) {
+    return ase_hip_disc_head_v2(logit, ld_l, d_logit, ld_d, db_logit, acc, amb, amb_global, disc_coef, grad_scale, grad_scale_dev, nullptr,
+                                dtype, stream);
 }
 
 extern "C" int ase_hip_enc_head(const float* e, int64_t ld_e, const float* z, int64_t ld_z, void* d_e, int64_t ld_de,
diff --git a/ase_amd/engine.py b/ase_amd/engine.py
--- a/ase_amd/engine.py
+++ b/ase_amd/engine.py
@@ -16,6 +16,9 @@
         self.disc_fwd_out = self.stats_mark_a = self.stats_mark_b = self.pre_done = self.prep = self.lat_ready = None
         self.fill_done = self.early_fork = self.gp_value_done = self.disc_acc_mark = None
         self.merged_stats = self.stats_exchanged = self.enc_z_ready = self.gp_x_done = self.acc_in_bucket = self.lr_live = False
+
+
+_GP_STACK_AUTO = True
 
 
 class UpdateEngine(ForwardEngine):
@@ -67,7 +70,8 @@
         self.multi_stream = bool(cfg.get('multi_stream', True)) and getattr(backend, 'name', '') == 'hip'
         self._side_streams = None
         o = dict(tn_grouped=True, tn_wg_side=64, disc_early=True, short_prologue=True, relu_bits=True, fused_apply=True,
-                 apply_wide=True, xstep=True, gp_stream='auto', side_priority=None, prefetch=True, gp_fuse='auto')
+                 apply_wide=True, xstep=True, gp_stream='auto', side_priority=None, prefetch=True, gp_fuse='auto',
+                 gp_stack='auto')
         unknown = set(cfg.get('engine_opts', {}) or {}) - set(o)
         assert not unknown, f"unknown engine_opts {sorted(unknown)}"
         o.update(cfg.get('engine_opts', {}) or {})
@@ -86,6 +90,9 @@
         self._gp_fuse = bool(self.gp32 and getattr(backend, 'nt_fused_epilogue', False) and cfg.get('gp_f32') == 'x3'
                              and getattr(backend, 'x3', None) is not None and (o['gp_fuse'] == 'auto' or bool(o['gp_fuse'])))
         self._gp_split = self._gp_fuse and hasattr(backend, 'apply_multi_split') and self._fused_apply and dtype == torch.float16
+        self._gp_stack = bool(self._gp_fuse and not self._gp_side and not self.dyn_scale and getattr(backend, 'nt_stack', False)
+                              and world_size == 1 and not cfg.get('force_dist', False)
+                              and (_GP_STACK_AUTO if o['gp_stack'] == 'auto' else bool(o['gp_stack'])))
         self._prefetch = bool(o['prefetch'])
         self._par, self._par_set, self._last_par, self._fenced = 0, False, None, False
         sp = o['side_priority']
@@ -241,11 +248,14 @@
             self.amp_mean = zt(3, self.amp, f32)
             self.amp_std = zt(3, self.amp, f32)
         n_amp = 3 * 2 * self.amp if self.has_disc else 0
-        self.stats_flat = torch.zeros(n_amp + 2 * self.obs + 1, dtype=torch.float64, device=dev)
-        self.obs_sums = self.stats_flat[n_amp:n_amp + 2 * self.obs]
+        c0 = 1 if (self.has_disc and self._gp_stack) else 0
+        self.stats_flat = torch.zeros(c0 + n_amp + 2 * self.obs + 1, dtype=torch.float64, device=dev)
+        self.obs_sums = self.stats_flat[c0 + n_amp:c0 + n_amp + 2 * self.obs]
         if self.has_disc:
-            self.amp_sums_flat = self.stats_flat[:n_amp]
+            self.gp_sq = self.stats_flat[:c0]
+            self.amp_sums_flat = self.stats_flat[c0:c0 + n_amp]
             self.amp_sums = self.amp_sums_flat.view(3, 2 * self.amp)
+            self.amp_zero = self.stats_flat[:c0 + n_amp]
         self.obs_mean = zt(1, self.obs, f32)
         self.obs_std = zt(1, self.obs, f32)
         self.acc = torch.zeros(L.ACC_COUNT, dtype=torch.float64, device=dev)
@@ -522,7 +532,7 @@
             with self._Branch(self, self._side(1), nowait=True):
                 be.zero_(self.grads[lo:hi])
                 if not merged:
-                    be.zero_(self.amp_sums)
+                    be.zero_(self.amp_zero)
                 st.disc_fwd_out = self._disc_forward(amp_streams, ds)
         if pf:
             with self._Branch(self, self._side(0), nowait=True) as st.pre_done:
@@ -738,7 +748,16 @@
     def _disc_matrices(self):
         be, AMB = self.be, self.AMB
         Rd = 3 * AMB
-        hd = self._fwd_chain(self.disc, self.Xd, self.Hd, Rd)
+        if self._stacked():
+            g, X = self._gp32, self.Xd4
+            for l, d in enumerate(self.disc[:-1]):
+                self._nt(X, d.Ws, self.Hd4[l], 4 * AMB, d.n_pad, d.k_pad, bias=d.bs, act=d.act, mask_out=self._mask_of(self.Hd[l]),
+                         stack=(Rd, g.bits[l], 1.0, None))
+                X = self.Hd4[l]
+            self._fwd(self.disc[-1], X[:Rd], self.Hd[-1], Rd)
+            hd = self.Hd[-1]
+        else:
+            hd = self._fwd_chain(self.disc, self.Xd, self.Hd, Rd)
         self._fwd(self.disc_head, hd, self.HD, Rd)
         if self.logit_slot is not None:
             be.gather_rows(self.HD, 1, None, (0, 0), Rd, self.logit_slot)
@@ -747,6 +766,9 @@
             he = self._fwd_chain(self.enc_chain, self.Xd[:AMB], self.He, AMB)
             self._fwd(self.enc_head, he, self.E, AMB)
         return hd, he
+
+    def _stacked(self):
+        return self._gp_stack and len(self.disc) >= 2 and self.cfg['disc_coef'] * self.cfg['disc_grad_penalty'] != 0
 
     def _gp_stream(self):
         if not self.multi_stream:
@@ -794,7 +816,7 @@
                 if not disc_early:
                     hd, he = self._disc_forward(amp_streams)
                 be.disc_head(self.HD, self.dHD, self.disc_head.gb[0], self.acc, AMB, self._amb_den, c['disc_coef'],
-                             grad_scale=self.gs, dyn=self._dS)
+                             grad_scale=self.gs, dyn=self._dS, **({'gp_add': self.gp_sq} if self._stacked() else {}))
                 if self.has_enc:
                     self._gather_enc_z(ds, amp_streams)
                     if self.enc_sep:
@@ -1074,9 +1096,11 @@
 
     def _gp_chain_backward(self, mask, top_scale):
         AMB, nl, d0 = self.AMB, len(self.disc), self.disc[0]
-        aux, mode = mask(0)
-        self._nt(self.G0, d0.Ws, self.dGp[0], AMB, d0.n_pad, d0.k_pad, aux=aux, aux_mode=mode)
-        for l in range(1, nl):
+        stacked = self._stacked()
+        if not stacked:
+            aux, mode = mask(0)
+            self._nt(self.G0, d0.Ws, self.dGp[0], AMB, d0.n_pad, d0.k_pad, aux=aux, aux_mode=mode)
+        for l in range(nl - 1 if stacked else 1, nl):
             d = self.disc[l]
             last = l == nl - 1
             aux, mode = mask(l)
@@ -1122,6 +1146,14 @@
             if not fuse:
                 d0 = self.disc[0]
                 self._nt(g.Gp[0], g.Wts[0], g.G0, AMB, d0.k_pad, d0.n_pad, alpha=S, alpha_dev=self._dS, **ex(12))
+            elif self._stacked():
+                self._gp_last(gp_coef, ex, (self.gp_sq, 0))
+
+    def _gp_last(self, gp_coef, ex, sq_cell):
+        g, S, d0 = self._gp32, self.gs, self.disc[0]
+        cg = gp_coef * 2.0 / self.AMBg
+        self._nt(g.Gp[0], g.Wts[0], g.G0, self.AMB, d0.k_pad, d0.n_pad, alpha=S, alpha_dev=self._dS, twin=self.G0, store=False,
+                 sq=sq_cell + (1.0 / (cg * S * S), self._dI2), **ex(12))
 
     @contextlib.contextmanager
     def _gp_mode(self):
@@ -1144,10 +1176,11 @@
         if self._st.gp_value_done is not None:
             self._join_branch(self._st.gp_value_done)
             self._st.gp_value_done = None
-        if self._gp_fuse:
+        if self._stacked():
+            pass
+        elif self._gp_fuse:
             with self._gp_mode() as ex:
-                self._nt(g.Gp[0], g.Wts[0], g.G0, AMB, d0.k_pad, d0.n_pad, alpha=S, alpha_dev=self._dS, twin=self.G0, store=False,
-                         sq=(self.acc, L.ACC_GP, 1.0 / (cg * S * S), self._dI2), **ex(12))
+                self._gp_last(gp_coef, ex, (self.acc, L.ACC_GP))
         else:
             self._gp_convert(cg)
         self._gp_backward(s)
diff --git a/ase_amd/lib.py b/ase_amd/lib.py
--- a/ase_amd/lib.py
+++ b/ase_amd/lib.py
@@ -37,6 +37,8 @@
     "ase_hip_gemm_nt": [_p, _i64, _p, _i64, _p, _i64, _p, _p, _i64, _i, _i, _p, _i, _p, _i64, _i, _i, _i, _i, _i, _i, _f, _p, _i, _p],
     "ase_hip_gemm_nt_ex": [_p, _i64, _p, _i64, _p, _i64, _p, _p, _i64, _i, _i, _p, _i, _p, _i64, _i, _i, _i, _i, _i, _i, _f, _p, _i,
                            _p, _i, _f, _p, _i64, _i, _p, _d, _p, _p],
+    "ase_hip_gemm_nt_stacked": [_p, _i64, _p, _i64, _p, _i64, _p, _p, _i64, _i, _i, _p, _i, _p, _i64, _i, _i, _i, _i, _i, _i, _f, _p,
+                                _i, _f, _p, _i, _p],
     "ase_hip_gemm_tn": [_p, _i64, _p, _i64, _p, _p, _i, _i, _i, _i, _i, _i, _i, _i, _f, _p, _i, _p],
     "ase_hip_refresh_shadow": [_p, _i, _i, _p, _i64, _p, _i64, _i, _i, _i, _p],
     "ase_hip_refresh_shadow_multi": [_p, _i, _i, _p],
@@ -50,6 +52,7 @@
     "ase_hip_ppo_head": [_p, _i64, _p, _i64] + [_p] * 11 + [_p, _i64, _p, _i64, _p, _p, _p, _p, _p] + [_i] * 8 + [_f] * 6 + [_p]
                         + [_i, _i64, _p, _i64, _p, _f] + [_i, _p],
     "ase_hip_disc_head": [_p, _i64, _p, _i64, _p, _p, _i, _i, _f, _f, _p, _i, _p],
+    "ase_hip_disc_head_v2": [_p, _i64, _p, _i64, _p, _p, _i, _i, _f, _f, _p, _p, _i, _p],
     "ase_hip_enc_head": [_p, _i64, _p, _i64, _p, _i64, _p, _p, _p, _i, _i, _i, _f, _f, _p, _i, _p],
     "ase_hip_gp_seed": [_p, _i64, _p, _p, _i64, _i, _i, _f, _i, _i, _p],
     "ase_hip_gp_second": [_p, _i64, _p, _i64, _p, _i64, _p, _i64, _i, _i, _i, _i, _p],
diff --git a/include/ase_hip.h b/include/ase_hip.h
--- a/include/ase_hip.h
+++ b/include/ase_hip.h
@@ -38,6 +38,12 @@
                        int aux_mode, int out_f32, float alpha, float* alpha_dev, int dtype,
                        const float* seed_w, int seed_n, float seed_scale, void* twin, int64_t ldtwin, int twin_dtype,
                        double* sq_acc, double sq_scale, const float* sq_dyn, void* stream);
+
+int ase_hip_gemm_nt_stacked(const void* A, int64_t lda, const void* B, int64_t ldb, void* C, int64_t ldc,
+                            const float* bias, const void* aux, int64_t ldaux, int aux_split, int aux_delta,
+                            float* colsum, int colsum_n, void* mask_out, int64_t ldmask, int M, int N, int K, int act,
+                            int aux_mode, int out_f32, float alpha, float* alpha_dev, int split, float alpha2, float* alpha_dev2,
+                            int dtype, void* stream);
 
 int ase_hip_gemm_tn(const void* A, int64_t lda, const void* B, int64_t ldb, float* G, float* gbias,
                     int bias_rows, int M, int N, int K, int n_real, int k_real, int split_src, int split_dst,
@@ -136,6 +142,9 @@
 int ase_hip_disc_head(const float* logit, int64_t ld_l, void* d_logit, int64_t ld_d, float* db_logit,
                       double* acc, int amb, int amb_global, float disc_coef, float grad_scale, float* grad_scale_dev, int dtype,
                       void* stream);
+int ase_hip_disc_head_v2(const float* logit, int64_t ld_l, void* d_logit, int64_t ld_d, float* db_logit,
+                         double* acc, int amb, int amb_global, float disc_coef, float grad_scale, float* grad_scale_dev,
+                         const double* gp_add, int dtype, void* stream);
 
 int ase_hip_enc_head(const float* e, int64_t ld_e, const float* z, int64_t ld_z, void* d_e,
                      int64_t ld_de, float* db_enc, float* enc_out, double* acc, int amb, int amb_global,
```

Measured after the change: 1.897 million samples/s, median of 6. +2.7%, better.
